# lmb-freiburg/optical-flow-2d-data-generation

Measured on AMD Instinct MI355X. Metric: training samples/sec (img0+img1+flow, 512x384), higher is better.
Workload: dtype u8 blends / fp64 affines -> f32 planes

## Files before the change

### include/ofdg.h

```cpp
#ifndef OFDG_H_
#define OFDG_H_

#include <stddef.h>
#include <stdint.h>

#ifdef __cplusplus
extern "C" {
#endif

#define OFDG_OK          0
#define OFDG_EBADMODE   (-1)
#define OFDG_ETEXTURES  (-2)
#define OFDG_EOBJTYPE   (-3)
#define OFDG_EHIP       (-4)
#define OFDG_ECAPACITY  (-5)
#define OFDG_EINVAL     (-6)
#define OFDG_ESTARTUP   (-7)

#define OFDG_OBJ_DUMMY     0
#define OFDG_OBJ_ELLIPSE   1
#define OFDG_OBJ_POLYGON   2
#define OFDG_OBJ_COMPOSITE 3
#define OFDG_SEG_DUMMY     0
#define OFDG_SEG_LINE      1
// ... 130 lines not shown
  int32_t  reserved[3];
} ofdg_extras_fmt;
int ofdg_render_ex_fmt(ofdg_ctx* ctx, const ofdg_task* tasks, int n_tasks, const ofdg_blueprint* bps, int n_bps,
                       void* d_image0, void* d_image1, void* d_flow, const ofdg_extras_fmt* ex, const ofdg_out_format* fmt,
                       void* stream);
int ofdg_forward_ex_fmt(ofdg_ctx* ctx, void* d_image0, void* d_image1, void* d_flow, const ofdg_extras_fmt* ex,
                        const ofdg_out_format* fmt, void* stream);
int ofdg_forward_counter_ex_fmt(ofdg_ctx* ctx, long long first_index, int n_samples, void* d_image0, void* d_image1,
                                void* d_flow, const ofdg_extras_fmt* ex, const ofdg_out_format* fmt, void* stream);

#define OFDG_MAX_OBJECT_ROWS 65
typedef struct ofdg_object_row {
  int32_t obj_id;
  int32_t obj_type;
  int32_t area0, area1;
  int32_t box0[4];
  int32_t box1[4];
  double  motion[6];
} ofdg_object_row;
int ofdg_object_table(ofdg_ctx* ctx, const uint8_t* d_label0, const uint8_t* d_label1,
                      ofdg_object_row* d_rows, int rows_per_sample, int32_t* d_counts, void* stream);
int ofdg_host_object_table(const uint8_t* label0, const uint8_t* label1, int n, int width, int height,
                           const int32_t* counts, ofdg_object_row* rows, int rows_per_sample);

#define OFDG_FLOW_HIST_BINS 64
#define OFDG_STATS_ACCUMULATE   1
#define OFDG_STATS_VISIBLE_ONLY 2
#define OFDG_STATS_ONE_ROW      4
typedef struct ofdg_flow_stats_row {
  uint32_t hist[OFDG_FLOW_HIST_BINS];
  uint32_t n_counted, n_bad, n_occluded, reserved;
  int64_t  sum_u_q8, sum_v_q8, sum_mag_q8;
  uint64_t max_key;
} ofdg_flow_stats_row;
int ofdg_flow_stats(ofdg_ctx* ctx, const void* d_flow, int flow_fmt, const void* d_occ, int occ_fmt,
                    int n_samples, float bin_px, int flags, ofdg_flow_stats_row* d_rows, void* stream);
int ofdg_host_flow_stats(const void* flow, int flow_fmt, const void* occ, int occ_fmt, int n, int width, int height,
                         float bin_px, int flags, ofdg_flow_stats_row* rows);

#define OFDG_PYR_MAX_LEVELS 6
#define OFDG_PYR_SCALE 1
struct ofdg_flow_pyramid {
  void* flow[OFDG_PYR_MAX_LEVELS];
  void* weight[OFDG_PYR_MAX_LEVELS];
  int32_t levels;
  int32_t out_fmt;
};
int ofdg_flow_pyramid(ofdg_ctx* ctx, const void* d_flow, int flow_fmt, const void* d_occ, int occ_fmt,
                      int n_samples, int flags, const struct ofdg_flow_pyramid* pyr, void* stream);
int ofdg_host_flow_pyramid(const void* flow, int flow_fmt, const void* occ, int occ_fmt, int n, int width, int height,
                           int flags, const struct ofdg_flow_pyramid* pyr);

int ofdg_flow_stats_sized(ofdg_ctx* ctx, const void* d_flow, int flow_fmt, const void* d_occ, int occ_fmt, int n_samples,
                          int width, int height, float bin_px, int flags, ofdg_flow_stats_row* d_rows, void* stream);
int ofdg_flow_pyramid_sized(ofdg_ctx* ctx, const void* d_flow, int flow_fmt, const void* d_occ, int occ_fmt, int n_samples,
                            int width, int height, int flags, const struct ofdg_flow_pyramid* pyr, void* stream);

#define OFDG_CROP_HFLIP         1
#define OFDG_CROP_VFLIP         2
#define OFDG_CROP_RANDOM_HFLIP  4
#define OFDG_CROP_RANDOM_VFLIP  8
#define OFDG_CROP_OCC_WINDOW   16
typedef struct ofdg_crop_rec { int32_t x0, y0, flags, reserved; } ofdg_crop_rec;
enum { OFDG_CROP_IMAGE0, OFDG_CROP_IMAGE1, OFDG_CROP_FLOW, OFDG_CROP_FLOW1,
       OFDG_CROP_OCC0, OFDG_CROP_OCC1, OFDG_CROP_LABEL0, OFDG_CROP_LABEL1, OFDG_CROP_PLANES };
struct ofdg_crop_job {
  const void* src[OFDG_CROP_PLANES];
  void*       dst[OFDG_CROP_PLANES];
  const ofdg_crop_rec* recs;
  ofdg_crop_rec*       recs_out;
  long long first_index;  uint32_t seed;
  int32_t crop_w, crop_h, flags, image_fmt, flow_fmt, occ_fmt, reserved;
};
int ofdg_crop(ofdg_ctx* ctx, const struct ofdg_crop_job* job, int n_samples, void* stream);
int ofdg_host_crop(const struct ofdg_crop_job* job, int n_samples, int width, int height);
int ofdg_crop_draw(uint32_t seed, long long index, int width, int height, int crop_w, int crop_h, int flags, ofdg_crop_rec* out);
int ofdg_crop_philox(const uint32_t counter[4], const uint32_t key[2], uint32_t out[4]);

long long ofdg_get_step(const ofdg_ctx* ctx);
int ofdg_set_step(ofdg_ctx* ctx, long long step);

void* ofdg_stream(ofdg_ctx* ctx);
int ofdg_num_chains(const ofdg_ctx* ctx);

int ofdg_synchronize(ofdg_ctx* ctx, void* stream);

int ofdg_poll_errors(ofdg_ctx* ctx);
long long ofdg_last_ticket(const ofdg_ctx* ctx);
int ofdg_poll_errors_of(ofdg_ctx* ctx, long long ticket);

int ofdg_warp_generate(ofdg_ctx* ctx, int n_fields, uint32_t seed);
int ofdg_warp_upload(ofdg_ctx* ctx, const float* crops, int n);
int ofdg_warp_info(const ofdg_ctx* ctx, int* n_crops, int* w, int* h);
int ofdg_warp_download(ofdg_ctx* ctx, int index, float* crop);
int ofdg_host_displacers(int width, int height, uint32_t seed, double* out, int cap);

int ofdg_debug_rasterize(ofdg_ctx* ctx, const double* xy, int n_vertices,
                         uint8_t* coverage_host);
int ofdg_debug_rasterize_path(ofdg_ctx* ctx, const double* xy, const int* types, int n, uint8_t* coverage_host);
int ofdg_debug_dda_rows(ofdg_ctx* ctx, const double* inv, int rows, int len, int* out_xy);
int ofdg_debug_coverage(ofdg_ctx* ctx, int sample, int shape, int frame,
                        uint8_t* coverage_host);
int ofdg_debug_num_shapes(ofdg_ctx* ctx, int sample);
int ofdg_debug_item_count(ofdg_ctx* ctx);
int ofdg_debug_bgprep_tiles(ofdg_ctx* ctx, int* tiles, int* workgroups);
int ofdg_debug_bgprep_paths(ofdg_ctx* ctx, unsigned* counts9);
int ofdg_debug_tables(ofdg_ctx* ctx, uint8_t* add_tbl, uint8_t* sub_tbl, uint8_t* aa_tbl,
                      uint8_t* blend_tbl, int s_fixed);
int ofdg_debug_detmath(ofdg_ctx* ctx, const double* angles, int n, double* sin_out, double* cos_out,
                       const float* x, int m, float* expf_out);
int ofdg_set_profiling(ofdg_ctx* ctx, int mode);
int ofdg_kernel_ms(ofdg_ctx* ctx, const char* kernel, float* ms);

typedef struct ofdg_host_sampler ofdg_host_sampler;
int ofdg_host_sampler_create(int mode, int width, int height, int num_objects,
                             ofdg_host_sampler** out);
int ofdg_host_sampler_next(ofdg_host_sampler* s, int n_tasks, ofdg_task* tasks,
                           ofdg_blueprint* bps, int bps_capacity, int* n_bps);
void ofdg_host_sampler_destroy(ofdg_host_sampler* s);
int ofdg_host_realize(const ofdg_params* prm, int pool_n, int pool_w, int pool_h,
                      const ofdg_task* tasks, int n_tasks, const ofdg_blueprint* bps,
                      int n_bps, double* shape_mats, int shape_cap, int* n_shapes,
                      double* object_mats, int object_cap, int* n_objects);
int ofdg_host_bg_prep(int pool_w, int pool_h, int width, int height, float angle, float zoom,
                      int shift_x, int shift_y, float* f, int* i);

int ofdg_host_decode_image(const char* path, uint8_t* planar_bgr, size_t capacity, int* width, int* height);

int ofdg_parse_prototxt(const char* text, ofdg_params* out, char* texture_dbases,
                        int texture_dbases_cap, int* n_top);
const char* ofdg_host_last_error(void);

typedef struct ofdg_layer ofdg_layer;
int ofdg_layer_create(const char* layer_prototxt, ofdg_layer** out);
int ofdg_layer_forward(ofdg_layer* layer, float** image0, float** image1, float** flow,
                       int* shape4);
void ofdg_layer_destroy(ofdg_layer* layer);
int ofdg_layer_in_flight(const ofdg_layer* layer);

#define OFDG_UNIQUE_ID_BYTES 128
#define OFDG_POOL_SYNTHETIC 0
#define OFDG_POOL_UNIFORM   1
#define OFDG_POOL_MIXED     2
typedef struct ofdg_setup {
  int32_t seed, mode, width, height, num_objects, use_antialiasing, batch_size, sampler, background_prep;
  int32_t n_tex;
  int32_t pool_kind;
  int32_t pool_w, pool_h;
  uint32_t pool_seed;
  int32_t n_table;
  int32_t status;
  int32_t max_shapes_per_sample;
  int32_t reserved;
} ofdg_setup;
typedef struct ofdg_tex_entry {
  uint64_t offset;
  uint32_t w, h, pitch, reserved;
} ofdg_tex_entry;
typedef struct ofdg_comm ofdg_comm;
int ofdg_comm_unique_id(void* id);
int ofdg_comm_init(const void* id, int rank, int world_size, int device, ofdg_comm** out);
int ofdg_comm_adopt(void* nccl_comm, int rank, int world_size, int device, ofdg_comm** out);
void ofdg_comm_destroy(ofdg_comm* comm);
int ofdg_comm_rank(const ofdg_comm* comm);
int ofdg_comm_world_size(const ofdg_comm* comm);
const char* ofdg_comm_last_error(const ofdg_comm* comm);
// ... 18 lines not shown
```

### optical-flow-2d-data-generation_amd/__init__.py

```python
import ctypes as C
import os
import subprocess

HERE = os.path.dirname(os.path.abspath(__file__))
LIB_PATH = os.environ.get("OFDG_LIB") or os.path.join(HERE, "lib", "libofdg.so")
MAX_SEG = 20

OK, EBADMODE, ETEXTURES, EOBJTYPE, EHIP, ECAPACITY, EINVAL, ESTARTUP = 0, -1, -2, -3, -4, -5, -6, -7
OBJ_ELLIPSE, OBJ_POLYGON, OBJ_COMPOSITE = 1, 2, 3
STREAM_OWN = (1 << 64) - 1
SEG_DUMMY, SEG_LINE, SEG_CURVE3 = 0, 1, 3


class Blueprint(C.Structure):
    _fields_ = [
        ("obj_id", C.c_int32), ("obj_type", C.c_int32),
        ("init_rot", C.c_float), ("init_scale", C.c_float),
        ("init_trans_x", C.c_float), ("init_trans_y", C.c_float),
        ("rot", C.c_float), ("scale", C.c_float),
        ("trans_x", C.c_float), ("trans_y", C.c_float),
        ("tex_id", C.c_int32), ("tex_rot", C.c_float), ("tex_scale", C.c_float),
        ("tex_shift_x", C.c_int32), ("tex_shift_y", C.c_int32),
        ("ellipse_scale_x", C.c_float), ("ellipse_scale_y", C.c_float),
        ("n_segments", C.c_int32),
        ("segment_type", C.c_int32 * MAX_SEG),
        ("segment_x", C.c_float * MAX_SEG),
        ("segment_y", C.c_float * MAX_SEG),
        ("first_component", C.c_int32), ("n_components", C.c_int32),
        ("is_additive_component", C.c_int32),
        ("do_warpfield_deformation", C.c_int32),
    ]


class Task(C.Structure):
    _fields_ = [("background", C.c_int32), ("first_object", C.c_int32),
                ("n_objects", C.c_int32), ("reserved", C.c_int32)]


class Params(C.Structure):
    _fields_ = [
        ("width", C.c_int32), ("height", C.c_int32), ("mode", C.c_int32),
        ("use_antialiasing", C.c_int32), ("batch_size", C.c_int32), ("prefetch", C.c_int32),
        ("first_level_threads", C.c_int32), ("second_level_threads", C.c_int32),
        ("num_objects", C.c_int32), ("sampler", C.c_int32), ("seed", C.c_int32),
        ("rank", C.c_int32), ("world_size", C.c_int32), ("device", C.c_int32),
        ("max_shapes_per_sample", C.c_int32), ("background_prep", C.c_int32),
        ("chains", C.c_int32), ("lookahead", C.c_int32), ("serial", C.c_int32), ("reserved", C.c_int32 * 5),
    ]


class Setup(C.Structure):
    _fields_ = [(k, C.c_int32) for k in ("seed", "mode", "width", "height", "num_objects", "use_antialiasing", "batch_size",
                                         "sampler", "background_prep", "n_tex", "pool_kind", "pool_w", "pool_h")] + \
               [("pool_seed", C.c_uint32), ("n_table", C.c_int32), ("status", C.c_int32), ("max_shapes_per_sample", C.c_int32),
                ("reserved", C.c_int32)]


class TexEntry(C.Structure):
    _fields_ = [("offset", C.c_uint64), ("w", C.c_uint32), ("h", C.c_uint32), ("pitch", C.c_uint32), ("reserved", C.c_uint32)]


UNIQUE_ID_BYTES = 128
POOL_SYNTHETIC, POOL_UNIFORM, POOL_MIXED = 0, 1, 2


class OfdgError(RuntimeError):
    def __init__(self, code, msg):
        super().__init__("ofdg error %d: %s" % (code, msg))
        self.code = code


_lib = None

EXPORTS = [
    "ofdg_default_params", "ofdg_create", "ofdg_destroy", "ofdg_last_error", "ofdg_ctx_info",
    "ofdg_host_bg_prep", "ofdg_ctx_params", "ofdg_pool_alloc_mixed", "ofdg_pool_upload_mixed", "ofdg_pool_synthetic", "ofdg_pool_alloc", "ofdg_pool_upload", "ofdg_pool_download", "ofdg_pool_info", "ofdg_pool_device",
    "ofdg_sample", "ofdg_render", "ofdg_render_resident", "ofdg_upload_slot", "ofdg_render_slot", "ofdg_forward", "ofdg_shard_first_index", "ofdg_synchronize", "ofdg_stream", "ofdg_get_step", "ofdg_set_step",
    "ofdg_debug_rasterize", "ofdg_debug_rasterize_path", "ofdg_debug_dda_rows", "ofdg_debug_coverage", "ofdg_debug_num_shapes", "ofdg_debug_item_count", "ofdg_debug_bgprep_tiles", "ofdg_debug_bgprep_paths", "ofdg_debug_tables", "ofdg_debug_detmath",
    "ofdg_set_profiling", "ofdg_kernel_ms",
    "ofdg_forward_counter", "ofdg_sample_counter", "ofdg_warp_generate", "ofdg_warp_upload", "ofdg_warp_info", "ofdg_warp_download", "ofdg_host_displacers",
    "ofdg_host_sampler_create", "ofdg_host_sampler_next", "ofdg_host_sampler_destroy", "ofdg_host_realize",
    "ofdg_parse_prototxt", "ofdg_host_last_error", "ofdg_host_decode_image", "ofdg_layer_create", "ofdg_layer_forward", "ofdg_layer_destroy",
    "ofdg_layer_in_flight", "ofdg_poll_errors", "ofdg_poll_errors_of", "ofdg_last_ticket", "ofdg_num_chains",
    "ofdg_comm_unique_id", "ofdg_comm_init", "ofdg_comm_adopt", "ofdg_comm_destroy", "ofdg_comm_rank", "ofdg_comm_world_size",
    "ofdg_comm_last_error", "ofdg_comm_bcast_setup", "ofdg_comm_bcast_abort", "ofdg_comm_nccl_count", "ofdg_comm_bcast_pool", "ofdg_comm_agree", "ofdg_setup_of", "ofdg_setup_params",
    "ofdg_setup_alloc_pool", "ofdg_pool_device_mixed", "ofdg_pool_device_image", "ofdg_layer_create_dist",
    "ofdg_render_ex", "ofdg_forward_ex", "ofdg_forward_counter_ex",
    "ofdg_render_fmt", "ofdg_forward_fmt", "ofdg_forward_counter_fmt",
    "ofdg_render_ex_fmt", "ofdg_forward_ex_fmt", "ofdg_forward_counter_ex_fmt",
    "ofdg_object_table", "ofdg_host_object_table",
    "ofdg_flow_stats", "ofdg_host_flow_stats",
    "ofdg_flow_pyramid", "ofdg_host_flow_pyramid",
    "ofdg_flow_stats_sized", "ofdg_flow_pyramid_sized", "ofdg_crop", "ofdg_host_crop", "ofdg_crop_draw", "ofdg_crop_philox",
]

EXTRAS = {"flow1": (2, "float32"), "occ0": (1, "float32"), "occ1": (1, "float32"), "label0": (None, "uint8"), "label1": (None, "uint8")}


class Extras(C.Structure):
    _fields_ = [("flow1", C.c_void_p), ("occ0", C.c_void_p), ("occ1", C.c_void_p), ("label0", C.c_void_p), ("label1", C.c_void_p)]


FMT_F32, FMT_U8, FMT_F16 = 0, 1, 2
_FMT_NAMES = {"f32": FMT_F32, "u8": FMT_U8, "f16": FMT_F16}


class OutFormat(C.Structure):
    _fields_ = [("image", C.c_int32), ("flow", C.c_int32), ("reserved", C.c_int32 * 2)]


def output_format(image0, image1, flow, n, height, width):
    def name(t):
        return str(t.dtype).replace("torch.", "")

    if image0.dtype != image1.dtype:
        raise ValueError("image0 and image1 must have one dtype, got %s and %s" % (name(image0), name(image1)))
    codes = []
    for what, t, valid in (("image0", image0, {"float32": FMT_F32, "uint8": FMT_U8}), ("flow", flow, {"float32": FMT_F32, "float16": FMT_F16})):
        if name(t) not in valid:
            raise ValueError("%s must be %s, got %s" % (what, " or ".join(sorted(valid)), name(t)))
        codes.append(valid[name(t)])
    for what, t, ch in (("image0", image0, 3), ("image1", image1, 3), ("flow", flow, 2)):
        if t.numel() < n * ch * height * width:
            raise ValueError("%s holds %d elements, [%d,%d,%d,%d] needs %d" % (what, t.numel(), n, ch, height, width, n * ch * height * width))
    return tuple(codes)


class ExtrasFmt(C.Structure):
    _fields_ = [("flow1", C.c_void_p), ("occ0", C.c_void_p), ("occ1", C.c_void_p), ("label0", C.c_void_p), ("label1", C.c_void_p),
                ("occ", C.c_int32), ("reserved", C.c_int32 * 3)]


def extras_format(extras, flow_code, n, height, width):
    def name(t):
        return str(t.dtype).replace("torch.", "")

    flow_dt = {FMT_F32: "float32", FMT_F16: "float16"}[flow_code]
    occ_dt = None
    for key, t in extras.items():
        if key not in EXTRAS:
            raise ValueError("unknown extra output %r (known: %s)" % (key, ", ".join(EXTRAS)))
        if t is None:
            continue
        ch = EXTRAS[key][0]
        shape = (n, height, width) if ch is None else (n, ch, height, width)
        if key == "flow1":
            valid = (flow_dt,)
        elif key in ("occ0", "occ1"):
            valid = ("float32", "uint8") if occ_dt is None else (occ_dt,)
        else:
            valid = ("uint8",)
        if tuple(t.shape) != shape or name(t) not in valid:
            why = " (the dtype of flow)" if key == "flow1" else " (occ0 and occ1 alike)" if key in ("occ0", "occ1") else ""
            raise ValueError("extra %r must be %s %s%s, got %s %s" % (key, " or ".join(valid), shape, why, name(t), tuple(t.shape)))
        if key in ("occ0", "occ1"):
            occ_dt = name(t)
    return FMT_U8 if occ_dt == "uint8" else FMT_F32


def _fmt_codes(fmt):
    if fmt is None:
        return FMT_F32, FMT_F32
    image, flow = fmt
    return tuple(_FMT_NAMES[f] if isinstance(f, str) else int(f) for f in (image, flow))


# ... 239 lines not shown
        L.ofdg_default_params.restype = None
        L.ofdg_create.argtypes = [C.POINTER(Params), C.POINTER(vp)]
        L.ofdg_destroy.argtypes = [vp]
        L.ofdg_destroy.restype = None
        L.ofdg_last_error.argtypes = [vp]
        L.ofdg_last_error.restype = C.c_char_p
        L.ofdg_ctx_info.argtypes = [vp]
        L.ofdg_ctx_info.restype = C.c_char_p
        L.ofdg_pool_synthetic.argtypes = [vp, i32, i32, i32, C.c_uint32]
        L.ofdg_pool_alloc.argtypes = [vp, i32, i32, i32]
        L.ofdg_pool_upload.argtypes = [vp, i32, vp, i32, i32]
        L.ofdg_pool_download.argtypes = [vp, i32, vp]
        L.ofdg_pool_device.argtypes = [vp, C.POINTER(vp), C.POINTER(C.c_ulonglong), i32]
        L.ofdg_pool_info.argtypes = [vp, C.POINTER(i32), C.POINTER(i32), C.POINTER(i32)]
        L.ofdg_sample.argtypes = [vp, i32, vp, vp, i32, C.POINTER(i32)]
        L.ofdg_render.argtypes = [vp, vp, i32, vp, i32, vp, vp, vp, vp]
        L.ofdg_render_resident.argtypes = [vp, vp, vp, vp, vp]
        L.ofdg_upload_slot.argtypes = [vp, i32, vp, i32, vp, i32, vp]
        L.ofdg_render_slot.argtypes = [vp, i32, vp, vp, vp, vp]
        L.ofdg_forward.argtypes = [vp, vp, vp, vp, vp]
        L.ofdg_synchronize.argtypes = [vp, vp]
        L.ofdg_stream.argtypes = [vp]
        L.ofdg_get_step.argtypes = [vp]
        L.ofdg_get_step.restype = C.c_longlong
        L.ofdg_set_step.argtypes = [vp, C.c_longlong]
        L.ofdg_stream.restype = vp
        L.ofdg_debug_rasterize.argtypes = [vp, vp, i32, vp]
        L.ofdg_debug_rasterize_path.argtypes = [vp, vp, vp, i32, vp]
        L.ofdg_debug_dda_rows.argtypes = [vp, vp, i32, i32, vp]
        L.ofdg_debug_coverage.argtypes = [vp, i32, i32, i32, vp]
        L.ofdg_debug_num_shapes.argtypes = [vp, i32]
        L.ofdg_debug_tables.argtypes = [vp, vp, vp, vp, vp, i32]
        L.ofdg_debug_bgprep_tiles.argtypes = [vp, C.POINTER(i32), C.POINTER(i32)]
        L.ofdg_debug_bgprep_paths.argtypes = [vp, C.POINTER(C.c_uint32)]
        L.ofdg_debug_detmath.argtypes = [vp, vp, i32, vp, vp, vp, i32, vp]
        L.ofdg_set_profiling.argtypes = [vp, i32]
        L.ofdg_kernel_ms.argtypes = [vp, C.c_char_p, C.POINTER(C.c_float)]
        L.ofdg_forward_counter.argtypes = [vp, C.c_longlong, i32, vp, vp, vp, vp]
        L.ofdg_render_ex.argtypes = [vp, vp, i32, vp, i32, vp, vp, vp, C.POINTER(Extras), vp]
        L.ofdg_forward_ex.argtypes = [vp, vp, vp, vp, C.POINTER(Extras), vp]
        L.ofdg_forward_counter_ex.argtypes = [vp, C.c_longlong, i32, vp, vp, vp, C.POINTER(Extras), vp]
        L.ofdg_render_fmt.argtypes = [vp, vp, i32, vp, i32, vp, vp, vp, C.POINTER(OutFormat), vp]
        L.ofdg_forward_fmt.argtypes = [vp, vp, vp, vp, C.POINTER(OutFormat), vp]
        L.ofdg_forward_counter_fmt.argtypes = [vp, C.c_longlong, i32, vp, vp, vp, C.POINTER(OutFormat), vp]
        L.ofdg_render_ex_fmt.argtypes = [vp, vp, i32, vp, i32, vp, vp, vp, C.POINTER(ExtrasFmt), C.POINTER(OutFormat), vp]
        L.ofdg_forward_ex_fmt.argtypes = [vp, vp, vp, vp, C.POINTER(ExtrasFmt), C.POINTER(OutFormat), vp]
        L.ofdg_forward_counter_ex_fmt.argtypes = [vp, C.c_longlong, i32, vp, vp, vp, C.POINTER(ExtrasFmt), C.POINTER(OutFormat), vp]
        L.ofdg_object_table.argtypes = [vp, vp, vp, vp, i32, vp, vp]
        L.ofdg_host_object_table.argtypes = [vp, vp, i32, i32, i32, vp, vp, i32]
        L.ofdg_flow_stats.argtypes = [vp, vp, i32, vp, i32, i32, C.c_float, i32, vp, vp]
        L.ofdg_host_flow_stats.argtypes = [vp, i32, vp, i32, i32, i32, i32, C.c_float, i32, vp]
        L.ofdg_flow_pyramid.argtypes = [vp, vp, i32, vp, i32, i32, i32, C.POINTER(FlowPyramid), vp]
        L.ofdg_host_flow_pyramid.argtypes = [vp, i32, vp, i32, i32, i32, i32, i32, C.POINTER(FlowPyramid)]
        L.ofdg_flow_stats_sized.argtypes = [vp, vp, i32, vp, i32, i32, i32, i32, C.c_float, i32, vp, vp]
        L.ofdg_flow_pyramid_sized.argtypes = [vp, vp, i32, vp, i32, i32, i32, i32, i32, C.POINTER(FlowPyramid), vp]
        L.ofdg_crop.argtypes = [vp, C.POINTER(CropJob), i32, vp]
        L.ofdg_host_crop.argtypes = [C.POINTER(CropJob), i32, i32, i32]
        L.ofdg_crop_draw.argtypes = [C.c_uint32, C.c_longlong, i32, i32, i32, i32, i32, C.POINTER(CropRec)]
        L.ofdg_crop_philox.argtypes = [C.POINTER(C.c_uint32 * 4), C.POINTER(C.c_uint32 * 2), C.POINTER(C.c_uint32 * 4)]
        L.ofdg_sample_counter.argtypes = [vp, C.c_longlong, i32, vp, vp]
        L.ofdg_warp_generate.argtypes = [vp, i32, C.c_uint32]
        L.ofdg_warp_upload.argtypes = [vp, vp, i32]
        L.ofdg_warp_info.argtypes = [vp, C.POINTER(i32), C.POINTER(i32), C.POINTER(i32)]
        L.ofdg_warp_download.argtypes = [vp, i32, vp]
        L.ofdg_host_displacers.argtypes = [i32, i32, C.c_uint32, vp, i32]
        L.ofdg_host_sampler_create.argtypes = [i32, i32, i32, i32, C.POINTER(vp)]
        L.ofdg_host_sampler_next.argtypes = [vp, i32, vp, vp, i32, C.POINTER(i32)]
        L.ofdg_host_sampler_destroy.argtypes = [vp]
        L.ofdg_host_sampler_destroy.restype = None
        L.ofdg_host_realize.argtypes = [C.POINTER(Params), i32, i32, i32, vp, i32, vp, i32, vp, i32, C.POINTER(i32),
                                        vp, i32, C.POINTER(i32)]
        L.ofdg_parse_prototxt.argtypes = [C.c_char_p, C.POINTER(Params), C.c_char_p, i32, C.POINTER(i32)]
        L.ofdg_host_last_error.restype = C.c_char_p
        L.ofdg_layer_create.argtypes = [C.c_char_p, C.POINTER(vp)]
        L.ofdg_layer_forward.argtypes = [vp, C.POINTER(vp), C.POINTER(vp), C.POINTER(vp), C.POINTER(i32 * 4)]
        L.ofdg_layer_destroy.argtypes = [vp]
        L.ofdg_layer_destroy.restype = None
        L.ofdg_layer_in_flight.argtypes = [vp]
        L.ofdg_poll_errors.argtypes = [vp]
        L.ofdg_poll_errors_of.argtypes = [vp, C.c_longlong]
        L.ofdg_last_ticket.argtypes = [vp]
        L.ofdg_last_ticket.restype = C.c_longlong
        L.ofdg_num_chains.argtypes = [vp]
        L.ofdg_comm_unique_id.argtypes = [vp]
        L.ofdg_comm_init.argtypes = [vp, i32, i32, i32, C.POINTER(vp)]
        L.ofdg_comm_adopt.argtypes = [vp, i32, i32, i32, C.POINTER(vp)]
        L.ofdg_comm_destroy.argtypes = [vp]
        L.ofdg_comm_destroy.restype = None
        L.ofdg_comm_rank.argtypes = [vp]
        L.ofdg_comm_world_size.argtypes = [vp]
        L.ofdg_comm_last_error.argtypes = [vp]
        L.ofdg_comm_last_error.restype = C.c_char_p
        L.ofdg_comm_bcast_setup.argtypes = [vp, i32, C.POINTER(Setup), vp, i32]
        L.ofdg_comm_bcast_pool.argtypes = [vp, i32, vp]
        L.ofdg_comm_agree.argtypes = [vp, i32]
        L.ofdg_comm_bcast_abort.argtypes = [vp, i32, i32, i32]
        L.ofdg_comm_nccl_count.argtypes = [vp]
        L.ofdg_setup_of.argtypes = [vp, C.POINTER(Setup), vp, i32]
        L.ofdg_setup_params.argtypes = [C.POINTER(Setup), vp, C.POINTER(Params)]
        L.ofdg_setup_alloc_pool.argtypes = [vp, C.POINTER(Setup), vp]
        L.ofdg_pool_device_image.argtypes = [vp, i32, C.POINTER(vp), C.POINTER(C.c_ulonglong)]
        L.ofdg_pool_device_mixed.argtypes = [vp, C.POINTER(vp), C.POINTER(C.c_ulonglong), C.POINTER(vp), C.POINTER(C.c_ulonglong)]
        L.ofdg_layer_create_dist.argtypes = [C.c_char_p, vp, C.POINTER(vp)]
        _lib = L
    return _lib


def shard_first_index(step, batch, world_size, rank):
    L = lib()
    L.ofdg_shard_first_index.argtypes = [C.c_longlong, C.c_int, C.c_int, C.c_int]
    L.ofdg_shard_first_index.restype = C.c_longlong
    return int(L.ofdg_shard_first_index(step, batch, world_size, rank))


def default_params(**kw):
    p = Params()
    lib().ofdg_default_params(C.byref(p))
    for k, v in kw.items():
        setattr(p, k, v)
    return p


class Generator:

    def __init__(self, params=None, **kw):
        self.params = params if params is not None else default_params(**kw)
        h = C.c_void_p()
        rc = lib().ofdg_create(C.byref(self.params), C.byref(h))
        if rc != OK:
            raise OfdgError(rc, lib().ofdg_last_error(None).decode())
        self.h = h
        self._last_n = None
        self._slot_n = {}

    def _check(self, rc):
        if rc != OK:
            raise OfdgError(rc, lib().ofdg_last_error(self.h).decode())

    def info(self):
        return lib().ofdg_ctx_info(self.h).decode()

    def close(self):
        if getattr(self, "h", None):
            lib().ofdg_destroy(self.h)
            self.h = None

    def __del__(self):
        try:
            self.close()
        except Exception:
            pass

    def pool_synthetic(self, n, w, h, seed=0):
        self._check(lib().ofdg_pool_synthetic(self.h, n, w, h, seed))

    def pool_alloc(self, n, w, h):
        self._check(lib().ofdg_pool_alloc(self.h, n, w, h))

    def pool_from_setup(self, setup, table=None):
        self._check(lib().ofdg_setup_alloc_pool(self.h, C.byref(setup), table))

    def pool_upload(self, index, bgr_planar):
        import numpy as np
        a = np.ascontiguousarray(bgr_planar, np.uint8)
        _, h, w = a.shape
        self._check(lib().ofdg_pool_upload(self.h, index, a.ctypes.data_as(C.c_void_p), w, h))
# ... 115 lines not shown
    def render_resident(self, img0, img1, flow, stream=0):
        self._check(lib().ofdg_render_resident(self.h, _dptr(img0), _dptr(img1), _dptr(flow), C.c_void_p(stream)))

    def upload_slot(self, slot, tasks, n_tasks, bps, n_bps, stream=0):
        self._check(lib().ofdg_upload_slot(self.h, slot, C.cast(tasks, C.c_void_p), n_tasks, C.cast(bps, C.c_void_p), n_bps,
                                           C.c_void_p(stream)))
        self._slot_n[slot] = n_tasks

    def render_slot(self, slot, img0, img1, flow, stream=0):
        self._check(lib().ofdg_render_slot(self.h, slot, _dptr(img0), _dptr(img1), _dptr(flow), C.c_void_p(stream)))
        self._last_n = self._slot_n.get(slot)

    def forward(self, img0, img1, flow, stream=0, extras=None, fmt=None):
        self._call("forward", (), img0, img1, flow, self.params.batch_size, stream, extras, fmt)

    def forward_counter(self, first_index, n, img0, img1, flow, stream=0, extras=None, fmt=None):
        self._call("forward_counter", (first_index, n), img0, img1, flow, n, stream, extras, fmt)

    def object_table(self, label0, label1, rows, counts, stream=0):
        n, per = object_table_format(label0, label1, rows, counts, self.params.height, self.params.width, self._last_n)
        self._check(lib().ofdg_object_table(self.h, _dptr(label0) if label0 is not None else None,
                                            _dptr(label1) if label1 is not None else None, _dptr(rows), per, _dptr(counts),
                                            C.c_void_p(stream)))

    def flow_stats(self, flow, rows, occ=None, bin_px=2.0, accumulate=False, visible_only=False, one_row=False, stream=0, size=None):
        height, width = (int(size[0]), int(size[1])) if size is not None else (self.params.height, self.params.width)
        n, fcode, ocode = flow_stats_format(flow, occ, rows, height, width, one_row)
        entry, plane = (lib().ofdg_flow_stats_sized, (width, height)) if size is not None else (lib().ofdg_flow_stats, ())
        self._check(entry(self.h, _dptr(flow), fcode, _dptr(occ) if occ is not None else None, ocode, n, *plane, float(bin_px),
                          _stats_flags(accumulate, visible_only, one_row), _dptr(rows), C.c_void_p(stream)))

    def flow_pyramid(self, flow, levels, occ=None, scale=True, out_dtype=None, weights=False, out=None, stream=0, size=None):
        n, height, width = int(flow.shape[0]), self.params.height, self.params.width
        if size is not None:
            height, width = int(size[0]), int(size[1])
        if out is None:
            out = alloc_flow_pyramid(n, height, width, levels, flow.dtype if out_dtype is None else out_dtype, weights, flow.device)
        lv, wt = out if isinstance(out, tuple) else (out, None)
        n, fcode, ocode, out_code = flow_pyramid_format(flow, occ, levels, lv, wt, height, width)
        rec = _pyramid_record(int(levels), out_code, [_dptr(t) for t in lv], None if wt is None else [_dptr(t) for t in wt])
        entry, plane = (lib().ofdg_flow_pyramid_sized, (width, height)) if size is not None else (lib().ofdg_flow_pyramid, ())
        self._check(entry(self.h, _dptr(flow), fcode, _dptr(occ) if occ is not None else None, ocode, n, *plane,
                          PYR_SCALE if scale else 0, C.byref(rec), C.c_void_p(stream)))
        return out

    def crop(self, src, dst, recs=None, first_index=0, seed=None, hflip=False, vflip=False, occ_window=False, recs_out=None, stream=0):
        n, crop_h, crop_w, *codes = crop_format(src, dst, self.params.height, self.params.width)
        for t in (recs, recs_out):
            if t is not None and (str(t.dtype) != "torch.int32" or tuple(t.shape) != (n, 4)):
                raise ValueError("recs and recs_out must be int32 [%d,4], got %s %s" % (n, t.dtype, tuple(t.shape)))
        job = _crop_job(src, dst, _dptr, codes, crop_h, crop_w, None if recs is None else _dptr(recs), None if recs_out is None else _dptr(recs_out),
                        first_index, self.params.seed if seed is None else seed, _crop_flags(hflip, vflip, occ_window))
        self._check(lib().ofdg_crop(self.h, C.byref(job), n, C.c_void_p(stream)))
        return dst

    def sample_counter(self, first_index, n):
        tasks = (Task * n)()
        bps = (Blueprint * (n * 257))()
        self._check(lib().ofdg_sample_counter(self.h, first_index, n, C.cast(tasks, C.c_void_p), C.cast(bps, C.c_void_p)))
        return tasks, bps, n * 257

    def synchronize(self, stream=0):
        self._check(lib().ofdg_synchronize(self.h, C.c_void_p(stream)))

    def last_ticket(self):
        return int(lib().ofdg_last_ticket(self.h))

    def poll_errors(self):
        self._check(lib().ofdg_poll_errors(self.h))

    def poll_errors_of(self, ticket):
        self._check(lib().ofdg_poll_errors_of(self.h, ticket))

    @property
    def step(self):
        return int(lib().ofdg_get_step(self.h))

    @step.setter
    def step(self, k):
        self._check(lib().ofdg_set_step(self.h, int(k)))

    def num_chains(self):
        return lib().ofdg_num_chains(self.h)

    def next_stream(self):
        return int(lib().ofdg_stream(self.h) or 0)

    def warp_generate(self, n_fields=1, seed=0):
        self._check(lib().ofdg_warp_generate(self.h, n_fields, seed))

    def warp_upload(self, crops):
        import numpy as np
        a = np.ascontiguousarray(crops, np.float32)
        assert a.ndim == 4 and a.shape[1:] == (4, self.params.height + 1, self.params.width + 1), a.shape
        self._check(lib().ofdg_warp_upload(self.h, a.ctypes.data_as(C.c_void_p), a.shape[0]))

    def warp_count(self):
        n = C.c_int()
        self._check(lib().ofdg_warp_info(self.h, C.byref(n), None, None))
        return n.value

    def warp_download(self, index):
        import numpy as np
        a = np.zeros((4, self.params.height + 1, self.params.width + 1), np.float32)
        self._check(lib().ofdg_warp_download(self.h, index, a.ctypes.data_as(C.c_void_p)))
        return a

    def debug_rasterize(self, xy):
        import numpy as np
        xy = np.ascontiguousarray(xy, np.float64)
        cov = np.zeros((self.params.height, self.params.width), np.uint8)
        self._check(lib().ofdg_debug_rasterize(self.h, xy.ctypes.data_as(C.c_void_p), len(xy), cov.ctypes.data_as(C.c_void_p)))
        return cov

    def debug_rasterize_path(self, xy, types):
        import numpy as np
        xy = np.ascontiguousarray(xy, np.float64)
        types = np.ascontiguousarray(types, np.int32)
        cov = np.zeros((self.params.height, self.params.width), np.uint8)
        self._check(lib().ofdg_debug_rasterize_path(self.h, xy.ctypes.data_as(C.c_void_p), types.ctypes.data_as(C.c_void_p), len(xy),
                                                    cov.ctypes.data_as(C.c_void_p)))
        return cov

    def debug_dda_rows(self, inv, rows, length):
        import numpy as np
        inv = np.ascontiguousarray(inv, np.float64)
        out = np.zeros((rows, length, 2), np.int32)
        self._check(lib().ofdg_debug_dda_rows(self.h, inv.ctypes.data_as(C.c_void_p), rows, length, out.ctypes.data_as(C.c_void_p)))
        return out

    def debug_num_shapes(self, sample):
        n = lib().ofdg_debug_num_shapes(self.h, sample)
        if n < 0:
            raise OfdgError(n, "debug_num_shapes")
        return n

    def debug_coverage(self, sample, shape, frame):
        import numpy as np
        cov = np.zeros((self.params.height, self.params.width), np.uint8)
        self._check(lib().ofdg_debug_coverage(self.h, sample, shape, frame, cov.ctypes.data_as(C.c_void_p)))
        return cov

    def debug_bgprep_tiles(self):
        t, w = C.c_int(0), C.c_int(0)
        self._check(lib().ofdg_debug_bgprep_tiles(self.h, C.byref(t), C.byref(w)))
        return t.value, w.value

    def debug_bgprep_paths(self):
        c = (C.c_uint32 * 9)()
        self._check(lib().ofdg_debug_bgprep_paths(self.h, c))
        return [[int(c[3 * r + k]) for k in range(3)] for r in range(3)]

    def debug_tables(self, s_fixed=200):
        import numpy as np
        add = np.zeros((256, 256), np.uint8)
        sub = np.zeros((256, 256), np.uint8)
        aa = np.zeros(256, np.uint8)
        bl = np.zeros((256, 256), np.uint8)
        vp = C.c_void_p
        self._check(lib().ofdg_debug_tables(self.h, add.ctypes.data_as(vp), sub.ctypes.data_as(vp), aa.ctypes.data_as(vp),
                                            bl.ctypes.data_as(vp), s_fixed))
        return add, sub, aa, bl

    def debug_detmath(self, angles, x):
        import numpy as np
        a = np.ascontiguousarray(angles, np.float64)
# ... 550 lines not shown
```

### optical-flow-2d-data-generation_amd/csrc/kernels.hip

```cpp
#include <hip/hip_runtime.h>
#include <stdint.h>
#include <type_traits>

#include "../../include/ofdg_detmath.h"
#include "ofdg_device.h"
#include "realize.h"
#include "warpfields.h"

namespace ofdg {

__device__ __forceinline__ int iround_d(double v) {
  return (int)((v < 0.0) ? v - 0.5 : v + 0.5);
}
__device__ __forceinline__ void xform(const Mat& m, double& x, double& y) {
  double t = x;
  x = t * m.sx + y * m.shx + m.tx;
  y = t * m.shy + y * m.sy + m.ty;
}
__device__ __forceinline__ long long floordiv64(long long a, long long b) {
  long long q = (long long)floor((double)a / (double)b);
  long long r = a - q * b;
  if (r < 0) --q;
  else if (r >= b) ++q;
  return q;
// ... 146 lines not shown
      xform(M, x, y);
      const int2 v = make_int2(iround_d(x * 256.0), iround_d(y * 256.0));
      out[k] = v;
      minx = min(minx, v.x); maxx = max(maxx, v.x);
      miny = min(miny, v.y); maxy = max(maxy, v.y);
    }
  } else {
    n_verts = path_verts(S.n_seg, [&](int i) { return S.seg_type[i]; },
                         [&](int i, double& x, double& y) { x = (double)S.seg_x[i]; y = (double)S.seg_y[i]; xform(M, x, y); },
                         out, stack, stage, err, lane, minx, miny, maxx, maxy);
  }
  minx = wave_min(minx); miny = wave_min(miny); maxx = wave_max(maxx); maxy = wave_max(maxy);
  return n_verts;
}

struct GeomWs {
  double stack[kCurveSlots][kCurveMaxDepth][5];
  int2 stage[kCurveSlots][kCurveMaxPts];
};
__device__ __forceinline__ void geom_wave(GeomWs& ws, int sf, int lane, const DevShape* __restrict__ shapes, int n_shapes,
                                          const double* __restrict__ cs_tab, int W, int H, DevShapeFrame* __restrict__ frames,
                                          int2* __restrict__ verts, unsigned long long* __restrict__ blockmask, uint32_t* __restrict__ err,
                                          int* __restrict__ item_count, int4* __restrict__ items, const DevCropRef* __restrict__ crops) {
  if (sf >= n_shapes * 2) return;
  const DevShape& S = shapes[sf >> 1];
  if (S.type == 0) return;
  const Mat M = S.m[sf & 1];
  int2* out = verts + (size_t)sf * kMaxVerts;

  int minx, miny, maxx, maxy;
  int n_verts = outline_verts(S, M, cs_tab, out, ws.stack, ws.stage, err, lane, minx, miny, maxx, maxy);
  if (n_verts > 0 && ((long long)maxx - (long long)minx >= (16384LL << 8))) {
    if (lane == 0) atomicOr(err, kErrDxLimit);
    n_verts = 0;
  }
  int x0 = minx >> 8, y0 = miny >> 8, x1 = maxx >> 8, y1 = maxy >> 8;
  const bool visible = !(n_verts < 2 || x1 < 0 || y1 < 0 || x0 > W - 1 || y0 > H - 1);
  int bx0 = 1, by0 = 1, bx1 = 0, by1 = 0;
  if (visible) {
    x0 = max(x0, 0); y0 = max(y0, 0); x1 = min(x1, W - 1); y1 = min(y1, H - 1);
    bx0 = x0; by0 = y0; bx1 = x1; by1 = y1;
    if ((sf & 1) && S.deform > 0) {
      const int d = (int)ceilf(__uint_as_float(*crops[S.deform - 1].max_bits)) + 2;
      bx0 = max(x0 - d, 0); by0 = max(y0 - d, 0); bx1 = min(x1 + d, W - 1); by1 = min(y1 + d, H - 1);
    }
  } else {
    x0 = 1; x1 = 0; y0 = 1; y1 = 0;
  }
  if (lane == 0) {
    DevShapeFrame f;
    f.n_verts = n_verts;
    f.x0 = x0; f.y0 = y0; f.x1 = x1; f.y1 = y1;
    f.pad[0] = S.sample; f.pad[1] = S.obj_local; f.pad[2] = 0;
    frames[sf] = f;
  }
  if (visible) {
    const int band0 = by0 / kBandRows, band1 = by1 / kBandRows;
    if ((sf & 1) && S.deform > 0) {
      const int nbx = (W + kTileW - 1) / kTileW, nby = (H + kBandRows - 1) / kBandRows;
      const int c0 = bx0 / kTileW, nc = bx1 / kTileW - c0 + 1;
      unsigned long long* m = blockmask + ((size_t)S.sample * nbx * nby) * 2 + (sf & 1);
      const unsigned long long bit = 1ull << S.obj_local;
      for (int i = lane; i < (band1 - band0 + 1) * nc; i += 64)
        atomicOr(m + (size_t)((band0 + i / nc) * nbx + c0 + i % nc) * 2, bit);
    }
    const int xa = (bx0 / kTileW) * kTileW, xb = min((bx1 / kTileW) * kTileW + kTileW - 1, W - 1);
    const int nchunks = (xb - xa + kChunkW) / kChunkW;
    const int n_items = (band1 - band0 + 1) * nchunks;
    int base = 0;
    if (lane == 0) base = atomicAdd(item_count, n_items);
    base = __shfl(base, 0, 64);
    for (int i = lane; i < n_items; i += 64) {
      const int b = band0 + i / nchunks, cx = xa + (i % nchunks) * kChunkW;
      items[base + i] = make_int4(sf, b, cx, min(cx + kChunkW - 1, xb));
    }
  }
}

__global__ __launch_bounds__(64 * kGeomWaves) void geom_kernel(const DevShape* __restrict__ shapes, int n_shapes,
                                                   const double* __restrict__ cs_tab, int W, int H,
                                                   DevShapeFrame* __restrict__ frames, int2* __restrict__ verts,
                                                   unsigned long long* __restrict__ blockmask, uint32_t* __restrict__ err,
                                                   int* __restrict__ item_count, int4* __restrict__ items,
                                                   const DevCropRef* __restrict__ crops) {
  __shared__ GeomWs s_ws[kGeomWaves];
  step_kernel_priority();
  const int wave = threadIdx.x >> 6, lane = threadIdx.x & 63;
  const int sf = __builtin_amdgcn_readfirstlane(blockIdx.x * kGeomWaves + wave);
  geom_wave(s_ws[wave], sf, lane, shapes, n_shapes, cs_tab, W, H, frames, verts, blockmask, err, item_count, items, crops);
}

struct CellAcc {
  int* cover;
  int* area;
  int pitch, X0, X1;
  __device__ __forceinline__ void add(int r, int cell, int dcover, int darea) const {
    if (cell > X1 || dcover == 0) return;
    if (cell < X0) {
      atomicAdd(&cover[r * pitch], dcover);
    } else {
      const int i = r * pitch + (cell - X0 + 1);
      atomicAdd(&cover[i], dcover);
      atomicAdd(&area[i], darea);
    }
  }
};

__device__ __forceinline__ int fdiv_small(int num, int den, float rcp) {
  int q = (int)floorf((float)num * rcp);
  const int r = num - q * den;
  if (r < 0) --q;
  else if (r >= den) ++q;
  return q;
}
__device__ __forceinline__ int fdiv_big(int num, int den, float rcp) {
  const int q0 = (int)floorf((float)num * rcp);
  const int r0 = num - q0 * den;
  return q0 + fdiv_small(r0, den, rcp);
}

template <class Acc>
__device__ __forceinline__ void hline32(const Acc& acc, int r, int xa, int ya, int xb, int yb) {
  if (ya == yb) return;
  const int exa = xa >> 8, exb = xb >> 8;
  const int fxa = xa & 255, fxb = xb & 255;
  const int Dy = yb - ya;
  if (exa == exb) {
    acc.add(r, exa, Dy, (fxa + fxb) * Dy);
    return;
  }
  const int lo = min(exa, exb), hi = max(exa, exb);
  if (hi < acc.X0) { acc.add(r, acc.X0 - 1, Dy, 0); return; }
  if (lo > acc.X1) return;
  const bool right = xb > xa;
  const int adx = right ? xb - xa : xa - xb;
  const float rcp = __frcp_rn((float)adx);
  const int m = hi - lo;
  const int f0 = right ? 256 - fxa : fxa;
  const int j_lo = right ? max(0, acc.X0 - exa) : max(0, exa - acc.X1);
  const int j_hi = right ? min(m, acc.X1 - exa) : min(m, exa - acc.X0);
  int yprev = (j_lo == 0) ? ya : ya + fdiv_small((f0 + 256 * (j_lo - 1)) * Dy, adx, rcp);
  if (right && j_lo > 0) acc.add(r, acc.X0 - 1, yprev - ya, 0);
  for (int j = j_lo; j <= j_hi; ++j) {
    const int ynext = (j == m) ? yb : ya + fdiv_small((f0 + 256 * j) * Dy, adx, rcp);
    const int d = ynext - yprev;
    const int fin = (j == 0) ? fxa : (right ? 0 : 256);
    const int fout = (j == m) ? fxb : (right ? 256 : 0);
    acc.add(r, right ? exa + j : exa - j, d, (fin + fout) * d);
    yprev = ynext;
  }
  if (!right && j_hi < m) acc.add(r, acc.X0 - 1, yb - yprev, 0);
}

template <class Acc>
__device__ __forceinline__ void hline(const Acc& acc, int r, int xa, int ya, int xb, int yb) {
  if (ya == yb) return;
  const int exa = xa >> 8, exb = xb >> 8;
  const int fxa = xa & 255, fxb = xb & 255;
  const int Dy = yb - ya;
  if (exa == exb) {
    acc.add(r, exa, Dy, (fxa + fxb) * Dy);
    return;
  }
  if (xb > xa) {
    const int m = exb - exa;
    const long long dxh = xb - xa;
    const long long f0 = 256 - fxa;
    int j = 0;
    int yprev = ya;
    if (exa < acc.X0) {
      const int jb = min(acc.X0 - exa, m + 1);
      int yb0 = (jb > m) ? yb : ya + (int)floordiv64((f0 + 256LL * (jb - 1)) * Dy, dxh);
// ... 2802 lines not shown
```

### optical-flow-2d-data-generation_amd/csrc/ofdg_api.hip

```cpp
#include <hip/hip_runtime.h>
#include <hip/hip_ext.h>

#include <algorithm>
#include <cmath>
#include <cstddef>
#include <cstdio>
#include <cstdlib>
#include <cstring>
#include <memory>
#include <string>
#include <type_traits>
#include <vector>

#include "../../include/ofdg.h"
#include "kernels.hip"
#include "sampler_counter.hip"
#include "cimg_resize.h"
#include "ofdg_device.h"
#include "owners.h"
#include "realize.h"
#include "sampler_ref.h"
#include "warpfields.h"

using namespace ofdg;
// ... 2 lines not shown
static const int g_hw_queues_env = [] { const char* q = std::getenv("GPU_MAX_HW_QUEUES"); return q ? std::atoi(q) : 0; }();

struct ofdg_ctx {
  ofdg_params prm;
  std::string err;
  std::string info;
  DevBuf<uint32_t> d_prep_paths;
  DevBuf<uint32_t> pool;
  int pool_n = 0, pool_w = 0, pool_h = 0;
  DevBuf<uint32_t> pool_fg;
  DevBuf<uint32_t> pool_bg;
  TexSource fg_src{}, bg_src{};
  bool pool_final = false;
  bool pool_mixed = false;
  std::vector<std::pair<int, int>> mixed_sizes;
  std::vector<DevBuf<uint32_t>> mixed_images;
  std::vector<DevTexEntry> tex_table;
  DevBuf<DevTexEntry> d_tex_table;
  int pool_kind = OFDG_POOL_UNIFORM;
  uint32_t pool_seed = 0;
  std::unique_ptr<RefSampler> sampler;
  long long step = 0;
  struct Slot {
    RealizedBatch batch;
    DevBuf<DevShape> d_shapes;
    DevBuf<DevShapeFrame> d_frames;
    DevBuf<int2> d_verts;
    DevBuf<DevObject> d_objects;
    DevBuf<DevSample> d_samples;
    DevBuf<char> d_rec;
    DevBuf<int4> d_items;
    DevBuf<DevBgPrep> d_bgprep;
    DevBuf<uint32_t> d_bgtex;
    DevBuf<uint32_t> d_bgC;
    DevBuf<unsigned long long> d_blockmask;
    int res_objects = 0;
    bool bgprep_pending = false;
    int box_parity = 0;
    size_t box_stride = 0;
    int mask_used[2] = {0, 0};
    Event ev_uploaded;
    bool upload_pending = false;
    hipStream_t upload_stream = nullptr;
    DevBuf<DevCropRef> d_croptab;
    DevBuf<float> d_bgwarp;
    DevBuf<unsigned> d_bgwarp_max;
    hipEvent_t compose_event = nullptr;
    bool compose_pending = false;
    hipStream_t compose_stream = nullptr;
    DevBuf<int> d_item_count;
    int res_samples = 0, res_shapes = 0;
  };
  static constexpr int kUserSlots = 16;
  Slot slots[kUserSlots];
  struct Stage {
    PinnedBuf h;
    Event free_ev;
    bool pending = false;
  };
  Stage user_stage;
  struct Chain {
    Stream stream;
    DevBuf<uint8_t> cov;
    DevBuf<uint8_t> x_labels;
    DevBuf<float> x_flow1;
    DevBuf<uint32_t> x_targets;
    Slot slot;
    Stage stage;
    Event ev_prep;
    Event ev_done;
    bool done_pending = false;
    hipStream_t done_stream = nullptr;
    struct Prepared {
      bool valid = false;
      Slot* slot = nullptr;
      long long first_index = -1;
      int n = 0;
      unsigned long long* box_cur = nullptr;
      const DevCropRef* croptab = nullptr;
      Event* ev = nullptr;
      hipStream_t stream = nullptr;
      long long ticket = -1;
      bool ahead = false;
    } prep;
  };
  static constexpr int kMaxChains = 8;
  Chain chains[kMaxChains];
  int lookahead = 0;
  long long last_first = -1;
  int n_chains = 3;
  unsigned next_chain = 0;
  int last_chain = 0;
  Slot* last_slot = nullptr;
  Chain* last_ch = nullptr;
  hipStream_t last_stream = nullptr;
  hipStream_t last_user_st = nullptr;
  bool have_last_user_st = false;
  CsMode cs_mode;
  DevBuf<ofdg_blueprint> d_cs_bps;
  DevBuf<int> d_cs_nobj;
  long long next_index = 0;
  long long last_ticket = -1;
  DevBuf<float> d_warp;
  DevBuf<unsigned> d_warp_max;
  DevBuf<DevCropRef> d_cs_croptab;
  DevBuf<float> d_cs_bgwarp;
  DevBuf<unsigned> d_cs_bgwarp_max;
  CropServer crop_server;
  int rs_w = 0, rs_h = 0;
  DevBuf<int> d_rs_xi, d_rs_yi;
  DevBuf<double> d_rs_xa, d_rs_ya;
  bool overlap = true;
  DevBuf<double> d_cs_tab;
  static constexpr int kErrWords = 256;
  DevBuf<uint32_t> d_err;
  bool asked_by_ticket = false;
  bool word_clean[kErrWords];
  long long word_reserved = -1;
  long long ticket = 0;
  DevBuf<uint16_t> d_bg_at_x, d_bg_at_y;
  DevBuf<double> d_bg_alpha_x, d_bg_alpha_y;
  int bg_tab_w = 0, bg_tab_h = 0;
  int bg_cap_cw = 0, bg_cap_ch = 0, bg_cap_n = -1;
  bool bg_fusable = false;
  PinnedBuf h_err;
  Stream err_stream;
  int profiling = 0;
  std::vector<Event> ev;
  int ev_sets = 0, ev_stride = 1;
  long long ev_count = 0, ev_alloc = 0, launch_count = 0;
  std::vector<char> ev_composed;
  std::vector<char> ev_bgprep;
  std::vector<ofdg_task> fw_tasks;
  std::vector<ofdg_blueprint> fw_bps;
};

#define HIP_OK(ctx, call)                                                                     \
  do {                                                                                        \
    hipError_t e_ = (call);                                                                   \
    if (e_ != hipSuccess) {                                                                   \
      (ctx)->err = std::string(#call) + ": " + hipGetErrorString(e_);                         \
      return OFDG_EHIP;                                                                       \
    }                                                                                         \
  } while (0)
#define OFDG_TRY(expr)                                                                        \
  do {                                                                                        \
    const int rc_ = (expr);                                                                   \
    if (rc_ != OFDG_OK) return rc_;                                                           \
  } while (0)

template <typename P, typename A>
constexpr bool kArgFits = std::is_same<A, P>::value ||
                          (std::is_pointer<P>::value && (std::is_convertible<A, P>::value || std::is_same<A, void*>::value));
struct Launch { unsigned grid, block; hipStream_t stream; hipEvent_t start, stop; };
template <typename... P, typename... A>
static void launch_kernel(const Launch& l, void (*kernel)(P...), A... args) {
  static_assert(sizeof...(P) == sizeof...(A), "one argument per kernel parameter");
  static_assert((kArgFits<P, A> && ...), "an argument that is neither of its parameter's type nor a void* for a pointer");
  hipExtLaunchKernelGGL(kernel, dim3(l.grid), dim3(l.block), 0, l.stream, l.start, l.stop, 0, static_cast<P>(args)...);
}

static uint32_t* err_word(ofdg_ctx* c, long long ticket) { return c->d_err.p + (size_t)(ticket % ofdg_ctx::kErrWords); }
static hipError_t take_err_word(ofdg_ctx* c, long long ticket, hipStream_t s) {
  const size_t i = (size_t)(ticket % ofdg_ctx::kErrWords);
  hipError_t e = hipSuccess;
  if (c->word_reserved == ticket) c->word_reserved = -1;
  else if (c->asked_by_ticket && !c->word_clean[i]) e = hipMemsetAsync(c->d_err.p + i, 0, sizeof(uint32_t), s);
  c->word_clean[i] = false;
  return e;
}
static std::string err_text(uint32_t e) {
  std::string t = "device capacity exceeded:";
  if (e & kErrVertCapacity) t += " outline vertices > 1024;";
  if (e & kErrCurveCapacity) t += " curve3 subdivision points/depth;";
  if (e & kErrDxLimit) t += " edge spans >= 16384 px;";
  if (e & kErrBgPrepCapacity) t += " background_prep: crop of the rotated image exceeds the workspace (zoom < 0.75);";
  return t;
}

static int discard_all_prepared(ofdg_ctx* c);
static int texture_of_image(ofdg_ctx* c, const uint32_t* image, int w, int h, int tw, int th, uint32_t* out);

extern "C" {

const char* ofdg_last_error(const ofdg_ctx* ctx) { return ctx ? ctx->err.c_str() : g_create_error.c_str(); }

int ofdg_create(const ofdg_params* params, ofdg_ctx** out) {
  if (!params || !out) { g_create_error = "null argument"; return OFDG_EINVAL; }
  *out = nullptr;
  if (params->mode < 1 || params->mode > 13) { g_create_error = "BAD MODE"; return OFDG_EBADMODE; }
  if (params->width < 8 || params->height < 2 || (params->width % 8) != 0 || (params->height % 2) != 0) {
    g_create_error = "width must be a multiple of 8 and height even";
    return OFDG_EINVAL;
  }
  {
    const int cap = params->sampler == OFDG_SAMPLER_COUNTER ? kCsMaxObjects : kMaxFgObjects;
    if (params->num_objects < 0 || params->num_objects > cap) {
      g_create_error = "num_objects must be 0 (reference: 16..23) or 1.." + std::to_string(cap) + " for this sampler";
      return OFDG_EINVAL;
    }
  }
  int ndev = 0;
  hipError_t e = hipGetDeviceCount(&ndev);
  if (e != hipSuccess || ndev <= 0) {
    g_create_error = "no HIP device available (the HIP kernels are the only render path)";
    return OFDG_EHIP;
  }
  e = hipSetDevice(params->device);
  if (e != hipSuccess) { g_create_error = std::string("hipSetDevice: ") + hipGetErrorString(e); return OFDG_EHIP; }
  std::unique_ptr<ofdg_ctx> c(new ofdg_ctx());
  std::fill(c->word_clean, c->word_clean + ofdg_ctx::kErrWords, true);
  c->prm = *params;
  if (c->prm.world_size < 1) c->prm.world_size = 1;
  c->sampler.reset(new RefSampler(params->mode, params->width, params->height, params->num_objects));
  if (!c->sampler->ok()) { g_create_error = "BAD MODE"; return OFDG_EBADMODE; }
  c->cs_mode = make_cs_mode(params->mode, params->width, params->height, params->num_objects, (uint32_t)params->seed);
  double tab[200];
  const double pi = 3.14159265358979323846;
  for (int step = 0; step < 100; ++step) {
    const double angle = double(step) / double(100) * 2.0 * pi;
    tab[2 * step] = std::cos(angle);
    tab[2 * step + 1] = std::sin(angle);
  }
  if ((e = c->d_cs_tab.alloc(sizeof(tab) / sizeof(tab[0]))) != hipSuccess ||
      (e = hipMemcpy(c->d_cs_tab.p, tab, sizeof(tab), hipMemcpyHostToDevice)) != hipSuccess ||
      (e = c->d_err.alloc(ofdg_ctx::kErrWords + 1)) != hipSuccess ||
      (e = hipMemset(c->d_err.p, 0, (ofdg_ctx::kErrWords + 1) * sizeof(uint32_t))) != hipSuccess ||
      (e = c->user_stage.free_ev.create(hipEventDisableTiming)) != hipSuccess) {
    g_create_error = std::string("HIP initialisation: ") + hipGetErrorString(e);
    return OFDG_EHIP;
  }
  c->overlap = params->serial == 0;
  c->lookahead = std::max(params->lookahead, 0);
  c->n_chains = params->chains > 0 ? std::min(params->chains, (int)ofdg_ctx::kMaxChains) : (g_hw_queues_env >= 8 ? 4 : 3);
  c->info = "chains=" + std::to_string(c->n_chains) +
            (params->chains > 0 ? " (ofdg_params.chains)"
             : g_hw_queues_env >= 8 ? " (GPU_MAX_HW_QUEUES=" + std::to_string(g_hw_queues_env) + ": one hardware queue per chain)"
             : g_hw_queues_env > 0 ? " (GPU_MAX_HW_QUEUES=" + std::to_string(g_hw_queues_env) + " < 8: start the process with GPU_MAX_HW_QUEUES=8 for four chains, +5-8 %)"
                                   : " (GPU_MAX_HW_QUEUES was not set when the library was loaded: HIP's default of 4 hardware queues; start the process with GPU_MAX_HW_QUEUES=8 for four chains, +5-8 %)") +
            " lookahead=" + std::to_string(c->lookahead) + (c->overlap ? "" : " serial");
  for (int i = 0; i < c->n_chains; ++i) {
    ofdg_ctx::Chain& ch = c->chains[i];
    if ((e = ch.stream.create(hipStreamNonBlocking)) != hipSuccess ||
        (e = ch.stage.free_ev.create(hipEventDisableTiming)) != hipSuccess ||
        (e = ch.ev_prep.create(hipEventDisableTiming)) != hipSuccess ||
        (e = ch.ev_done.create(hipEventDisableTiming)) != hipSuccess) {
      g_create_error = std::string("hipStreamCreate: ") + hipGetErrorString(e);
      return OFDG_EHIP;
    }
  }
  {
    hipFuncAttributes fa;
    e = hipFuncGetAttributes(&fa, (const void*)compose_rigid_kernel);
    if (e != hipSuccess) {
      g_create_error = std::string("compose_rigid_kernel is not loadable (is the gfx950 code object present?): ") + hipGetErrorString(e);
      return OFDG_EHIP;
    }
  }
  *out = c.release();
  return OFDG_OK;
}

const ofdg_params* ofdg_ctx_params(const ofdg_ctx* c) { return c ? &c->prm : nullptr; }
const char* ofdg_ctx_info(const ofdg_ctx* c) { return c ? c->info.c_str() : ""; }

void ofdg_destroy(ofdg_ctx* c) {
  if (!c) return;
  (void)hipDeviceSynchronize();
  delete c;
}

static int pool_check_dims(ofdg_ctx* c, int n, int w, int h) {
  const int W = c->prm.width, H = c->prm.height;
  if (n < 1) { c->err = "texture pool needs at least one image"; return OFDG_ETEXTURES; }
  (void)W; (void)H;
  if (w < 2 || h < 2) { c->err = "pool images must be at least 2 x 2"; return OFDG_ETEXTURES; }
  return OFDG_OK;
}

int ofdg_pool_alloc(ofdg_ctx* c, int n, int w, int h) {
  if (!c) return OFDG_EINVAL;
  OFDG_TRY(discard_all_prepared(c));
  OFDG_TRY(pool_check_dims(c, n, w, h));
  HIP_OK(c, hipDeviceSynchronize());
  HIP_OK(c, c->pool.alloc((size_t)n * w * h));
  HIP_OK(c, hipMemset(c->pool.p, 0, (size_t)n * w * h * sizeof(uint32_t)));
  c->pool_n = n; c->pool_w = w; c->pool_h = h;
  c->pool_final = false;
  c->pool_mixed = false;
  c->pool_kind = OFDG_POOL_UNIFORM;
  return OFDG_OK;
}

int ofdg_pool_alloc_mixed(ofdg_ctx* c, int n) {
  if (!c) return OFDG_EINVAL;
  OFDG_TRY(discard_all_prepared(c));
  if (n < 1) { c->err = "texture pool needs at least one image"; return OFDG_ETEXTURES; }
  const int W = c->prm.width, H = c->prm.height;
  HIP_OK(c, hipDeviceSynchronize());
  c->mixed_images.clear();
  c->mixed_images.resize((size_t)n);
  c->d_tex_table.release();
  c->tex_table.clear();
  c->pool.release(); c->pool_fg.release(); c->pool_bg.release();
  HIP_OK(c, c->pool_fg.alloc((size_t)n * W * H));
  HIP_OK(c, c->pool_bg.alloc((size_t)n * 4 * W * H));
  HIP_OK(c, hipMemset(c->pool_fg.p, 0, (size_t)n * W * H * sizeof(uint32_t)));
  HIP_OK(c, hipMemset(c->pool_bg.p, 0, (size_t)n * 4 * W * H * sizeof(uint32_t)));
  HIP_OK(c, hipDeviceSynchronize());
  c->pool_n = n; c->pool_w = 0; c->pool_h = 0;
  c->fg_src = TexSource{(uint64_t)W * H, 0, W, 0};
  c->bg_src = TexSource{(uint64_t)4 * W * H, 0, 2 * W, 0};
  c->pool_mixed = true;
  c->pool_final = true;
  c->pool_kind = OFDG_POOL_MIXED;
  c->mixed_sizes.assign((size_t)n, std::make_pair(0, 0));
  return OFDG_OK;
}

int ofdg_pool_upload_mixed(ofdg_ctx* c, int index, const uint8_t* bgr_planar, int w, int h) {
  if (!c || !bgr_planar) return OFDG_EINVAL;
  OFDG_TRY(discard_all_prepared(c));
  if (!c->pool_mixed || index < 0 || index >= c->pool_n || w < 2 || h < 2) {
// ... 269 lines not shown
}

static int finalise_pool(ofdg_ctx* c) {
  if (c->pool_final) return OFDG_OK;
  if (c->pool_mixed) { c->pool_final = true; return OFDG_OK; }
  HIP_OK(c, hipDeviceSynchronize());
  const int W = c->prm.width, H = c->prm.height, w = c->pool_w, h = c->pool_h;
  const uint64_t img = (uint64_t)w * h;
  c->pool_fg.release();
  c->pool_bg.release();
  if (w >= W && h >= H) {
    c->fg_src = TexSource{img, (uint64_t)(h / 2 - H / 2) * w + (uint64_t)(w / 2 - W / 2), w, 0};
  } else {
    OFDG_TRY(pool_resized_copy(c, W, H, c->pool_fg));
    c->fg_src = TexSource{(uint64_t)W * H, 0, W, 0};
  }
  if (w >= 2 * W && h >= 2 * H) {
    c->bg_src = TexSource{img, (uint64_t)(h / 2 - H) * w + (uint64_t)(w / 2 - W), w, 0};
  } else {
    OFDG_TRY(pool_resized_copy(c, 2 * W, 2 * H, c->pool_bg));
    c->bg_src = TexSource{(uint64_t)4 * W * H, 0, 2 * W, 0};
  }
  c->pool_final = true;
  return OFDG_OK;
}

static int ensure_tex_table(ofdg_ctx* c) {
  if (!c->pool_mixed || !c->prm.background_prep || c->d_tex_table.p) return OFDG_OK;
  c->tex_table.resize((size_t)c->pool_n);
  for (int i = 0; i < c->pool_n; ++i) {
    if (!c->mixed_images[(size_t)i].p) { c->err = "background_prep: image " + std::to_string(i) + " of the mixed pool has not been uploaded"; return OFDG_ETEXTURES; }
    c->tex_table[(size_t)i] = DevTexEntry{(uint64_t)(uintptr_t)c->mixed_images[(size_t)i].p, c->mixed_sizes[(size_t)i].first, c->mixed_sizes[(size_t)i].second};
  }
  HIP_OK(c, c->d_tex_table.alloc(c->tex_table.size()));
  HIP_OK(c, hipMemcpy(c->d_tex_table.p, c->tex_table.data(), c->tex_table.size() * sizeof(DevTexEntry), hipMemcpyHostToDevice));
  return OFDG_OK;
}
static void bgprep_caps(ofdg_ctx* c, int* cap_cw, int* cap_ch, bool* fusable) {
  if (c->bg_cap_n == c->pool_n && c->bg_cap_cw > 0) { *cap_cw = c->bg_cap_cw; *cap_ch = c->bg_cap_ch; *fusable = c->bg_fusable; return; }
  const int TW = 2 * c->prm.width, TH = 2 * c->prm.height;
  int cw = (int)((float)TW / 0.75f) + 2, ch = (int)((float)TH / 0.75f) + 2;
  bool all_large = true;
  auto small = [&](int w, int h) { if (w < TW || h < TH) { all_large = false; cw = std::max(cw, w + h / 8 + 4); ch = std::max(ch, h + w / 8 + 4); } };
  if (c->pool_mixed) for (const auto& wh : c->mixed_sizes) small(wh.first, wh.second);
  else small(c->pool_w, c->pool_h);
  c->bg_cap_cw = cw; c->bg_cap_ch = ch; c->bg_cap_n = c->pool_n; c->bg_fusable = all_large;
  *cap_cw = cw; *cap_ch = ch; *fusable = all_large;
}

static int reserve_workspaces(ofdg_ctx* c, size_t n_shapes) {
  const size_t need_cov = n_shapes * 2 * (size_t)c->prm.width * c->prm.height + 16;
  if (need_cov <= c->chains[0].cov.cap) return OFDG_OK;
  HIP_OK(c, hipDeviceSynchronize());
  for (int k = 0; k < c->n_chains; ++k) HIP_OK(c, c->chains[k].cov.reserve(need_cov));
  return OFDG_OK;
}

static int ensure_item_count(ofdg_ctx* c, ofdg_ctx::Slot& sl) {
  if (sl.d_item_count.p) return OFDG_OK;
  HIP_OK(c, sl.d_item_count.alloc(1));
  HIP_OK(c, hipMemset(sl.d_item_count.p, 0, sizeof(int)));
  HIP_OK(c, hipDeviceSynchronize());
  return OFDG_OK;
}
static int size_slot(ofdg_ctx* c, ofdg_ctx::Slot& sl, int n_samples, size_t n_shapes, size_t n_objects = 0) {
  const int W = c->prm.width, H = c->prm.height;
  if (n_objects) HIP_OK(c, sl.d_shapes.reserve(n_shapes));
  HIP_OK(c, sl.d_frames.reserve(n_shapes * 2));
  HIP_OK(c, sl.d_verts.reserve(n_shapes * 2 * kMaxVerts));
  if (n_objects) {
    HIP_OK(c, sl.d_objects.reserve(n_objects));
    HIP_OK(c, sl.d_samples.reserve(n_samples));
  }
  OFDG_TRY(reserve_workspaces(c, n_shapes));
  HIP_OK(c, sl.d_items.reserve(n_shapes * 2 * (size_t)((H + kBandRows - 1) / kBandRows) * ((W + kChunkW - 1) / kChunkW) + 1));
  OFDG_TRY(reserve_blockmask(c, sl, n_samples));
  if (n_objects && c->prm.background_prep) {
    HIP_OK(c, sl.d_bgprep.reserve(n_samples));
    HIP_OK(c, sl.d_bgtex.reserve((size_t)n_samples * 4 * W * H));
  }
  return ensure_item_count(c, sl);
}

static int prepare_backgrounds(ofdg_ctx* c, ofdg_ctx::Slot& sl, int n, bool records_resident, hipStream_t s, uint32_t* err, hipEvent_t stop = nullptr);
static int launch_counter_sampler(ofdg_ctx* c, ofdg_ctx::Slot& sl, long long first_index, hipStream_t s, uint32_t* err) {
  const int stride = sl.res_shapes / sl.res_samples;
  const int prep = c->prm.background_prep ? 1 : 0;
  CsRealizeDims D{c->prm.width, c->prm.height, c->pool_n, c->pool_w, c->pool_h, sl.res_samples, stride, prep,
                  c->prm.mode == 9 ? c->crop_server.n_crops : 0, c->fg_src.stride, c->fg_src.origin, c->bg_src.stride, c->bg_src.origin,
                  (unsigned long long)(uintptr_t)c->pool.p, c->d_tex_table.p, c->prm.mode == 9 ? c->d_cs_croptab.p : nullptr};
  hipLaunchKernelGGL(cs_sample_realize_kernel, dim3(sl.res_samples * kCsGroups), dim3(64), 0, s, c->cs_mode, D, first_index,
                     sl.d_shapes.p, sl.d_objects.p, sl.d_samples.p, err, sl.d_bgprep.p);
  HIP_OK(c, hipGetLastError());
  sl.bgprep_pending = prep != 0;
  return OFDG_OK;
}

static void* own_stream(ofdg_ctx* c, void* stream) { return stream == OFDG_STREAM_OWN ? ofdg_stream(c) : stream; }

static ofdg_ctx::Chain& take_chain(ofdg_ctx* c) {
  const int k = (int)(c->next_chain % (unsigned)c->n_chains);
  c->next_chain++;
  c->last_chain = k;
  return c->chains[k];
}
static hipStream_t chain_stream(const ofdg_ctx* c, const ofdg_ctx::Chain& ch, hipStream_t st) { return c->overlap ? ch.stream.s : st; }

static int discard_prepared(ofdg_ctx* c, ofdg_ctx::Chain& ch) {
  if (!ch.prep.valid) return OFDG_OK;
  ch.prep.valid = false;
  if (ch.prep.slot && ch.prep.slot->d_item_count.p) HIP_OK(c, hipMemsetAsync(ch.prep.slot->d_item_count.p, 0, sizeof(int), ch.prep.stream));
  if (ch.prep.ticket >= 0 && ch.prep.ticket + ofdg_ctx::kErrWords > c->ticket) {
    HIP_OK(c, hipMemsetAsync(err_word(c, ch.prep.ticket), 0, sizeof(uint32_t), ch.prep.stream));
    c->word_clean[(size_t)(ch.prep.ticket % ofdg_ctx::kErrWords)] = true;
  }
  return OFDG_OK;
}
static int discard_all_prepared(ofdg_ctx* c) {
  c->bg_cap_n = -1;
  for (int k = 0; k < c->n_chains; ++k) OFDG_TRY(discard_prepared(c, c->chains[k]));
  return OFDG_OK;
}

static RenderDims render_dims(const ofdg_ctx* c, const ofdg_ctx::Slot& sl) {
  const int W = c->prm.width, H = c->prm.height;
  RenderDims dm;
  dm.W = W; dm.H = H; dm.pool_w = c->pool_w; dm.pool_h = c->pool_h;
  dm.use_aa = c->prm.use_antialiasing ? 1 : 0;
  dm.n_samples = sl.res_samples;
  dm.n_shapes = sl.res_shapes;
  dm.tiles_x = (W + kTileW - 1) / kTileW;
  dm.tiles_y = (H + kTileH - 1) / kTileH;
  dm.bg_pitch = c->prm.background_prep ? 2 * W : c->bg_src.pitch;
  dm.fg_pitch = c->fg_src.pitch;
  return dm;
}

static int wait_unless_fired(ofdg_ctx* c, hipStream_t s, hipEvent_t ev, bool* pending, bool settles = false) {
  if (hipEventQuery(ev) == hipSuccess) { *pending = false; return OFDG_OK; }
  HIP_OK(c, hipStreamWaitEvent(s, ev, 0));
  if (settles) *pending = false;
  return OFDG_OK;
}
static void track_completion(ofdg_ctx::Slot& sl, ofdg_ctx::Chain& ch, hipStream_t s, hipEvent_t done) {
  sl.compose_pending = true; sl.compose_stream = s; sl.compose_event = done;
  ch.done_pending = true; ch.done_stream = s;
}

static int launch_prepare(ofdg_ctx* c, ofdg_ctx::Chain& ch, ofdg_ctx::Slot& sl, hipStream_t st, long long cs_first_index = -1,
                          bool hand_over = true) {
  const int W = c->prm.width, H = c->prm.height;
  const int n_sf = sl.res_shapes * 2;
  const RenderDims dm = render_dims(c, sl);
  OFDG_TRY(discard_prepared(c, ch));
  const long long ticket = c->ticket++;
  uint32_t* const err = err_word(c, ticket);
  Event* ev = nullptr;
  if (c->profiling && c->ev_sets > 0 && (c->launch_count % c->ev_stride) == 0) {
    const size_t set = (size_t)(c->ev_alloc++ % c->ev_sets);
    ev = &c->ev[set * 6];
    c->ev_composed[set] = 0;
    c->ev_bgprep[set] = 0;
  }
  c->launch_count++;
  if (!c->overlap) {
    if (c->have_last_user_st && c->last_user_st != st) HIP_OK(c, hipDeviceSynchronize());
    c->last_user_st = st; c->have_last_user_st = true;
  }
  hipStream_t S = chain_stream(c, ch, st);
  uint8_t* cov = ch.cov.p;
  if (sl.upload_pending && sl.upload_stream != S) OFDG_TRY(wait_unless_fired(c, S, sl.ev_uploaded, &sl.upload_pending));
  if (ch.done_pending && ch.done_stream != S) OFDG_TRY(wait_unless_fired(c, S, ch.ev_done, &ch.done_pending, true));
  if (sl.compose_pending && sl.compose_stream != S) OFDG_TRY(wait_unless_fired(c, S, sl.compose_event, &sl.compose_pending));
  const DevCropRef* croptab = cs_first_index >= 0 ? c->d_cs_croptab.p : sl.d_croptab.p;
  HIP_OK(c, take_err_word(c, ticket, S));
  if (cs_first_index >= 0) {
    OFDG_TRY(launch_counter_sampler(c, sl, cs_first_index, S, err));
  }
  const int bp = sl.box_parity;
  sl.box_parity ^= 1;
  unsigned long long* box_cur = sl.d_blockmask.p + (size_t)bp * sl.box_stride;
  unsigned long long* box_next = sl.d_blockmask.p + (size_t)(bp ^ 1) * sl.box_stride;
  sl.mask_used[bp] = sl.res_samples * dm.tiles_x * ((H + kBandRows - 1) / kBandRows) * 2;
  const int n_mask_words = sl.mask_used[bp ^ 1];
  const bool prof_prep = ev && c->profiling == 2;
  hipExtLaunchKernelGGL(geom_kernel, dim3(std::max(1, (n_sf + kGeomWaves - 1) / kGeomWaves)), dim3(64 * kGeomWaves), 0, S,
                        prof_prep ? ev[0].e : nullptr, prof_prep ? ev[1].e : nullptr, 0, sl.d_shapes.p, sl.res_shapes, c->d_cs_tab.p, W, H,
                        sl.d_frames.p, sl.d_verts.p, box_cur, err, sl.d_item_count.p, sl.d_items.p, croptab);
  HIP_OK(c, hipGetLastError());
  const bool prep_last = sl.bgprep_pending;
  hipEvent_t last_stop = ev ? (c->profiling == 2 ? nullptr : ev[4].e) : (hand_over ? ch.ev_prep.e : nullptr);
  hipExtLaunchKernelGGL(raster_kernel, dim3(kRasterGrid * 4 / kRasterWaves), dim3(64 * kRasterWaves), 0, S, nullptr,
                        (ev && (c->profiling == 2 || prep_last)) ? ev[3].e : (prep_last ? nullptr : last_stop), 0,
                        sl.d_frames.p, sl.d_items.p, sl.d_item_count.p, sl.d_verts.p, W, H, cov, box_next, n_mask_words, box_cur);
  HIP_OK(c, hipGetLastError());
  if (prep_last) {
    OFDG_TRY(prepare_backgrounds(c, sl, sl.res_samples, true, S, err, (ev && c->profiling == 2) ? ev[2].e : last_stop));
    sl.bgprep_pending = false;
    if (ev) c->ev_bgprep[(size_t)(ev - c->ev.data()) / 6] = 1;
  }
  if (ev && hand_over) HIP_OK(c, hipEventRecord(ch.ev_prep, S));
  ch.prep.valid = true; ch.prep.slot = &sl; ch.prep.first_index = cs_first_index; ch.prep.n = sl.res_samples;
  ch.prep.box_cur = box_cur; ch.prep.croptab = croptab; ch.prep.ev = ev; ch.prep.stream = S; ch.prep.ticket = ticket;
  ch.prep.ahead = false;
  return OFDG_OK;
}

struct CallOut {
  const char* fn;
  void *img0, *img1, *flow;
  ofdg_extras_fmt ex;
  int out_fmt;
};
static int invalid_argument(ofdg_ctx* c, const char* fn) {
  if (c) c->err = std::string(fn) + ": invalid argument";
  return OFDG_EINVAL;
}
static bool extras_requested(const ofdg_extras_fmt* ex) { return ex && (ex->flow1 || ex->occ0 || ex->occ1 || ex->label0 || ex->label1); }
static ofdg_extras_fmt widen_extras(const ofdg_extras* ex) {
  ofdg_extras_fmt x{};
  if (ex) { x.flow1 = ex->flow1; x.occ0 = ex->occ0; x.occ1 = ex->occ1; x.label0 = ex->label0; x.label1 = ex->label1; }
  x.occ = OFDG_FMT_F32;
  return x;
}
static int check_extras(ofdg_ctx* c, const ofdg_extras_fmt* ex, const char* fn) {
  if (extras_requested(ex) && c->prm.mode == 9) {
    c->err = std::string(fn) + ": backward flow, labels and occlusion are defined for the rigid modes only (mode 9: the reference's "
             "inverse branch adds the forward warp field, DG:403-406, 715-716)";
    return OFDG_EINVAL;
  }
  return OFDG_OK;
}
static int check_extras_fmt(ofdg_ctx* c, const ofdg_extras_fmt* ex, const char* fn) {
  if (!ex) return OFDG_OK;
  auto fail = [&](const std::string& field, int value, const char* valid) {
    c->err = std::string(fn) + ": ofdg_extras_fmt." + field + " = " + std::to_string(value) + " (valid: " + valid + ")";
    return OFDG_EINVAL;
  };
  if (ex->occ != OFDG_FMT_F32 && ex->occ != OFDG_FMT_U8) return fail("occ", ex->occ, "OFDG_FMT_F32, OFDG_FMT_U8");
  for (int k = 0; k < 3; ++k)
    if (ex->reserved[k] != 0) return fail("reserved[" + std::to_string(k) + "]", ex->reserved[k], "0");
  return check_extras(c, ex, fn);
}
static int check_out_format(ofdg_ctx* c, const ofdg_out_format* fmt, const char* fn, int* out_fmt) {
  *out_fmt = 0;
  if (!fmt) return OFDG_OK;
  auto fail = [&](const char* field, int value, const char* valid) {
    c->err = std::string(fn) + ": ofdg_out_format." + field + " = " + std::to_string(value) + " (valid: " + valid + ")";
    return OFDG_EINVAL;
  };
  if (fmt->image != OFDG_FMT_F32 && fmt->image != OFDG_FMT_U8) return fail("image", fmt->image, "OFDG_FMT_F32, OFDG_FMT_U8");
  if (fmt->flow != OFDG_FMT_F32 && fmt->flow != OFDG_FMT_F16) return fail("flow", fmt->flow, "OFDG_FMT_F32, OFDG_FMT_F16");
  for (int k = 0; k < 2; ++k)
    if (fmt->reserved[k] != 0) return fail(k ? "reserved[1]" : "reserved[0]", fmt->reserved[k], "0");
  *out_fmt = (fmt->image == OFDG_FMT_U8 ? kOutImageU8 : 0) | (fmt->flow == OFDG_FMT_F16 ? kOutFlowF16 : 0);
  return OFDG_OK;
}
static int check_call(ofdg_ctx* c, const char* fn, bool args_ok, void* img0, void* img1, void* flow, const ofdg_extras* ex,
                      const ofdg_extras_fmt* exf, const ofdg_out_format* fmt, CallOut* o, const char* args_fn = nullptr) {
  if (!args_ok) return invalid_argument(c, args_fn ? args_fn : fn);
  *o = CallOut{fn, img0, img1, flow, exf ? *exf : widen_extras(ex), 0};
  OFDG_TRY(check_out_format(c, fmt, fn, &o->out_fmt));
  return exf ? check_extras_fmt(c, exf, fn) : check_extras(c, &o->ex, fn);
}

struct ComposeExtras {
  bool any = false;
  bool occ = false;
  bool fmt = false;
  ExtOut xo{nullptr, nullptr, nullptr};
  uint32_t *tgt0 = nullptr, *tgt1 = nullptr;
};
static int plan_extras(ofdg_ctx* c, ofdg_ctx::Chain& ch, int n_samples, const CallOut& o, ComposeExtras* x) {
  const ofdg_extras_fmt& ex = o.ex;
  if (!extras_requested(&ex)) return OFDG_OK;
  x->any = true;
  x->occ = ex.occ0 || ex.occ1;
  x->fmt = o.out_fmt || ex.occ == OFDG_FMT_U8;
  const size_t plane = (size_t)c->prm.width * c->prm.height, n = (size_t)n_samples;
  const bool ws_labels = x->occ && (!ex.label0 || !ex.label1), ws_flow1 = !x->fmt && ex.occ1 && !ex.flow1, ws_tgt = x->fmt && x->occ;
  if ((ws_labels && 2 * n * plane > ch.x_labels.cap) || (ws_flow1 && 2 * n * plane > ch.x_flow1.cap) ||
      (ws_tgt && 2 * n * plane > ch.x_targets.cap)) {
    HIP_OK(c, hipDeviceSynchronize());
    if (ws_labels) HIP_OK(c, ch.x_labels.reserve(2 * n * plane));
    if (ws_flow1) HIP_OK(c, ch.x_flow1.reserve(2 * n * plane));
    if (ws_tgt) HIP_OK(c, ch.x_targets.reserve(2 * n * plane));
  }
  if (ws_tgt) {
    x->tgt0 = ex.occ0 ? ch.x_targets.p : nullptr;
    x->tgt1 = ex.occ1 ? ch.x_targets.p + n * plane : nullptr;
  }
  x->xo.flow1 = ex.flow1 ? static_cast<float*>(ex.flow1) : (ws_flow1 ? ch.x_flow1.p : nullptr);
  x->xo.label0 = ex.label0 ? ex.label0 : (x->occ ? ch.x_labels.p : nullptr);
  x->xo.label1 = ex.label1 ? ex.label1 : (x->occ ? ch.x_labels.p + n * plane : nullptr);
  return OFDG_OK;
}

static int compose_stream(ofdg_ctx* c, ofdg_ctx::Chain& ch, hipStream_t st, hipStream_t* cs) {
  *cs = ch.prep.stream;
  if (*cs == st) return OFDG_OK;
  HIP_OK(c, hipStreamWaitEvent(st, ch.ev_prep, 0));
  *cs = st;
  return OFDG_OK;
}

static int launch_compose_kernels(ofdg_ctx* c, const ofdg_ctx::Chain& ch, const ofdg_ctx::Slot& sl, const CallOut& o, const ComposeExtras& x,
                                  const uint32_t* fgpool, const uint32_t* bgpool, hipStream_t cs, hipEvent_t done) {
  const int W = c->prm.width, H = c->prm.height;
  const RenderDims dm = render_dims(c, sl);
  const int grid = dm.tiles_x * dm.tiles_y * dm.n_samples * 4;
  Event* const ev = ch.prep.ev;
  enum class Kind { kRigid, kRigidExt, kRigidFmt, kRigidExtFmt, kDeform, kDeformFmt };
  const Kind kind = c->prm.mode == 9 ? (o.out_fmt ? Kind::kDeformFmt : Kind::kDeform)
                                     : x.fmt ? Kind::kRigidExtFmt : x.any ? Kind::kRigidExt : o.out_fmt ? Kind::kRigidFmt : Kind::kRigid;
  const bool pow2 = (W & (W - 1)) == 0;
  const Launch lc{(unsigned)grid, 64, cs, (ev && c->profiling == 2) ? ev[4].e : nullptr, ev ? ev[5].e : (x.occ ? nullptr : done)};
  auto compose = [&](auto* k_pow2, auto* k, auto... args) { launch_kernel(lc, pow2 ? k_pow2 : k, args...); };
  auto rigid = [&](auto* k_pow2, auto* k, auto... tail) {
    compose(k_pow2, k, sl.d_samples.p, ch.prep.box_cur, sl.d_objects.p, ch.cov.p, grid, dm.tiles_x, dm.tiles_y, W, H, dm.use_aa, dm.bg_pitch,
            dm.fg_pitch, fgpool, bgpool, o.img0, o.img1, o.flow, sl.d_frames.p, sl.d_item_count.p, tail...);
  };
  auto deform = [&](auto* k_pow2, auto* k, auto... tail) {
    compose(k_pow2, k, dm, sl.d_samples.p, sl.d_objects.p, ch.prep.box_cur, ch.cov.p, fgpool, bgpool, o.img0, o.img1, o.flow, sl.d_frames.p,
            ch.prep.croptab, sl.d_item_count.p, tail...);
  };
  switch (kind) {
    case Kind::kRigid: rigid(compose_rigid_pow2_kernel, compose_rigid_kernel); break;
    case Kind::kRigidExt: rigid(compose_rigid_ext_pow2_kernel, compose_rigid_ext_kernel, x.xo); break;
    case Kind::kRigidFmt: rigid(compose_rigid_fmt_pow2_kernel, compose_rigid_fmt_kernel, o.out_fmt); break;
    case Kind::kRigidExtFmt: rigid(compose_rigid_ext_fmt_pow2_kernel, compose_rigid_ext_fmt_kernel, x.xo, o.out_fmt, x.tgt0, x.tgt1); break;
    case Kind::kDeform: deform(compose_deform_pow2_kernel, compose_deform_kernel); break;
    case Kind::kDeformFmt: deform(compose_deform_fmt_pow2_kernel, compose_deform_fmt_kernel, o.out_fmt); break;
  }
  HIP_OK(c, hipGetLastError());
  if (x.occ) {
    const long long quads = (long long)dm.n_samples * H * (W / 4);
    const Launch lo{(unsigned)((quads + 255) / 256), 256, cs, nullptr, ev ? nullptr : done};
    if (x.fmt)
      launch_kernel(lo, occlusion_fmt_kernel, x.tgt0, x.tgt1, x.xo.label0, x.xo.label1, o.ex.occ0, o.ex.occ1, W, H, dm.n_samples,
                    o.ex.occ == OFDG_FMT_U8 ? kOutOccU8 : 0);
    else
      launch_kernel(lo, occlusion_kernel, o.flow, x.xo.flow1, x.xo.label0, x.xo.label1, o.ex.occ0, o.ex.occ1, W, H, dm.n_samples);
    HIP_OK(c, hipGetLastError());
  }
  return OFDG_OK;
}

static int note_compose(ofdg_ctx* c, ofdg_ctx::Chain& ch, ofdg_ctx::Slot& sl, hipStream_t cs, bool foreign, hipEvent_t done) {
  if (Event* const ev = ch.prep.ev) {
    if (done) HIP_OK(c, hipEventRecord(done, cs));
    const bool span_is_the_launch = c->profiling == 2 || (!foreign && !ch.prep.ahead);
    if (span_is_the_launch) {
      c->ev_count++;
      c->ev_composed[(size_t)(ev - c->ev.data()) / 6] = 1;
    }
  }
  if (done) track_completion(sl, ch, cs, done);
  else sl.compose_pending = false;
  return OFDG_OK;
}

static int launch_compose(ofdg_ctx* c, ofdg_ctx::Chain& ch, const CallOut& o, hipStream_t st) {
  if (!ch.prep.valid) { c->err = "internal: compose without a prepared batch"; return OFDG_EINVAL; }
  ofdg_ctx::Slot& sl = *ch.prep.slot;
  ComposeExtras x;
  OFDG_TRY(plan_extras(c, ch, sl.res_samples, o, &x));
  const uint32_t* bgpool = c->prm.background_prep ? sl.d_bgtex.p : (c->pool_bg.p ? c->pool_bg.p : c->pool.p);
  const uint32_t* fgpool = c->pool_fg.p ? c->pool_fg.p : c->pool.p;
  if (c->prm.background_prep && !bgpool) { c->err = "background_prep: the slot has no prepared backgrounds"; return OFDG_EINVAL; }
  c->last_slot = &sl; c->last_ch = &ch;
  c->last_stream = ch.prep.stream; c->last_ticket = ch.prep.ticket;
  ch.prep.valid = false;
  const bool foreign = ch.prep.stream != st;
  hipStream_t cs;
  OFDG_TRY(compose_stream(c, ch, st, &cs));
  const bool shared_slot = &sl != &ch.slot;
  const hipEvent_t done = (foreign || shared_slot) ? ch.ev_done.e : nullptr;
  OFDG_TRY(launch_compose_kernels(c, ch, sl, o, x, fgpool, bgpool, cs, done));
  return note_compose(c, ch, sl, cs, foreign, done);
}

static int launch_resident(ofdg_ctx* c, ofdg_ctx::Chain& ch, ofdg_ctx::Slot& sl, const CallOut& o, hipStream_t st, long long cs_first_index = -1) {
  OFDG_TRY(launch_prepare(c, ch, sl, st, cs_first_index, chain_stream(c, ch, st) != st));
  return launch_compose(c, ch, o, st);
}

constexpr int kPrepGrid = 4096;
static int ensure_bgprep_tables(ofdg_ctx* c) {
  const int TW = 2 * c->prm.width, TH = 2 * c->prm.height;
  if (c->bg_tab_w == TW && c->bg_tab_h == TH) return OFDG_OK;
  auto build = [&](int s, DevBuf<uint16_t>& d_at, DevBuf<double>& d_alpha) -> int {
    std::vector<uint16_t> at((size_t)s * s, 0);
    std::vector<double> alpha((size_t)s * s, 0.0);
    for (int n = 1; n < s; ++n) cimg_enlarge_table(n, s, &at[(size_t)n * s], &alpha[(size_t)n * s]);
    HIP_OK(c, d_at.reserve(at.size()));
    HIP_OK(c, d_alpha.reserve(alpha.size()));
    HIP_OK(c, hipMemcpy(d_at.p, at.data(), at.size() * sizeof(uint16_t), hipMemcpyHostToDevice));
    HIP_OK(c, hipMemcpy(d_alpha.p, alpha.data(), alpha.size() * sizeof(double), hipMemcpyHostToDevice));
    return OFDG_OK;
  };
  if (TW > 65535 || TH > 65535) { c->err = "background_prep: frame too large for the resize tables"; return OFDG_EINVAL; }
  HIP_OK(c, hipDeviceSynchronize());
  int rc = build(TW, c->d_bg_at_x, c->d_bg_alpha_x);
  if (rc == OFDG_OK) rc = build(TH, c->d_bg_at_y, c->d_bg_alpha_y);
  if (rc != OFDG_OK) return rc;
  c->bg_tab_w = TW; c->bg_tab_h = TH;
  return OFDG_OK;
}

static int prepare_backgrounds(ofdg_ctx* c, ofdg_ctx::Slot& sl, int n, bool records_resident, hipStream_t s, uint32_t* err, hipEvent_t stop) {
  const int W = c->prm.width, H = c->prm.height;
  if (!records_resident || !sl.d_bgprep.p || sl.d_bgprep.cap < (size_t)n) { c->err = "internal: background preparation without its records"; return OFDG_EINVAL; }
  HIP_OK(c, sl.d_bgtex.reserve((size_t)n * 4 * W * H));
  int cap_cw, cap_ch;
  bool fusable;
  bgprep_caps(c, &cap_cw, &cap_ch, &fusable);
  const bool staged = c->prm.background_prep == 1;
  constexpr int kBgPrepBlocks = 192;
  if (staged) {
    OFDG_TRY(ensure_bgprep_tables(c));
  }
  if (!staged) {
    hipExtLaunchKernelGGL(bgprep_kernel, dim3((W * H + 255) / 256, n), dim3(256), 0, s, nullptr, stop, 0, sl.d_bgprep.p, W, H, sl.d_bgtex.p);
    HIP_OK(c, hipGetLastError());
    return OFDG_OK;
  }
  const DevResizeTabs T{c->d_bg_at_x.p, c->d_bg_alpha_x.p, c->d_bg_at_y.p, c->d_bg_alpha_y.p};
  if (fusable && n <= kPrepMaxSamples) {
    hipExtLaunchKernelGGL(bgprep_stream_kernel, dim3(kPrepGrid), dim3(64), (size_t)(n + 1) * sizeof(int), s, nullptr, stop, 0, sl.d_bgprep.p, T, W, H, n, cap_cw, cap_ch, sl.d_bgtex.p, err,
                          c->d_prep_paths.p);
    HIP_OK(c, hipGetLastError());
    return OFDG_OK;
  }
  HIP_OK(c, sl.d_bgC.reserve((size_t)n * cap_cw * cap_ch));
  hipLaunchKernelGGL(bgprep_rotcrop_kernel, dim3(kBgPrepBlocks, n), dim3(256), 0, s, sl.d_bgprep.p, T, W, H, cap_cw, cap_ch, sl.d_bgC.p,
                     err);
  hipExtLaunchKernelGGL(bgprep_resize_kernel, dim3(kBgPrepBlocks, n), dim3(256), 0, s, nullptr, stop, 0, sl.d_bgprep.p, T, W, H, cap_cw, cap_ch, sl.d_bgC.p,
                        sl.d_bgtex.p);
  HIP_OK(c, hipGetLastError());
  return OFDG_OK;
}

static int upload_slot(ofdg_ctx* c, ofdg_ctx::Slot& sl, const ofdg_task* tasks, int n_tasks, const ofdg_blueprint* bps,
                       int n_bps, hipStream_t st, ofdg_ctx::Stage& stage, bool shared) {
  if (!c->pool.p && !c->pool_mixed) { c->err = "Could not open texture collection (no texture pool)"; return OFDG_ETEXTURES; }
  OFDG_TRY(finalise_pool(c));
  OFDG_TRY(ensure_tex_table(c));
  RealizeConfig cfg{c->prm.width, c->prm.height, c->prm.mode, c->pool_n, c->pool_w, c->pool_h, c->prm.background_prep};
  cfg.pool_addr = (uint64_t)(uintptr_t)c->pool.p;
  cfg.tex_table = c->pool_mixed && c->prm.background_prep ? c->tex_table.data() : nullptr;
  cfg.fg_stride = c->fg_src.stride; cfg.fg_origin = c->fg_src.origin; cfg.bg_stride = c->bg_src.stride; cfg.bg_origin = c->bg_src.origin;
  if (stage.pending) {
    if (hipEventQuery(stage.free_ev) != hipSuccess) HIP_OK(c, hipEventSynchronize(stage.free_ev));
    stage.pending = false;
  }
  if (sl.compose_pending && sl.compose_stream != st) {
    HIP_OK(c, hipStreamWaitEvent(st, sl.compose_event, 0));
    sl.compose_pending = false;
  }
  sl.res_samples = 0;
  OFDG_TRY(realize_batch(cfg, tasks, n_tasks, bps, n_bps, &sl.batch, &c->err, &c->crop_server));
  const RealizedBatch& B = sl.batch;
  const size_t n_shapes = B.shapes.size(), n_obj = B.objects.size();
  const size_t b_shapes = (n_shapes * sizeof(DevShape) + 255) & ~(size_t)255, b_obj = (n_obj * sizeof(DevObject) + 255) & ~(size_t)255,
               b_smp = ((size_t)n_tasks * sizeof(DevSample) + 255) & ~(size_t)255,
               b_prep = c->prm.background_prep ? B.bgprep.size() * sizeof(DevBgPrep) : 0;
  const size_t need = b_shapes + b_obj + b_smp + b_prep + 64;
  if (need > sl.d_rec.cap) {
    HIP_OK(c, hipDeviceSynchronize());
    HIP_OK(c, sl.d_rec.reserve(need));
  }
  HIP_OK(c, sl.d_shapes.alias((DevShape*)sl.d_rec.p, n_shapes));
  HIP_OK(c, sl.d_objects.alias((DevObject*)(sl.d_rec.p + b_shapes), n_obj));
  HIP_OK(c, sl.d_samples.alias((DevSample*)(sl.d_rec.p + b_shapes + b_obj), (size_t)n_tasks));
  if (b_prep) HIP_OK(c, sl.d_bgprep.alias((DevBgPrep*)(sl.d_rec.p + b_shapes + b_obj + b_smp), B.bgprep.size()));
  OFDG_TRY(size_slot(c, sl, n_tasks, n_shapes));
  if (need > stage.h.bytes) HIP_OK(c, stage.h.alloc(need * 2, hipHostMallocDefault));
  char* hs = (char*)stage.h.p;
  if (n_shapes) std::memcpy(hs, B.shapes.data(), n_shapes * sizeof(DevShape));
  std::memcpy(hs + b_shapes, B.objects.data(), n_obj * sizeof(DevObject));
  std::memcpy(hs + b_shapes + b_obj, B.samples.data(), (size_t)n_tasks * sizeof(DevSample));
  if (b_prep) std::memcpy(hs + b_shapes + b_obj + b_smp, B.bgprep.data(), b_prep);
  HIP_OK(c, hipMemcpyAsync(sl.d_rec.p, hs, b_shapes + b_obj + b_smp + b_prep, hipMemcpyHostToDevice, st));
  if (!B.crops.empty()) {
    const int W = c->prm.width, H = c->prm.height;
    const size_t crop_floats = (size_t)4 * (W + 1) * (H + 1), bg_floats = (size_t)4 * 2 * W * 2 * H;
    size_t n_bg = 0;
    for (const CropUse& u : B.crops) n_bg += u.background ? 1 : 0;
    HIP_OK(c, sl.d_croptab.reserve(B.crops.size()));
    if (n_bg) {
      HIP_OK(c, sl.d_bgwarp.reserve(n_bg * bg_floats));
      HIP_OK(c, sl.d_bgwarp_max.reserve(n_bg));
      HIP_OK(c, hipMemsetAsync(sl.d_bgwarp_max.p, 0, n_bg * sizeof(unsigned), st));
      OFDG_TRY(ensure_resize_tables(c));
    }
    std::vector<DevCropRef> tab(B.crops.size());
    size_t bg_at = 0;
    for (size_t k = 0; k < B.crops.size(); ++k) {
      const float* src = c->d_warp.p + (size_t)B.crops[k].crop * crop_floats;
      if (B.crops[k].background) {
        OFDG_TRY(upscale_crop(c, src, sl.d_bgwarp.p + bg_at * bg_floats, sl.d_bgwarp_max.p + bg_at, st, &tab[k]));
        ++bg_at;
      } else {
        tab[k] = make_crop_ref(src, c->d_warp_max.p + B.crops[k].crop, W + 1, H + 1);
      }
    }
    HIP_OK(c, hipMemcpyAsync(sl.d_croptab.p, tab.data(), tab.size() * sizeof(DevCropRef), hipMemcpyHostToDevice, st));
    HIP_OK(c, hipStreamSynchronize(st));
  }
  if (c->prm.background_prep) {
    if (shared) {
      if (c->word_reserved != c->ticket) { HIP_OK(c, take_err_word(c, c->ticket, st)); c->word_reserved = c->ticket; }
      OFDG_TRY(prepare_backgrounds(c, sl, n_tasks, true, st, err_word(c, c->ticket)));
      sl.bgprep_pending = false;
    } else {
      sl.bgprep_pending = true;
    }
  }
  HIP_OK(c, hipEventRecord(stage.free_ev, st));
  stage.pending = true;
  if (shared) {
    if (!sl.ev_uploaded.e) HIP_OK(c, sl.ev_uploaded.create(hipEventDisableTiming));
    HIP_OK(c, hipEventRecord(sl.ev_uploaded, st));
    sl.upload_pending = true;
    sl.upload_stream = st;
  } else {
    sl.upload_pending = false;
  }
  sl.res_samples = n_tasks;
  sl.res_shapes = (int)n_shapes;
  sl.res_objects = (int)n_obj;
  return OFDG_OK;
}

static int render_impl(ofdg_ctx* c, const ofdg_task* tasks, int n_tasks, const ofdg_blueprint* bps, int n_bps, const CallOut& o, void* stream) {
  stream = own_stream(c, stream);
  ofdg_ctx::Chain& ch = take_chain(c);
  OFDG_TRY(upload_slot(c, ch.slot, tasks, n_tasks, bps, n_bps, chain_stream(c, ch, (hipStream_t)stream), ch.stage, false));
  return launch_resident(c, ch, ch.slot, o, (hipStream_t)stream);
}
static bool render_args_ok(const ofdg_ctx* c, const ofdg_task* tasks, int n_tasks, const ofdg_blueprint* bps, const void* d_img0,
                           const void* d_img1, const void* d_flow) {
  return c && tasks && bps && n_tasks >= 1 && d_img0 && d_img1 && d_flow;
}
int ofdg_render(ofdg_ctx* c, const ofdg_task* tasks, int n_tasks, const ofdg_blueprint* bps, int n_bps,
                float* d_img0, float* d_img1, float* d_flow, void* stream) {
  CallOut o;
  OFDG_TRY(check_call(c, "ofdg_render", render_args_ok(c, tasks, n_tasks, bps, d_img0, d_img1, d_flow),
                      d_img0, d_img1, d_flow, nullptr, nullptr, nullptr, &o));
  return render_impl(c, tasks, n_tasks, bps, n_bps, o, stream);
}
int ofdg_render_ex(ofdg_ctx* c, const ofdg_task* tasks, int n_tasks, const ofdg_blueprint* bps, int n_bps,
                   float* d_img0, float* d_img1, float* d_flow, const ofdg_extras* ex, void* stream) {
  CallOut o;
  OFDG_TRY(check_call(c, "ofdg_render_ex", render_args_ok(c, tasks, n_tasks, bps, d_img0, d_img1, d_flow),
                      d_img0, d_img1, d_flow, ex, nullptr, nullptr, &o, "ofdg_render"));
  return render_impl(c, tasks, n_tasks, bps, n_bps, o, stream);
}
int ofdg_render_fmt(ofdg_ctx* c, const ofdg_task* tasks, int n_tasks, const ofdg_blueprint* bps, int n_bps,
                    void* d_img0, void* d_img1, void* d_flow, const ofdg_out_format* fmt, void* stream) {
  CallOut o;
  OFDG_TRY(check_call(c, "ofdg_render_fmt", render_args_ok(c, tasks, n_tasks, bps, d_img0, d_img1, d_flow),
                      d_img0, d_img1, d_flow, nullptr, nullptr, fmt, &o));
  return render_impl(c, tasks, n_tasks, bps, n_bps, o, stream);
}
int ofdg_render_ex_fmt(ofdg_ctx* c, const ofdg_task* tasks, int n_tasks, const ofdg_blueprint* bps, int n_bps,
                       void* d_img0, void* d_img1, void* d_flow, const ofdg_extras_fmt* ex, const ofdg_out_format* fmt, void* stream) {
  CallOut o;
  OFDG_TRY(check_call(c, "ofdg_render_ex_fmt", render_args_ok(c, tasks, n_tasks, bps, d_img0, d_img1, d_flow),
                      d_img0, d_img1, d_flow, nullptr, ex, fmt, &o));
  return render_impl(c, tasks, n_tasks, bps, n_bps, o, stream);
}

int ofdg_upload_slot(ofdg_ctx* c, int slot, const ofdg_task* tasks, int n_tasks, const ofdg_blueprint* bps, int n_bps,
                     void* stream) {
  if (!c || !tasks || !bps || n_tasks < 1 || slot < 0 || slot >= ofdg_ctx::kUserSlots) return invalid_argument(c, "ofdg_upload_slot");
  return upload_slot(c, c->slots[slot], tasks, n_tasks, bps, n_bps, (hipStream_t)stream, c->user_stage, true);
}

int ofdg_render_slot(ofdg_ctx* c, int slot, float* d_img0, float* d_img1, float* d_flow, void* stream) {
  if (!c || !d_img0 || !d_img1 || !d_flow || slot < 0 || slot >= ofdg_ctx::kUserSlots) return invalid_argument(c, "ofdg_render_slot");
  if (c->slots[slot].res_samples <= 0) { c->err = "ofdg_render_slot: no batch is resident in this slot"; return OFDG_EINVAL; }
  stream = own_stream(c, stream);
  return launch_resident(c, take_chain(c), c->slots[slot], CallOut{"ofdg_render_slot", d_img0, d_img1, d_flow, {}, 0}, (hipStream_t)stream);
}

int ofdg_render_resident(ofdg_ctx* c, float* d_img0, float* d_img1, float* d_flow, void* stream) {
  if (!c || !d_img0 || !d_img1 || !d_flow) return invalid_argument(c, "ofdg_render_resident");
  if (!c->last_slot || c->last_slot->res_samples <= 0) { c->err = "ofdg_render_resident: nothing has been rendered yet"; return OFDG_EINVAL; }
  stream = own_stream(c, stream);
  for (int k = 0; k < c->n_chains; ++k)
    if (&c->chains[k].slot == c->last_slot && !c->last_slot->compose_pending) HIP_OK(c, hipStreamSynchronize(c->chains[k].stream));
  return launch_resident(c, take_chain(c), *c->last_slot, CallOut{"ofdg_render_resident", d_img0, d_img1, d_flow, {}, 0}, (hipStream_t)stream);
}

static_assert(sizeof(ofdg_object_row) == sizeof(DevObjectRow) && sizeof(ofdg_object_row) == 96 && offsetof(ofdg_object_row, area0) == 8 &&
              offsetof(ofdg_object_row, area0) == offsetof(DevObjectRow, area) && offsetof(ofdg_object_row, box0) == 16 &&
              offsetof(ofdg_object_row, box0) == offsetof(DevObjectRow, box) && offsetof(ofdg_object_row, box1) == 32 &&
              offsetof(ofdg_object_row, motion) == 48 && offsetof(ofdg_object_row, motion) == offsetof(DevObjectRow, motion),
              "ofdg_object_row: 96 bytes without padding, the layout the kernels write");
static_assert(OFDG_MAX_OBJECT_ROWS == kObjectRows, "background + kMaxFgObjects");
int ofdg_object_table(ofdg_ctx* c, const uint8_t* d_label0, const uint8_t* d_label1, ofdg_object_row* d_rows, int rows_per_sample,
                      int32_t* d_counts, void* stream) {
  if (!c) return OFDG_EINVAL;
  auto fail = [&](const std::string& why) { c->err = "ofdg_object_table: " + why; return OFDG_EINVAL; };
  if (c->prm.mode == 9) return fail("the table restates the label planes, which are defined for the rigid modes only (mode 9)");
  if (!d_rows) return fail("d_rows is NULL");
  if (!d_counts) return fail("d_counts is NULL");
  if (rows_per_sample < 1) return fail("rows_per_sample = " + std::to_string(rows_per_sample) + " (valid: >= 1)");
  if (((uintptr_t)d_rows & 7) || ((uintptr_t)d_counts & 3) || ((uintptr_t)d_label0 & 3) || ((uintptr_t)d_label1 & 3))
    return fail("d_rows must be 8-byte aligned, d_counts and the label planes 4-byte aligned");
  if (!c->last_slot || !c->last_ch || c->last_slot->res_samples <= 0)
    return fail("no render / forward call has been made yet on this context");
  ofdg_ctx::Slot& sl = *c->last_slot;
  ofdg_ctx::Chain& ch = *c->last_ch;
  const hipStream_t S = c->last_stream;
  const hipStream_t st = stream == OFDG_STREAM_OWN ? S : (hipStream_t)stream;
  const int W = c->prm.width, H = c->prm.height, n = sl.res_samples;
  const bool tracked = st != S || &sl != &ch.slot;
  const hipEvent_t done = tracked ? ch.ev_done.e : nullptr;
  const bool reduce = d_label0 || d_label1;
  DevObjectRow* const rows = reinterpret_cast<DevObjectRow*>(d_rows);
  const long long cells = (long long)n * rows_per_sample;
  hipExtLaunchKernelGGL(object_table_header_kernel, dim3((unsigned)((cells + 255) / 256)), dim3(256), 0, st, nullptr, reduce ? nullptr : done, 0,
                        sl.d_samples.p, sl.d_objects.p, sl.d_shapes.p, n, rows_per_sample, W, H, rows, d_counts);
  HIP_OK(c, hipGetLastError());
  if (reduce) {
    hipExtLaunchKernelGGL(object_table_reduce_kernel, dim3((unsigned)((H + kTabBand - 1) / kTabBand), 2, (unsigned)n), dim3(64 * kTabWaves), 0,
                          st, nullptr, done, 0, sl.d_samples.p, d_label0, d_label1, W, H, rows_per_sample, rows);
    HIP_OK(c, hipGetLastError());
  }
  if (tracked) track_completion(sl, ch, st, done);
  return OFDG_OK;
}

static_assert(sizeof(ofdg_flow_stats_row) == sizeof(DevFlowStatsRow) && OFDG_FLOW_HIST_BINS == kFlowHistBins &&
              offsetof(ofdg_flow_stats_row, n_counted) == offsetof(DevFlowStatsRow, count) &&
              offsetof(ofdg_flow_stats_row, sum_u_q8) == offsetof(DevFlowStatsRow, sum_q8) &&
              offsetof(ofdg_flow_stats_row, max_key) == offsetof(DevFlowStatsRow, max_key) && offsetof(ofdg_flow_stats_row, max_key) == 296,
              "ofdg_flow_stats_row: 304 bytes without padding, the layout the kernel adds to");
static_assert(OFDG_FMT_F32 == 0 && OFDG_FMT_U8 == 1 && OFDG_FMT_F16 == 2 && OFDG_STATS_ACCUMULATE == 1 && OFDG_STATS_VISIBLE_ONLY == 2 &&
              OFDG_STATS_ONE_ROW == 4, "flow_stats_arg_error spells these codes out");
static int flow_stats_on(ofdg_ctx* c, const char* who, int W, int H, const void* d_flow, int flow_fmt, const void* d_occ, int occ_fmt,
                         int n_samples, float bin_px, int flags, ofdg_flow_stats_row* d_rows, void* stream) {
  auto fail = [&](const std::string& why) { c->err = std::string(who) + ": " + why; return OFDG_EINVAL; };
  if (const char* why = flow_stats_arg_error(d_flow, flow_fmt, d_occ, occ_fmt, n_samples, W, H, bin_px, flags, d_rows)) return fail(why);
  const bool half = flow_fmt == OFDG_FMT_F16;
  if ((uintptr_t)d_flow & (half ? 7 : 15)) return fail(half ? "d_flow must be 8-byte aligned (binary16)" : "d_flow must be 16-byte aligned (float32)");
  if (d_occ && ((uintptr_t)d_occ & (occ_fmt == OFDG_FMT_U8 ? 3 : 15)))
    return fail(occ_fmt == OFDG_FMT_U8 ? "d_occ must be 4-byte aligned (uint8)" : "d_occ must be 16-byte aligned (float32)");
  if (stream == OFDG_STREAM_OWN && !c->last_ch) return fail("stream: OFDG_STREAM_OWN before any render / forward call on this context");
  const hipStream_t st = stream == OFDG_STREAM_OWN ? c->last_stream : (hipStream_t)stream;
  const bool one_row = flags & OFDG_STATS_ONE_ROW;
  if (!(flags & OFDG_STATS_ACCUMULATE))
    HIP_OK(c, hipMemsetAsync(d_rows, 0, sizeof(ofdg_flow_stats_row) * (one_row ? 1 : (size_t)n_samples), st));
  const uint32_t plane_quads = (uint32_t)((size_t)W * H / 4);
  const dim3 grid((plane_quads + kStatsQuads - 1) / kStatsQuads, (unsigned)std::min(n_samples, 65535));
  const int kind = (half ? 3 : 0) + (d_occ ? (occ_fmt == OFDG_FMT_U8 ? 2 : 1) : 0);
  DevFlowStatsRow* const rows = reinterpret_cast<DevFlowStatsRow*>(d_rows);
  const float inv_bin = 1.0f / bin_px;
  const int vis = (flags & OFDG_STATS_VISIBLE_ONLY) ? 1 : 0, one = one_row ? 1 : 0;
#define OFDG_STATS_LAUNCH(HALF, OCC)                                                                                               \
  hipLaunchKernelGGL((flow_stats_kernel<HALF, OCC>), grid, dim3(kStatsThreads), 0, st, d_flow, d_occ, n_samples, plane_quads, bin_px, \
                     inv_bin, vis, one, rows)
  switch (kind) {
    case 0: OFDG_STATS_LAUNCH(false, 0); break;
    case 1: OFDG_STATS_LAUNCH(false, 1); break;
    case 2: OFDG_STATS_LAUNCH(false, 2); break;
    case 3: OFDG_STATS_LAUNCH(true, 0); break;
    case 4: OFDG_STATS_LAUNCH(true, 1); break;
    default: OFDG_STATS_LAUNCH(true, 2); break;
  }
#undef OFDG_STATS_LAUNCH
  HIP_OK(c, hipGetLastError());
  return OFDG_OK;
}
int ofdg_flow_stats(ofdg_ctx* c, const void* d_flow, int flow_fmt, const void* d_occ, int occ_fmt, int n_samples, float bin_px,
                    int flags, ofdg_flow_stats_row* d_rows, void* stream) {
  if (!c) return OFDG_EINVAL;
  return flow_stats_on(c, "ofdg_flow_stats", c->prm.width, c->prm.height, d_flow, flow_fmt, d_occ, occ_fmt, n_samples, bin_px, flags, d_rows, stream);
}
int ofdg_flow_stats_sized(ofdg_ctx* c, const void* d_flow, int flow_fmt, const void* d_occ, int occ_fmt, int n_samples, int width, int height,
                          float bin_px, int flags, ofdg_flow_stats_row* d_rows, void* stream) {
  if (!c) return OFDG_EINVAL;
  if (const char* why = plane_size_error(width, height)) { c->err = std::string("ofdg_flow_stats_sized: ") + why; return OFDG_EINVAL; }
  return flow_stats_on(c, "ofdg_flow_stats_sized", width, height, d_flow, flow_fmt, d_occ, occ_fmt, n_samples, bin_px, flags, d_rows, stream);
}

static_assert(sizeof(struct ofdg_flow_pyramid) == sizeof(DevFlowPyramid) && OFDG_PYR_MAX_LEVELS == kPyrMaxLevels &&
              offsetof(struct ofdg_flow_pyramid, weight) == offsetof(DevFlowPyramid, weight) &&
              offsetof(struct ofdg_flow_pyramid, levels) == offsetof(DevFlowPyramid, levels) &&
              offsetof(struct ofdg_flow_pyramid, out_fmt) == offsetof(DevFlowPyramid, out_fmt) && OFDG_PYR_SCALE == 1,
              "struct ofdg_flow_pyramid: the layout the kernel takes; flow_pyramid_arg_error spells the flag out");
static int flow_pyramid_on(ofdg_ctx* c, const char* who, int W, int H, const void* d_flow, int flow_fmt, const void* d_occ, int occ_fmt,
                           int n_samples, int flags, const struct ofdg_flow_pyramid* pyr, void* stream) {
  auto fail = [&](const std::string& why) { c->err = std::string(who) + ": " + why; return OFDG_EINVAL; };
  const DevFlowPyramid* const out = reinterpret_cast<const DevFlowPyramid*>(pyr);
  if (const char* why = flow_pyramid_arg_error(d_flow, flow_fmt, d_occ, occ_fmt, n_samples, W, H, flags, out)) return fail(why);
  const bool half = flow_fmt == OFDG_FMT_F16, half_out = pyr->out_fmt == OFDG_FMT_F16;
  if ((uintptr_t)d_flow & (half ? 7 : 15)) return fail(half ? "d_flow must be 8-byte aligned (binary16)" : "d_flow must be 16-byte aligned (float32)");
  if (d_occ && ((uintptr_t)d_occ & (occ_fmt == OFDG_FMT_U8 ? 3 : 15)))
    return fail(occ_fmt == OFDG_FMT_U8 ? "d_occ must be 4-byte aligned (uint8)" : "d_occ must be 16-byte aligned (float32)");
  if (stream == OFDG_STREAM_OWN && !c->last_ch) return fail("stream: OFDG_STREAM_OWN before any render / forward call on this context");
  const hipStream_t st = stream == OFDG_STREAM_OWN ? c->last_stream : (hipStream_t)stream;
  DevFlowPyramid arg = *out;
  for (int k = arg.levels; k < kPyrMaxLevels; ++k) arg.flow[k] = arg.weight[k] = nullptr;
  const dim3 grid((unsigned)((W + kPyrTile - 1) / kPyrTile), (unsigned)((H + kPyrTile - 1) / kPyrTile), (unsigned)std::min(n_samples, 65535));
  const int kind = (half ? 6 : 0) + (half_out ? 3 : 0) + (d_occ ? (occ_fmt == OFDG_FMT_U8 ? 2 : 1) : 0);
  const int scaled = (flags & OFDG_PYR_SCALE) ? 1 : 0, n_weights = arg.weight[0] ? 1 : 0;
#define OFDG_PYR_LAUNCH(HALF, HALF_OUT, OCC)                                                                                          \
  hipLaunchKernelGGL((flow_pyramid_kernel<HALF, HALF_OUT, OCC>), grid, dim3(kPyrThreads), 0, st, d_flow, d_occ, n_samples, W, H, scaled, \
                     n_weights, arg)
// ... 4 lines not shown
    case 3: OFDG_PYR_LAUNCH(false, true, 0); break;
    case 4: OFDG_PYR_LAUNCH(false, true, 1); break;
    case 5: OFDG_PYR_LAUNCH(false, true, 2); break;
    case 6: OFDG_PYR_LAUNCH(true, false, 0); break;
    case 7: OFDG_PYR_LAUNCH(true, false, 1); break;
    case 8: OFDG_PYR_LAUNCH(true, false, 2); break;
    case 9: OFDG_PYR_LAUNCH(true, true, 0); break;
    case 10: OFDG_PYR_LAUNCH(true, true, 1); break;
    default: OFDG_PYR_LAUNCH(true, true, 2); break;
  }
#undef OFDG_PYR_LAUNCH
  HIP_OK(c, hipGetLastError());
  return OFDG_OK;
}
int ofdg_flow_pyramid(ofdg_ctx* c, const void* d_flow, int flow_fmt, const void* d_occ, int occ_fmt, int n_samples, int flags,
                      const struct ofdg_flow_pyramid* pyr, void* stream) {
  if (!c) return OFDG_EINVAL;
  return flow_pyramid_on(c, "ofdg_flow_pyramid", c->prm.width, c->prm.height, d_flow, flow_fmt, d_occ, occ_fmt, n_samples, flags, pyr, stream);
}
int ofdg_flow_pyramid_sized(ofdg_ctx* c, const void* d_flow, int flow_fmt, const void* d_occ, int occ_fmt, int n_samples, int width, int height,
                            int flags, const struct ofdg_flow_pyramid* pyr, void* stream) {
  if (!c) return OFDG_EINVAL;
  if (const char* why = plane_size_error(width, height)) { c->err = std::string("ofdg_flow_pyramid_sized: ") + why; return OFDG_EINVAL; }
  return flow_pyramid_on(c, "ofdg_flow_pyramid_sized", width, height, d_flow, flow_fmt, d_occ, occ_fmt, n_samples, flags, pyr, stream);
}

static_assert(sizeof(ofdg_crop_rec) == sizeof(DevCropRec) && sizeof(struct ofdg_crop_job) == sizeof(DevCropJob) && OFDG_CROP_PLANES == kCropPlanes &&
              offsetof(struct ofdg_crop_job, dst) == offsetof(DevCropJob, dst) && offsetof(struct ofdg_crop_job, recs) == offsetof(DevCropJob, recs) &&
              offsetof(struct ofdg_crop_job, recs_out) == offsetof(DevCropJob, recs_out) &&
              offsetof(struct ofdg_crop_job, first_index) == offsetof(DevCropJob, first_index) &&
              offsetof(struct ofdg_crop_job, seed) == offsetof(DevCropJob, seed) && offsetof(struct ofdg_crop_job, crop_w) == offsetof(DevCropJob, crop_w) &&
              offsetof(struct ofdg_crop_job, occ_fmt) == offsetof(DevCropJob, occ_fmt) && offsetof(struct ofdg_crop_job, reserved) == 180,
              "struct ofdg_crop_job: the layout the kernel takes");
static_assert(OFDG_CROP_HFLIP == 1 && OFDG_CROP_VFLIP == 2 && OFDG_CROP_RANDOM_HFLIP == 4 && OFDG_CROP_RANDOM_VFLIP == 8 && OFDG_CROP_OCC_WINDOW == 16 &&
              OFDG_CROP_FLOW == 2 && OFDG_CROP_OCC0 == 4 && OFDG_CROP_LABEL0 == 6, "crop_arg_error and crop_kernel spell these codes out");
int ofdg_crop(ofdg_ctx* c, const struct ofdg_crop_job* job, int n_samples, void* stream) {
  if (!c) return OFDG_EINVAL;
  auto fail = [&](const std::string& why) { c->err = "ofdg_crop: " + why; return OFDG_EINVAL; };
  const int W = c->prm.width, H = c->prm.height;
  const DevCropJob* const j = reinterpret_cast<const DevCropJob*>(job);
  if (const char* why = crop_arg_error(j, n_samples, W, H)) return fail(why);
  static const char* const kPlane[kCropPlanes] = {"image0", "image1", "flow", "flow1", "occ0", "occ1", "label0", "label1"};
  for (int k = 0; k < kCropPlanes; ++k) {
    if (!j->src[k]) continue;
    const int es = crop_elem_bytes(*j, k), need = es == 4 ? 16 : es == 2 ? 8 : 4;
    if ((uintptr_t)j->src[k] & (uintptr_t)(need - 1))
      return fail(std::string("src[") + kPlane[k] + "] must be " + std::to_string(need) + "-byte aligned");
    if ((uintptr_t)j->dst[k] & 15) return fail(std::string("dst[") + kPlane[k] + "] must be 16-byte aligned");
  }
  if ((uintptr_t)j->recs & 15) return fail("recs must be 16-byte aligned");
  if ((uintptr_t)j->recs_out & 15) return fail("recs_out must be 16-byte aligned");
  if (stream == OFDG_STREAM_OWN && !c->last_ch) return fail("stream: OFDG_STREAM_OWN before any render / forward call on this context");
  const hipStream_t st = stream == OFDG_STREAM_OWN ? c->last_stream : (hipStream_t)stream;
  DevCropGrid grid;
  uint32_t blocks = 0;
  for (int k = 0, slot = 0; k < kCropPlanes; ++k) {
    const uint32_t pieces = (uint32_t)((size_t)j->crop_w * j->crop_h * crop_elem_bytes(*j, k) / 16);
    const uint32_t per_channel = j->src[k] ? (pieces + kCropThreads * kCropPerLane - 1) / (kCropThreads * kCropPerLane) : 0u;
    for (int ch = 0; ch < crop_channels(k); ++ch, ++slot) {
      grid.first_block[slot] = blocks;
      blocks += per_channel;
    }
  }
  grid.first_block[kCropSlots] = blocks;
  const dim3 g(blocks, (unsigned)std::min(n_samples, 65535));
  const int kind = (j->image_fmt == OFDG_FMT_U8 ? 4 : 0) + (j->flow_fmt == OFDG_FMT_F16 ? 2 : 0) + (j->occ_fmt == OFDG_FMT_U8 ? 1 : 0);
#define OFDG_CROP_LAUNCH(IMAGE_U8, FLOW_HALF, OCC_U8) \
  hipLaunchKernelGGL((crop_kernel<IMAGE_U8, FLOW_HALF, OCC_U8>), g, dim3(kCropThreads), 0, st, *j, grid, n_samples, W, H)
  switch (kind) {
    case 0: OFDG_CROP_LAUNCH(false, false, false); break;
    case 1: OFDG_CROP_LAUNCH(false, false, true); break;
    case 2: OFDG_CROP_LAUNCH(false, true, false); break;
    case 3: OFDG_CROP_LAUNCH(false, true, true); break;
    case 4: OFDG_CROP_LAUNCH(true, false, false); break;
    case 5: OFDG_CROP_LAUNCH(true, false, true); break;
    case 6: OFDG_CROP_LAUNCH(true, true, false); break;
    default: OFDG_CROP_LAUNCH(true, true, true); break;
  }
#undef OFDG_CROP_LAUNCH
  HIP_OK(c, hipGetLastError());
  return OFDG_OK;
}

static int prepare_counter_slot(ofdg_ctx* c, ofdg_ctx::Slot& sl, int n) {
  if (c->prm.mode == 9) OFDG_TRY(ensure_counter_croptab(c));
  OFDG_TRY(finalise_pool(c));
  OFDG_TRY(ensure_tex_table(c));
  if (!c->pool.p && !c->pool_mixed) { c->err = "Could not open texture collection (no texture pool)"; return OFDG_ETEXTURES; }
  if (n < 1 || n > 512) { c->err = "counter sampler: batch must be 1..512 samples"; return OFDG_EINVAL; }
  const int max_objects = c->prm.num_objects > 0 ? std::min(c->prm.num_objects, kCsMaxObjects) : 24;
  const size_t shapes_cap = (size_t)n * (size_t)(c->prm.mode >= 6 ? max_objects * 7 : max_objects);
  const size_t n_obj = (size_t)n * (1 + kCsMaxObjects);
  OFDG_TRY(size_slot(c, sl, n, shapes_cap, n_obj));
  sl.res_samples = n;
  sl.res_shapes = (int)shapes_cap;
  sl.res_objects = (int)n_obj;
  sl.batch.samples.clear();
  return OFDG_OK;
}

static int forward_counter_impl(ofdg_ctx* c, long long first_index, int n_samples, const CallOut& o, void* stream) {
  stream = own_stream(c, stream);
  const int k = (int)(c->next_chain % (unsigned)c->n_chains);
  ofdg_ctx::Chain& ch = take_chain(c);
  hipStream_t st = (hipStream_t)stream;
  auto prepare_on = [&](ofdg_ctx::Chain& cj, long long first, hipStream_t s_, bool hand_over) -> int {
    if (cj.prep.valid && cj.prep.slot == &cj.slot && cj.prep.first_index == first && cj.prep.n == n_samples) return OFDG_OK;
    OFDG_TRY(prepare_counter_slot(c, cj.slot, n_samples));
    return launch_prepare(c, cj, cj.slot, s_, first, hand_over);
  };
  OFDG_TRY(prepare_on(ch, first_index, st, chain_stream(c, ch, st) != st));
  OFDG_TRY(launch_compose(c, ch, o, st));
  const long long prev_first = c->last_first;
  c->last_first = first_index;
  if (c->overlap && c->lookahead > 0) {
    const long long stride = (prev_first >= 0 && first_index > prev_first) ? first_index - prev_first
                                                                             : (long long)n_samples * std::max(1, c->prm.world_size);
    for (int d = 1; d <= std::min(c->lookahead, c->n_chains - 1); ++d) {
      ofdg_ctx::Chain& cj = c->chains[(k + d) % c->n_chains];
      if (prepare_on(cj, first_index + (long long)d * stride, cj.stream, true) != OFDG_OK) { (void)discard_prepared(c, cj); break; }
      cj.prep.ahead = true;
    }
  }
  return OFDG_OK;
}

static bool forward_counter_args_ok(const ofdg_ctx* c, long long first_index, const void* d_img0, const void* d_img1, const void* d_flow) {
  return c && d_img0 && d_img1 && d_flow && first_index >= 0;
}
int ofdg_forward_counter(ofdg_ctx* c, long long first_index, int n_samples, float* d_img0, float* d_img1, float* d_flow,
                         void* stream) {
  CallOut o;
  OFDG_TRY(check_call(c, "ofdg_forward_counter", forward_counter_args_ok(c, first_index, d_img0, d_img1, d_flow),
                      d_img0, d_img1, d_flow, nullptr, nullptr, nullptr, &o));
  return forward_counter_impl(c, first_index, n_samples, o, stream);
}
int ofdg_forward_counter_ex(ofdg_ctx* c, long long first_index, int n_samples, float* d_img0, float* d_img1, float* d_flow,
                            const ofdg_extras* ex, void* stream) {
  CallOut o;
  OFDG_TRY(check_call(c, "ofdg_forward_counter_ex", forward_counter_args_ok(c, first_index, d_img0, d_img1, d_flow),
                      d_img0, d_img1, d_flow, ex, nullptr, nullptr, &o));
  return forward_counter_impl(c, first_index, n_samples, o, stream);
}
int ofdg_forward_counter_fmt(ofdg_ctx* c, long long first_index, int n_samples, void* d_img0, void* d_img1, void* d_flow,
                             const ofdg_out_format* fmt, void* stream) {
  CallOut o;
  OFDG_TRY(check_call(c, "ofdg_forward_counter_fmt", forward_counter_args_ok(c, first_index, d_img0, d_img1, d_flow),
                      d_img0, d_img1, d_flow, nullptr, nullptr, fmt, &o));
  return forward_counter_impl(c, first_index, n_samples, o, stream);
}
int ofdg_forward_counter_ex_fmt(ofdg_ctx* c, long long first_index, int n_samples, void* d_img0, void* d_img1, void* d_flow,
                                const ofdg_extras_fmt* ex, const ofdg_out_format* fmt, void* stream) {
  CallOut o;
  OFDG_TRY(check_call(c, "ofdg_forward_counter_ex_fmt", forward_counter_args_ok(c, first_index, d_img0, d_img1, d_flow),
                      d_img0, d_img1, d_flow, nullptr, ex, fmt, &o));
  return forward_counter_impl(c, first_index, n_samples, o, stream);
}

int ofdg_num_chains(const ofdg_ctx* c) { return c ? c->n_chains : OFDG_EINVAL; }
void* ofdg_stream(ofdg_ctx* c) {
  if (!c) return nullptr;
  return (void*)c->chains[c->next_chain % (unsigned)c->n_chains].stream.s;
}

int ofdg_sample_counter(ofdg_ctx* c, long long first_index, int n_samples, ofdg_task* tasks, ofdg_blueprint* bps) {
  if (!c || !tasks || !bps || n_samples < 1 || first_index < 0) return OFDG_EINVAL;
  HIP_OK(c, hipDeviceSynchronize());
  HIP_OK(c, c->d_cs_bps.reserve((size_t)n_samples * kCsBlueprintsPerSample));
  HIP_OK(c, c->d_cs_nobj.reserve(n_samples));
  hipLaunchKernelGGL(cs_sample_kernel, dim3(n_samples * kCsGroups), dim3(64), 0, 0, c->cs_mode, first_index, n_samples,
                     c->prm.mode == 9 ? c->crop_server.n_crops : 0, c->d_cs_bps.p,
                     c->d_cs_nobj.p);
  HIP_OK(c, hipGetLastError());
  std::vector<int> nobj(n_samples);
  HIP_OK(c, hipMemcpy(bps, c->d_cs_bps.p, (size_t)n_samples * kCsBlueprintsPerSample * sizeof(ofdg_blueprint), hipMemcpyDeviceToHost));
  HIP_OK(c, hipMemcpy(nobj.data(), c->d_cs_nobj.p, n_samples * sizeof(int), hipMemcpyDeviceToHost));
  for (int s = 0; s < n_samples; ++s) {
    tasks[s].background = s * kCsBlueprintsPerSample;
    tasks[s].first_object = s * kCsBlueprintsPerSample + 1;
    tasks[s].n_objects = nobj[s];
    tasks[s].reserved = 0;
  }
  return OFDG_OK;
}

long long ofdg_shard_first_index(long long step, int batch, int world_size, int rank) {
  if (step < 0 || batch < 1 || world_size < 1 || rank < 0 || rank >= world_size) return -1;
  return step * (long long)batch * world_size + (long long)rank * batch;
}

static int forward_impl(ofdg_ctx* c, const CallOut& o, void* stream) {
  const int B = c->prm.batch_size, world = c->prm.world_size, rank = c->prm.rank;
  if (B < 1 || rank < 0 || rank >= world) { c->err = "ofdg_forward: bad batch_size / rank"; return OFDG_EINVAL; }
  const bool outputs = o.img0 && o.img1 && o.flow;
  int rc = OFDG_EINVAL;
  if (c->prm.sampler == OFDG_SAMPLER_COUNTER) {
    const long long first = ofdg_shard_first_index(c->step, B, world, rank);
    if (!outputs || first < 0) return invalid_argument(c, o.fn);
    rc = forward_counter_impl(c, first, B, o, stream);
    if (rc == OFDG_OK) c->step++;
    return rc;
  }
  c->fw_bps.clear();
  c->fw_tasks.assign((size_t)B * world, ofdg_task());
  for (int i = 0; i < B * world; ++i) OFDG_TRY(c->sampler->next_task(&c->fw_bps, &c->fw_tasks[i], &c->err));
  if (!outputs) c->err = "ofdg_render: invalid argument";
  else rc = render_impl(c, c->fw_tasks.data() + (size_t)rank * B, B, c->fw_bps.data(), (int)c->fw_bps.size(), o, stream);
  if (rc == OFDG_OK) c->step++;
  else ofdg_set_step(c, c->step);
  return rc;
}
int ofdg_forward(ofdg_ctx* c, float* d_img0, float* d_img1, float* d_flow, void* stream) {
  CallOut o;
  OFDG_TRY(check_call(c, "ofdg_forward", c != nullptr, d_img0, d_img1, d_flow, nullptr, nullptr, nullptr, &o));
  return forward_impl(c, o, stream);
}
int ofdg_forward_ex(ofdg_ctx* c, float* d_img0, float* d_img1, float* d_flow, const ofdg_extras* ex, void* stream) {
  CallOut o;
  OFDG_TRY(check_call(c, "ofdg_forward_ex", c != nullptr, d_img0, d_img1, d_flow, ex, nullptr, nullptr, &o));
  return forward_impl(c, o, stream);
}
int ofdg_forward_fmt(ofdg_ctx* c, void* d_img0, void* d_img1, void* d_flow, const ofdg_out_format* fmt, void* stream) {
  CallOut o;
  OFDG_TRY(check_call(c, "ofdg_forward_fmt", c != nullptr, d_img0, d_img1, d_flow, nullptr, nullptr, fmt, &o));
  return forward_impl(c, o, stream);
}
int ofdg_forward_ex_fmt(ofdg_ctx* c, void* d_img0, void* d_img1, void* d_flow, const ofdg_extras_fmt* ex, const ofdg_out_format* fmt,
                        void* stream) {
  CallOut o;
  OFDG_TRY(check_call(c, "ofdg_forward_ex_fmt", c != nullptr, d_img0, d_img1, d_flow, nullptr, ex, fmt, &o));
  return forward_impl(c, o, stream);
}

long long ofdg_get_step(const ofdg_ctx* c) { return c ? c->step : -1; }
int ofdg_set_step(ofdg_ctx* c, long long step) {
  if (!c || step < 0) return OFDG_EINVAL;
  if (c->prm.sampler != OFDG_SAMPLER_COUNTER) {
    const long long n = step * (long long)std::max(c->prm.batch_size, 1) * c->prm.world_size;
    c->sampler.reset(new RefSampler(c->prm.mode, c->prm.width, c->prm.height, c->prm.num_objects));
    std::vector<ofdg_blueprint> bps;
    ofdg_task t;
    const int B = std::max(c->prm.batch_size, 1), world = c->prm.world_size, rank = c->prm.rank;
    const bool crops = c->prm.mode == 9 && c->crop_server.n_crops > 0;
    if (crops) { c->crop_server.head = 0; c->crop_server.counter = 0; }
    for (long long i = 0; i < n; ++i) {
      bps.clear();
      OFDG_TRY(c->sampler->next_task(&bps, &t, &c->err));
      if (crops && (i / B) % world == rank) {
        if (bps[t.background].do_warpfield_deformation) (void)c->crop_server.get();
        for (int k = 0; k < t.n_objects; ++k)
          if (bps[t.first_object + k].do_warpfield_deformation) (void)c->crop_server.get();
      }
    }
  }
  c->step = step;
  return OFDG_OK;
}

int ofdg_synchronize(ofdg_ctx* c, void* stream) {
  if (!c) return OFDG_EINVAL;
  if (stream == OFDG_STREAM_OWN) stream = nullptr;
  HIP_OK(c, hipStreamSynchronize((hipStream_t)stream));
  for (int k = 0; k < c->n_chains; ++k) {
    HIP_OK(c, hipStreamSynchronize(c->chains[k].stream));
    if (c->chains[k].done_pending) HIP_OK(c, hipEventSynchronize(c->chains[k].ev_done));
  }
  uint32_t words[ofdg_ctx::kErrWords];
  HIP_OK(c, hipMemcpy(words, c->d_err.p, sizeof(words), hipMemcpyDeviceToHost));
  uint32_t e = 0;
  long long first_bad = -1;
  for (int i = 0; i < ofdg_ctx::kErrWords; ++i)
    if (words[i]) {
      e |= words[i];
      const long long q = c->ticket - 1 - ((c->ticket - 1 - i) % ofdg_ctx::kErrWords + ofdg_ctx::kErrWords) % ofdg_ctx::kErrWords;
      if (first_bad < 0 || q < first_bad) first_bad = q;
    }
  if (e) HIP_OK(c, hipMemset(c->d_err.p, 0, sizeof(words)));
  if (c->word_reserved < 0) std::fill(c->word_clean, c->word_clean + ofdg_ctx::kErrWords, true);
  if (e) {
    c->err = err_text(e) + " (first in batch " + std::to_string(first_bad) + " of this context, or one " + std::to_string(ofdg_ctx::kErrWords) + " calls earlier)";
    return OFDG_ECAPACITY;
  }
  return OFDG_OK;
}

static int poll_words(ofdg_ctx* c, int first, int n, uint32_t* flags) {
  if (!c->h_err.p) HIP_OK(c, c->h_err.alloc(sizeof(uint32_t), hipHostMallocMapped));
  if (!c->err_stream.s) HIP_OK(c, c->err_stream.create(hipStreamNonBlocking));
  uint32_t* h_dev = nullptr;
  HIP_OK(c, hipHostGetDevicePointer((void**)&h_dev, c->h_err.p, 0));
  hipLaunchKernelGGL(err_exchange_kernel, dim3(1), dim3(64), 0, c->err_stream, c->d_err.p + first, n, h_dev);
  HIP_OK(c, hipGetLastError());
  HIP_OK(c, hipStreamSynchronize(c->err_stream));
  *flags = *(const uint32_t*)c->h_err.p;
  return OFDG_OK;
}
int ofdg_poll_errors(ofdg_ctx* c) {
  if (!c) return OFDG_EINVAL;
  uint32_t e = 0;
  OFDG_TRY(poll_words(c, 0, ofdg_ctx::kErrWords, &e));
  if (e) { c->err = err_text(e); return OFDG_ECAPACITY; }
  return OFDG_OK;
}

long long ofdg_last_ticket(const ofdg_ctx* c) { return c ? c->last_ticket : -1; }
int ofdg_poll_errors_of(ofdg_ctx* c, long long ticket) {
  if (!c) return OFDG_EINVAL;
  if (ticket < 0 || ticket >= c->ticket || ticket + ofdg_ctx::kErrWords <= c->ticket) { c->err = "ofdg_poll_errors_of: no such batch (tickets of the last " + std::to_string(ofdg_ctx::kErrWords) + " calls are kept)"; return OFDG_EINVAL; }
  uint32_t e = 0;
  c->asked_by_ticket = true;
  OFDG_TRY(poll_words(c, (int)(ticket % ofdg_ctx::kErrWords), 1, &e));
  c->word_clean[(size_t)(ticket % ofdg_ctx::kErrWords)] = true;
  if (e) { c->err = "batch " + std::to_string(ticket) + ": " + err_text(e); return OFDG_ECAPACITY; }
  return OFDG_OK;
}

static int warp_alloc(ofdg_ctx* c, int n_crops) {
  const size_t crop_floats = (size_t)4 * (c->prm.width + 1) * (c->prm.height + 1);
  HIP_OK(c, hipDeviceSynchronize());
  drop_counter_croptab(c);
  HIP_OK(c, c->d_warp.alloc((size_t)n_crops * crop_floats));
  HIP_OK(c, c->d_warp_max.alloc((size_t)n_crops));
  HIP_OK(c, hipMemset(c->d_warp_max.p, 0, (size_t)n_crops * sizeof(unsigned)));
  c->crop_server = CropServer();
  c->crop_server.n_crops = n_crops;
  return OFDG_OK;
}

int ofdg_warp_generate(ofdg_ctx* c, int n_fields, uint32_t seed) {
  if (!c || n_fields < 1) return OFDG_EINVAL;
  OFDG_TRY(discard_all_prepared(c));
  const int W = c->prm.width, H = c->prm.height;
  const int S = std::max(W, H) * 3;
  std::vector<std::pair<int, int>> org;
  for (int y = H / 4; y < S - 5 * H / 4; y += H / 3)
    for (int x = W / 4; x < S - 5 * W / 4; x += W / 3) org.push_back({x, y});
  if (org.empty()) { c->err = "frame too small for warp crops"; return OFDG_EINVAL; }
  OFDG_TRY(warp_alloc(c, n_fields * (int)org.size()));
// ... 136 lines not shown
}

int ofdg_debug_rasterize_path(ofdg_ctx* c, const double* xy, const int* types, int n, uint8_t* coverage_host) {
  if (!c || !xy || !types || !coverage_host || n < 1 || n > 64) return OFDG_EINVAL;
  OFDG_TRY(discard_all_prepared(c));
  HIP_OK(c, hipDeviceSynchronize());
  DevBuf<double> d_xy;
  DevBuf<int> d_ty, d_n;
  DevBuf<int2> d_v;
  HIP_OK(c, d_xy.alloc(2 * (size_t)n));
  HIP_OK(c, d_ty.alloc(n));
  HIP_OK(c, d_v.alloc(kMaxVerts));
  HIP_OK(c, d_n.alloc(1));
  HIP_OK(c, hipMemcpy(d_xy.p, xy, sizeof(double) * 2 * n, hipMemcpyHostToDevice));
  HIP_OK(c, hipMemcpy(d_ty.p, types, sizeof(int) * n, hipMemcpyHostToDevice));
  HIP_OK(c, hipMemset(d_v.p, 0, sizeof(int2) * kMaxVerts));
  uint32_t* const dbg_err = c->d_err.p + ofdg_ctx::kErrWords;
  hipLaunchKernelGGL(debug_path_kernel, dim3(1), dim3(64), 0, 0, d_xy.p, d_ty.p, n, d_v.p, d_n.p, dbg_err);
  HIP_OK(c, hipGetLastError());
  uint32_t dbg_flags = 0;
  HIP_OK(c, hipMemcpy(&dbg_flags, dbg_err, sizeof(uint32_t), hipMemcpyDeviceToHost));
  if (dbg_flags) HIP_OK(c, hipMemset(dbg_err, 0, sizeof(uint32_t)));
  std::vector<int2> v(kMaxVerts);
  int nv = 0;
  HIP_OK(c, hipMemcpy(v.data(), d_v.p, sizeof(int2) * kMaxVerts, hipMemcpyDeviceToHost));
  HIP_OK(c, hipMemcpy(&nv, d_n.p, sizeof(int), hipMemcpyDeviceToHost));
  if (dbg_flags) { c->err = "debug_rasterize_path: " + err_text(dbg_flags); return OFDG_ECAPACITY; }
  if (nv < 1 || nv > kMaxVerts) { c->err = "debug_rasterize_path: the flattened outline has " + std::to_string(nv) + " vertices"; return OFDG_ECAPACITY; }
  return debug_rasterize_verts(c, v, nv, coverage_host);
}

int ofdg_debug_dda_rows(ofdg_ctx* c, const double* inv, int rows, int len, int* out_xy) {
  if (!c || !inv || !out_xy || rows < 1 || len < 1 || (size_t)rows * len > (1u << 24)) return OFDG_EINVAL;
  DevBuf<int2> d;
  HIP_OK(c, d.alloc((size_t)rows * len));
  const Mat m{inv[0], inv[1], inv[2], inv[3], inv[4], inv[5]};
  hipLaunchKernelGGL(debug_dda_kernel, dim3((rows * len + 255) / 256), dim3(256), 0, 0, m, rows, len, d.p);
  HIP_OK(c, hipGetLastError());
  HIP_OK(c, hipMemcpy(out_xy, d.p, sizeof(int2) * (size_t)rows * len, hipMemcpyDeviceToHost));
  return OFDG_OK;
}

int ofdg_debug_num_shapes(ofdg_ctx* c, int sample) {
  if (!c || !c->last_slot) return OFDG_EINVAL;
  const ofdg_ctx::Slot& sl = *c->last_slot;
  if (sl.res_samples <= 0 || sample < 0 || sample >= (int)sl.batch.samples.size()) return OFDG_EINVAL;
  return sl.batch.samples[sample].n_shapes;
}

int ofdg_debug_coverage(ofdg_ctx* c, int sample, int shape, int frame, uint8_t* coverage_host) {
  if (!c || !coverage_host || frame < 0 || frame > 1 || !c->last_slot || c->last_slot->res_samples <= 0) return OFDG_EINVAL;
  const ofdg_ctx::Slot& sl = *c->last_slot;
  if (sample < 0 || sample >= (int)sl.batch.samples.size()) return OFDG_EINVAL;
  const DevSample& s = sl.batch.samples[sample];
  if (shape < 0 || shape >= s.n_shapes) return OFDG_EINVAL;
  const int W = c->prm.width, H = c->prm.height;
  const size_t sf = (size_t)(s.first_shape + shape) * 2 + frame;
  HIP_OK(c, hipDeviceSynchronize());
  DevShapeFrame f;
  HIP_OK(c, hipMemcpy(&f, sl.d_frames.p + sf, sizeof(f), hipMemcpyDeviceToHost));
  std::vector<uint8_t> tmp((size_t)W * H);
  HIP_OK(c, hipMemcpy(tmp.data(), c->chains[c->last_chain].cov.p + sf * W * H, tmp.size(), hipMemcpyDeviceToHost));
  std::memset(coverage_host, 0, tmp.size());
  for (int y = f.y0; y <= f.y1; ++y)
    for (int x = f.x0; x <= f.x1; ++x) coverage_host[(size_t)y * W + x] = tmp[(size_t)y * W + x];
  return OFDG_OK;
}

int ofdg_debug_item_count(ofdg_ctx* c) {
  if (!c || !c->last_slot || !c->last_slot->d_item_count.p) return OFDG_EINVAL;
  int n = 0;
  if (hipDeviceSynchronize() != hipSuccess) return OFDG_EHIP;
  if (hipMemcpy(&n, c->last_slot->d_item_count.p, sizeof(int), hipMemcpyDeviceToHost) != hipSuccess) return OFDG_EHIP;
  return n;
}

int ofdg_debug_bgprep_tiles(ofdg_ctx* c, int* tiles, int* workgroups) {
  if (!c || !tiles || !workgroups || !c->last_slot) return OFDG_EINVAL;
  const ofdg_ctx::Slot& sl = *c->last_slot;
  *tiles = 0; *workgroups = kPrepGrid;
  int cap_cw, cap_ch;
  bool fusable;
  bgprep_caps(c, &cap_cw, &cap_ch, &fusable);
  const int n = sl.res_samples;
  if (c->prm.background_prep != 1 || !fusable || n > kPrepMaxSamples || n < 1 || !sl.d_bgprep.p) return OFDG_OK;
  HIP_OK(c, hipDeviceSynchronize());
  std::vector<DevBgPrep> rec((size_t)n);
  HIP_OK(c, hipMemcpy(rec.data(), sl.d_bgprep.p, rec.size() * sizeof(DevBgPrep), hipMemcpyDeviceToHost));
  for (const DevBgPrep& q : rec)
    if (prep_sample_fits(q, cap_cw, cap_ch)) *tiles += prep_tile_cols(q) * prep_tile_rows(q);
  return OFDG_OK;
}

int ofdg_debug_bgprep_paths(ofdg_ctx* c, unsigned* counts9) {
  if (!c || !counts9) return OFDG_EINVAL;
  HIP_OK(c, hipDeviceSynchronize());
  if (!c->d_prep_paths.p) {
    HIP_OK(c, c->d_prep_paths.alloc(9));
    HIP_OK(c, hipMemset(c->d_prep_paths.p, 0, 9 * sizeof(uint32_t)));
  }
  HIP_OK(c, hipMemcpy(counts9, c->d_prep_paths.p, 9 * sizeof(uint32_t), hipMemcpyDeviceToHost));
  HIP_OK(c, hipMemset(c->d_prep_paths.p, 0, 9 * sizeof(uint32_t)));
  return OFDG_OK;
}

int ofdg_set_profiling(ofdg_ctx* c, int mode) {
  if (!c || mode < 0 || mode > 2) return OFDG_EINVAL;
  HIP_OK(c, hipDeviceSynchronize());
  OFDG_TRY(discard_all_prepared(c));
  HIP_OK(c, hipDeviceSynchronize());
  c->profiling = mode;
  c->ev_count = 0; c->ev_alloc = 0;
  c->launch_count = 0;
  c->ev_stride = (mode == 1) ? 4 : 1;
  if (mode && c->ev.empty()) {
    c->ev_sets = 256;
    c->ev.resize((size_t)c->ev_sets * 6);
    for (auto& e : c->ev) HIP_OK(c, e.create(hipEventDefault));
  }
  c->ev_composed.assign((size_t)c->ev_sets, 0);
  c->ev_bgprep.assign((size_t)c->ev_sets, 0);
  return OFDG_OK;
}

int ofdg_kernel_ms(ofdg_ctx* c, const char* kernel, float* ms) {
  if (!c || !kernel || !ms) return OFDG_EINVAL;
  int i = -1;
  if (!std::strcmp(kernel, "geom")) i = 0;
  else if (!std::strcmp(kernel, "raster")) i = 1;
  else if (!std::strcmp(kernel, "compose")) i = 2;
  else if (!std::strcmp(kernel, "background_prep")) i = 3;
  if (i < 0) { c->err = "unknown kernel name"; return OFDG_EINVAL; }
  if (!c->profiling || c->ev_count == 0 || (i < 2 && c->profiling != 2)) {
    c->err = "no profiled launch of that kernel yet (ofdg_set_profiling)";
    return OFDG_EINVAL;
  }
  int n = 0;
  double acc = 0;
  for (int k = 0; k < c->ev_sets; ++k) {
    if (!c->ev_composed[(size_t)k]) continue;
    if (i == 3 && !c->ev_bgprep[(size_t)k]) continue;
    ++n;
    const Event* ev = &c->ev[(size_t)k * 6];
    HIP_OK(c, hipEventSynchronize(ev[5]));
    float t = 0;
    if (i == 3) {
      HIP_OK(c, hipEventElapsedTime(&t, ev[3], ev[c->profiling == 2 ? 2 : 4]));
      acc += t;
      continue;
    }
    HIP_OK(c, hipEventElapsedTime(&t, ev[i == 0 ? 0 : (i == 2 ? 4 : 1)], ev[2 * i + 1]));
    acc += t;
  }
  if (n == 0) { c->err = "no profiled launch of that kernel yet (ofdg_set_profiling)"; return OFDG_EINVAL; }
  *ms = (float)(acc / n);
  return OFDG_OK;
}

int ofdg_debug_tables(ofdg_ctx* c, uint8_t* add_tbl, uint8_t* sub_tbl, uint8_t* aa_tbl, uint8_t* blend_tbl, int s_fixed) {
  if (!c) return OFDG_EINVAL;
  DevBuf<uint8_t> buf;
  HIP_OK(c, buf.alloc(3 * 65536 + 256));
  uint8_t* const d = buf.p;
  hipLaunchKernelGGL(tables_kernel, dim3(256), dim3(256), 0, 0, d, d + 65536, d + 3 * 65536, d + 2 * 65536, s_fixed);
  HIP_OK(c, hipGetLastError());
  HIP_OK(c, hipMemcpy(add_tbl, d, 65536, hipMemcpyDeviceToHost));
  HIP_OK(c, hipMemcpy(sub_tbl, d + 65536, 65536, hipMemcpyDeviceToHost));
  HIP_OK(c, hipMemcpy(blend_tbl, d + 2 * 65536, 65536, hipMemcpyDeviceToHost));
  HIP_OK(c, hipMemcpy(aa_tbl, d + 3 * 65536, 256, hipMemcpyDeviceToHost));
  return OFDG_OK;
}

int ofdg_debug_detmath(ofdg_ctx* c, const double* angles, int n, double* sin_out, double* cos_out, const float* x, int m, float* expf_out) {
  if (!c || n < 0 || m < 0 || (n > 0 && (!angles || !sin_out || !cos_out)) || (m > 0 && (!x || !expf_out))) return OFDG_EINVAL;
  DevBuf<double> dbuf;
  DevBuf<float> fbuf;
  const int k = std::max(std::max(n, m), 1);
  HIP_OK(c, dbuf.alloc((size_t)3 * k));
  HIP_OK(c, fbuf.alloc((size_t)2 * k));
  double* const d = dbuf.p;
  float* const f = fbuf.p;
  if (n) HIP_OK(c, hipMemcpy(d, angles, (size_t)n * sizeof(double), hipMemcpyHostToDevice));
  if (m) HIP_OK(c, hipMemcpy(f, x, (size_t)m * sizeof(float), hipMemcpyHostToDevice));
  hipLaunchKernelGGL(detmath_kernel, dim3((k + 255) / 256), dim3(256), 0, 0, d, n, d + k, d + 2 * k, f, m, f + k);
  HIP_OK(c, hipGetLastError());
  if (n) {
    HIP_OK(c, hipMemcpy(sin_out, d + k, (size_t)n * sizeof(double), hipMemcpyDeviceToHost));
    HIP_OK(c, hipMemcpy(cos_out, d + 2 * k, (size_t)n * sizeof(double), hipMemcpyDeviceToHost));
  }
  if (m) HIP_OK(c, hipMemcpy(expf_out, f + k, (size_t)m * sizeof(float), hipMemcpyDeviceToHost));
  return OFDG_OK;
}

}
```

### optical-flow-2d-data-generation_amd/csrc/ofdg_device.h

```cpp
#pragma once
#include <math.h>
#include <stdint.h>

namespace ofdg {

constexpr int kMaxSegments = 20;
constexpr int kMaxComponents = 8;
constexpr int kMaxVerts = 1024;
constexpr int kCurveMaxPts = 96;
constexpr int kCurveMaxDepth = 16;
constexpr int kBandRows = 8;
constexpr int kMaxFgObjects = 64;
constexpr int kRasterGrid = 512;

constexpr uint32_t kErrVertCapacity = 1u;
constexpr uint32_t kErrCurveCapacity = 2u;
constexpr uint32_t kErrDxLimit = 4u;
constexpr uint32_t kErrBgPrepCapacity = 8u;

struct Mat {
  double sx, shy, shx, sy, tx, ty;
};

struct DevShape {
  Mat m[2];
  float seg_x[kMaxSegments];
  float seg_y[kMaxSegments];
  int32_t seg_type[kMaxSegments];
  float rx, ry;
  int32_t type;
  int32_t n_seg;
  int32_t sample;
  int32_t deform;
  int32_t object;
  int32_t obj_local;
};

struct DevShapeFrame {
  int32_t n_verts;
  int32_t x0, y0, x1, y1;
  int32_t pad[3];
};

struct DevObject {
  Mat motion;
  Mat tex_inv;
  uint64_t tex_base;
  int32_t first_shape;
  int32_t n_shapes;
  uint32_t additive;
  int32_t kind;
  int32_t id;
  int32_t deform;
  int32_t pad[2];
};
static_assert(sizeof(DevObject) == 136, "record layout is read dword-wise by compose");

struct DevSample {
  int32_t first_object;
  int32_t n_objects;
  int32_t first_shape;
  int32_t n_shapes;
  Mat bg_motion;
  Mat bg_tex_inv;
  uint64_t bg_tex_base;
  int32_t bg_deform;
  int32_t pad;
  uint16_t shape_of[kMaxFgObjects];
};
static_assert(sizeof(DevSample) == 256, "compose reads the sample record as 128 + 128 bytes");
constexpr uint16_t kShapeComposite = 0x8000u;

struct DevObjectHdr {
  uint64_t tex_base;
  int32_t first_shape, n_shapes;
  uint32_t additive;
  int32_t kind, id, deform;
};

struct DevObjectRow {
  int32_t obj_id, obj_type;
  int32_t area[2];
  int32_t box[2][4];
  double motion[6];
};
static_assert(sizeof(DevObjectRow) == 96, "ofdg_object_row is 96 bytes without padding");
constexpr int kObjectRows = kMaxFgObjects + 1;

constexpr int kFlowHistBins = 64;
struct DevFlowStatsRow {
  uint32_t hist[kFlowHistBins];
  uint32_t count[4];
  unsigned long long sum_q8[3];
  unsigned long long max_key;
};
static_assert(sizeof(DevFlowStatsRow) == 304, "ofdg_flow_stats_row is 304 bytes without padding");
// ... 204 lines not shown
```

### optical-flow-2d-data-generation_amd/csrc/sampler_counter.hip

```cpp
#pragma once
#include <hip/hip_runtime.h>
#include <stdint.h>

#include "../../include/ofdg.h"
#include "../../include/ofdg_detmath.h"
#include "ofdg_device.h"
#include "realize.h"
#include "sampler_ref.h"

namespace ofdg {

constexpr int kCsMaxObjects = 32;
constexpr int kCsParts = 8;
constexpr int kCsBlueprintsPerSample = 1 + kCsMaxObjects * (1 + 7);

__device__ __forceinline__ uint4 philox4x32(uint4 ctr, uint2 key) {
  const uint32_t M0 = 0xD2511F53u, M1 = 0xCD9E8D57u, W0 = 0x9E3779B9u, W1 = 0xBB67AE85u;
#pragma unroll
  for (int r = 0; r < 10; ++r) {
    const unsigned long long p0 = (unsigned long long)M0 * ctr.x, p1 = (unsigned long long)M1 * ctr.z;
    const uint32_t hi0 = (uint32_t)(p0 >> 32), lo0 = (uint32_t)p0;
    const uint32_t hi1 = (uint32_t)(p1 >> 32), lo1 = (uint32_t)p1;
    ctr = make_uint4(hi1 ^ ctr.y ^ key.x, lo1, hi0 ^ ctr.w ^ key.y, lo0);
    key.x += W0; key.y += W1;
// ... 357 lines not shown
      ob.tex_base = (unsigned long long)(bg.tex_id % D.pool_n) * D.bg_stride + bg_origin;
      if (D.background_prep) {
        const int ti = bg.tex_id % D.pool_n;
        int ipw = D.pool_w, iph = D.pool_h;
        unsigned long long iaddr = D.pool_addr + (unsigned long long)ti * img_texels * 4ull;
        if (D.tex_table) { const DevTexEntry e = D.tex_table[ti]; ipw = e.w; iph = e.h; iaddr = e.addr; }
        double sa, ca;
        ofdg_det_sincos((double)bg_prep_rad(bg.tex_rot), &sa, &ca);
        DevBgPrep bp = make_bg_prep(ipw, iph, W, H, (float)ca, (float)sa, bg.tex_scale, bg.tex_shift_x, bg.tex_shift_y, iaddr);
        const bool bg_deforms = bg.do_warpfield_deformation && D.n_crops > 0;
        if (!bg_deforms || D.crops) {
          double grow = 0.;
          if (bg_deforms) grow = ceil((double)__uint_as_float(*D.crops[D.n_crops + cs_crop_of(key, kCsSampleCtx, D.n_crops)].max_bits)) + 2.;
          bg_prep_region(ob.tex_inv, W, H, grow, &bp);
        }
        bgprep[s] = bp;
        ob.tex_base = (unsigned long long)s * 4ull * (unsigned long long)W * (unsigned long long)H;
      }
      ob.id = bg.obj_id;
      if (bg.do_warpfield_deformation && D.n_crops > 0) ob.deform = 1 + D.n_crops + cs_crop_of(key, kCsSampleCtx, D.n_crops);
      objects[obj_base] = ob;
      DevSample* sp = samples + s;
      sp->bg_motion = ob.motion; sp->bg_tex_inv = ob.tex_inv; sp->bg_tex_base = ob.tex_base; sp->bg_deform = ob.deform; sp->pad = 0;
    }
  }
  CsLane L;
  cs_generate(M, key, n_obj, group, S, L);
  if (tid == 0) {
    int acc = 0;
    for (int o = 0; o < kCsMaxObjects; ++o) { const int c = S.cnt[o]; S.cnt[o] = acc; acc += c; }
    S.n_items = acc;
    if (group == 0) {
      if (acc > D.shape_stride) atomicOr(err, kErrVertCapacity);
      DevSample* sp = samples + s;
      sp->first_object = obj_base; sp->n_objects = 1 + n_obj;
      sp->first_shape = s * D.shape_stride; sp->n_shapes = min(acc, D.shape_stride);
    }
  }
  __syncthreads();
  for (int i = S.n_items + group * 64 + tid; i < D.shape_stride; i += 64 * kCsGroups) { sh_base[i].type = 0; sh_base[i].n_seg = 0; sh_base[i].deform = 0; }
  if (L.type == 0) return;
  const Mat bgm = s_bgm;
  const Mat intr = mat_mul(mat_rotation_det((double)L.init_rot), mat_translation((double)L.init_tx, (double)L.init_ty));
  Mat mot = mat_mul(mat_mul(mat_rotation_det((double)L.rot), mat_scaling((double)L.scale)), mat_translation((double)L.tx, (double)L.ty));
  mot = mat_mul(mot, mat_mul(mat_mul(mat_translation(-W / 2., -H / 2.), bgm), mat_translation(W / 2., H / 2.)));
  const bool composite = (part == 0 && L.type == OFDG_OBJ_COMPOSITE);
  const int n_sh = composite ? L.n_comp : 1;
  const int first = S.cnt[object];
  const int off = first + (part > 0 ? part - 1 : 0);
  const bool fits = first + (part == 0 ? n_sh : part) <= D.shape_stride;
  if (part == 0) {
    DevObject ob = DevObject();
    ob.motion = mot;
    ob.tex_inv = mat_invert(mot);
    ob.tex_base = (unsigned long long)(L.tex_id % D.pool_n) * D.fg_stride + fg_origin;
    ob.first_shape = s * D.shape_stride + first;
    ob.n_shapes = fits ? n_sh : 0;
    ob.additive = S.additive[tid >> 3];
    ob.kind = (composite || !fits) ? 2 : 1;
    ob.id = object + 10;
    if (L.deform && D.n_crops > 0) ob.deform = 1 + cs_crop_of(key, object, D.n_crops);
    objects[obj_base + 1 + object] = ob;
    samples[s].shape_of[object] = (uint16_t)(first | (ob.kind == 2 ? kShapeComposite : 0));
  }
  if (!composite && fits) {
    DevShape* sh = sh_base + off;
    sh->m[0] = intr;
    sh->m[1] = mat_mul(intr, mot);
    for (int i = 0; i < L.spokes; ++i) { sh->seg_x[i] = S.seg_x[i][tid]; sh->seg_y[i] = S.seg_y[i][tid]; }
    if (L.spokes > 0) cs_segment_types(S.trig[tid], L.spokes, sh->seg_type);
    sh->rx = L.rx; sh->ry = L.ry;
    sh->type = L.type;
    sh->n_seg = L.spokes;
    sh->sample = s;
    sh->deform = (L.deform && D.n_crops > 0) ? 1 + cs_crop_of(key, object, D.n_crops) : 0;
    sh->object = obj_base + 1 + object;
    sh->obj_local = object;
  }
}

__global__ __launch_bounds__(64) void cs_sample_realize_kernel(CsMode M, CsRealizeDims D, long long first_index,
                                                               DevShape* __restrict__ shapes, DevObject* __restrict__ objects,
                                                               DevSample* __restrict__ samples, uint32_t* __restrict__ err,
                                                               DevBgPrep* __restrict__ bgprep) {
  __shared__ CsShared S;
  __shared__ Mat s_bgm;
  __builtin_amdgcn_s_setprio(3);
  cs_sample_realize_block(S, s_bgm, (int)blockIdx.x, M, D, first_index, shapes, objects, samples, err, bgprep);
}

}
```

Baseline: 355,900.

## Batch two future front-end preparations into one paired geometry/raster launch

Adds a 'front_batches' mode, on by default at 2. Each chain runs the sampler, geometry and raster kernels once for two batches: the current one and the one it will serve n_chains calls later. Only the current half's background prep runs immediately. The second half reuses the stored geometry, launches only its background prep, and composes over a sample/box offset view. This amortises launch overhead and small-grid underutilisation of the front-end kernels through a larger raster grid. In exchange it adds complex bookkeeping for error words, discard paths and profiling events, with a risk of stale halves when indices don't follow the expected stride.

```diff
diff --git a/include/ofdg.h b/include/ofdg.h
--- a/include/ofdg.h
+++ b/include/ofdg.h
@@ -236,6 +236,7 @@
 
 void* ofdg_stream(ofdg_ctx* ctx);
 int ofdg_num_chains(const ofdg_ctx* ctx);
+int ofdg_set_front_batches(ofdg_ctx* ctx, int n);
 
 int ofdg_synchronize(ofdg_ctx* ctx, void* stream);
 
diff --git a/optical-flow-2d-data-generation_amd/__init__.py b/optical-flow-2d-data-generation_amd/__init__.py
--- a/optical-flow-2d-data-generation_amd/__init__.py
+++ b/optical-flow-2d-data-generation_amd/__init__.py
@@ -81,7 +81,7 @@
     "ofdg_forward_counter", "ofdg_sample_counter", "ofdg_warp_generate", "ofdg_warp_upload", "ofdg_warp_info", "ofdg_warp_download", "ofdg_host_displacers",
     "ofdg_host_sampler_create", "ofdg_host_sampler_next", "ofdg_host_sampler_destroy", "ofdg_host_realize",
     "ofdg_parse_prototxt", "ofdg_host_last_error", "ofdg_host_decode_image", "ofdg_layer_create", "ofdg_layer_forward", "ofdg_layer_destroy",
-    "ofdg_layer_in_flight", "ofdg_poll_errors", "ofdg_poll_errors_of", "ofdg_last_ticket", "ofdg_num_chains",
+    "ofdg_layer_in_flight", "ofdg_poll_errors", "ofdg_poll_errors_of", "ofdg_last_ticket", "ofdg_num_chains", "ofdg_set_front_batches",
     "ofdg_comm_unique_id", "ofdg_comm_init", "ofdg_comm_adopt", "ofdg_comm_destroy", "ofdg_comm_rank", "ofdg_comm_world_size",
     "ofdg_comm_last_error", "ofdg_comm_bcast_setup", "ofdg_comm_bcast_abort", "ofdg_comm_nccl_count", "ofdg_comm_bcast_pool", "ofdg_comm_agree", "ofdg_setup_of", "ofdg_setup_params",
     "ofdg_setup_alloc_pool", "ofdg_pool_device_mixed", "ofdg_pool_device_image", "ofdg_layer_create_dist",
@@ -487,6 +487,7 @@
         L.ofdg_last_ticket.argtypes = [vp]
         L.ofdg_last_ticket.restype = C.c_longlong
         L.ofdg_num_chains.argtypes = [vp]
+        L.ofdg_set_front_batches.argtypes = [vp, i32]
         L.ofdg_comm_unique_id.argtypes = [vp]
         L.ofdg_comm_init.argtypes = [vp, i32, i32, i32, C.POINTER(vp)]
         L.ofdg_comm_adopt.argtypes = [vp, i32, i32, i32, C.POINTER(vp)]
@@ -768,6 +769,9 @@
 
     def num_chains(self):
         return lib().ofdg_num_chains(self.h)
+
+    def set_front_batches(self, n):
+        self._check(lib().ofdg_set_front_batches(self.h, int(n)))
 
     def next_stream(self):
         return int(lib().ofdg_stream(self.h) or 0)
diff --git a/optical-flow-2d-data-generation_amd/csrc/kernels.hip b/optical-flow-2d-data-generation_amd/csrc/kernels.hip
--- a/optical-flow-2d-data-generation_amd/csrc/kernels.hip
+++ b/optical-flow-2d-data-generation_amd/csrc/kernels.hip
@@ -252,12 +252,12 @@
                                                    DevShapeFrame* __restrict__ frames, int2* __restrict__ verts,
                                                    unsigned long long* __restrict__ blockmask, uint32_t* __restrict__ err,
                                                    int* __restrict__ item_count, int4* __restrict__ items,
-                                                   const DevCropRef* __restrict__ crops) {
+                                                   const DevCropRef* __restrict__ crops, int split_sf, uint32_t* __restrict__ err2) {
   __shared__ GeomWs s_ws[kGeomWaves];
   step_kernel_priority();
   const int wave = threadIdx.x >> 6, lane = threadIdx.x & 63;
   const int sf = __builtin_amdgcn_readfirstlane(blockIdx.x * kGeomWaves + wave);
-  geom_wave(s_ws[wave], sf, lane, shapes, n_shapes, cs_tab, W, H, frames, verts, blockmask, err, item_count, items, crops);
+  geom_wave(s_ws[wave], sf, lane, shapes, n_shapes, cs_tab, W, H, frames, verts, blockmask, sf >= split_sf ? err2 : err, item_count, items, crops);
 }
 
 struct CellAcc {
diff --git a/optical-flow-2d-data-generation_amd/csrc/ofdg_api.hip b/optical-flow-2d-data-generation_amd/csrc/ofdg_api.hip
--- a/optical-flow-2d-data-generation_amd/csrc/ofdg_api.hip
+++ b/optical-flow-2d-data-generation_amd/csrc/ofdg_api.hip
@@ -108,16 +108,21 @@
       hipStream_t stream = nullptr;
       long long ticket = -1;
       bool ahead = false;
+      int base = 0;
     } prep;
+    Prepared half;
   };
   static constexpr int kMaxChains = 8;
   Chain chains[kMaxChains];
   int lookahead = 0;
+  int front_batches = 2;
+  std::string info_head;
   long long last_first = -1;
   int n_chains = 3;
   unsigned next_chain = 0;
   int last_chain = 0;
   Slot* last_slot = nullptr;
+  int last_base = 0, last_n = 0;
   Chain* last_ch = nullptr;
   hipStream_t last_stream = nullptr;
   hipStream_t last_user_st = nullptr;
@@ -157,6 +162,7 @@
   long long ev_count = 0, ev_alloc = 0, launch_count = 0;
   std::vector<char> ev_composed;
   std::vector<char> ev_bgprep;
+  std::vector<char> ev_front;
   std::vector<ofdg_task> fw_tasks;
   std::vector<ofdg_blueprint> fw_bps;
 };
@@ -259,12 +265,13 @@
   c->overlap = params->serial == 0;
   c->lookahead = std::max(params->lookahead, 0);
   c->n_chains = params->chains > 0 ? std::min(params->chains, (int)ofdg_ctx::kMaxChains) : (g_hw_queues_env >= 8 ? 4 : 3);
-  c->info = "chains=" + std::to_string(c->n_chains) +
+  c->info_head = "chains=" + std::to_string(c->n_chains) +
             (params->chains > 0 ? " (ofdg_params.chains)"
              : g_hw_queues_env >= 8 ? " (GPU_MAX_HW_QUEUES=" + std::to_string(g_hw_queues_env) + ": one hardware queue per chain)"
              : g_hw_queues_env > 0 ? " (GPU_MAX_HW_QUEUES=" + std::to_string(g_hw_queues_env) + " < 8: start the process with GPU_MAX_HW_QUEUES=8 for four chains, +5-8 %)"
                                    : " (GPU_MAX_HW_QUEUES was not set when the library was loaded: HIP's default of 4 hardware queues; start the process with GPU_MAX_HW_QUEUES=8 for four chains, +5-8 %)") +
             " lookahead=" + std::to_string(c->lookahead) + (c->overlap ? "" : " serial");
+  c->info = c->info_head + " front=" + std::to_string(c->front_batches);
   for (int i = 0; i < c->n_chains; ++i) {
     ofdg_ctx::Chain& ch = c->chains[i];
     if ((e = ch.stream.create(hipStreamNonBlocking)) != hipSuccess ||
@@ -700,15 +707,17 @@
   return ensure_item_count(c, sl);
 }
 
-static int prepare_backgrounds(ofdg_ctx* c, ofdg_ctx::Slot& sl, int n, bool records_resident, hipStream_t s, uint32_t* err, hipEvent_t stop = nullptr);
-static int launch_counter_sampler(ofdg_ctx* c, ofdg_ctx::Slot& sl, long long first_index, hipStream_t s, uint32_t* err) {
+static int prepare_backgrounds(ofdg_ctx* c, ofdg_ctx::Slot& sl, int n, bool records_resident, hipStream_t s, uint32_t* err, hipEvent_t stop = nullptr,
+                               int base = 0, hipEvent_t start = nullptr);
+static int launch_counter_sampler(ofdg_ctx* c, ofdg_ctx::Slot& sl, long long first_index, hipStream_t s, uint32_t* err, int split,
+                                  long long first_index2, uint32_t* err2) {
   const int stride = sl.res_shapes / sl.res_samples;
   const int prep = c->prm.background_prep ? 1 : 0;
   CsRealizeDims D{c->prm.width, c->prm.height, c->pool_n, c->pool_w, c->pool_h, sl.res_samples, stride, prep,
                   c->prm.mode == 9 ? c->crop_server.n_crops : 0, c->fg_src.stride, c->fg_src.origin, c->bg_src.stride, c->bg_src.origin,
                   (unsigned long long)(uintptr_t)c->pool.p, c->d_tex_table.p, c->prm.mode == 9 ? c->d_cs_croptab.p : nullptr};
   hipLaunchKernelGGL(cs_sample_realize_kernel, dim3(sl.res_samples * kCsGroups), dim3(64), 0, s, c->cs_mode, D, first_index,
-                     sl.d_shapes.p, sl.d_objects.p, sl.d_samples.p, err, sl.d_bgprep.p);
+                     sl.d_shapes.p, sl.d_objects.p, sl.d_samples.p, err, sl.d_bgprep.p, split, first_index2, err2);
   HIP_OK(c, hipGetLastError());
   sl.bgprep_pending = prep != 0;
   return OFDG_OK;
@@ -724,15 +733,24 @@
 }
 static hipStream_t chain_stream(const ofdg_ctx* c, const ofdg_ctx::Chain& ch, hipStream_t st) { return c->overlap ? ch.stream.s : st; }
 
+static int clean_discarded_word(ofdg_ctx* c, const ofdg_ctx::Chain::Prepared& p) {
+  if (p.ticket >= 0 && p.ticket + ofdg_ctx::kErrWords > c->ticket) {
+    HIP_OK(c, hipMemsetAsync(err_word(c, p.ticket), 0, sizeof(uint32_t), p.stream));
+    c->word_clean[(size_t)(p.ticket % ofdg_ctx::kErrWords)] = true;
+  }
+  return OFDG_OK;
+}
+static int discard_half(ofdg_ctx* c, ofdg_ctx::Chain& ch) {
+  if (!ch.half.valid) return OFDG_OK;
+  ch.half.valid = false;
+  return clean_discarded_word(c, ch.half);
+}
 static int discard_prepared(ofdg_ctx* c, ofdg_ctx::Chain& ch) {
+  OFDG_TRY(discard_half(c, ch));
   if (!ch.prep.valid) return OFDG_OK;
   ch.prep.valid = false;
   if (ch.prep.slot && ch.prep.slot->d_item_count.p) HIP_OK(c, hipMemsetAsync(ch.prep.slot->d_item_count.p, 0, sizeof(int), ch.prep.stream));
-  if (ch.prep.ticket >= 0 && ch.prep.ticket + ofdg_ctx::kErrWords > c->ticket) {
-    HIP_OK(c, hipMemsetAsync(err_word(c, ch.prep.ticket), 0, sizeof(uint32_t), ch.prep.stream));
-    c->word_clean[(size_t)(ch.prep.ticket % ofdg_ctx::kErrWords)] = true;
-  }
-  return OFDG_OK;
+  return clean_discarded_word(c, ch.prep);
 }
 static int discard_all_prepared(ofdg_ctx* c) {
   c->bg_cap_n = -1;
@@ -766,19 +784,26 @@
 }
 
 static int launch_prepare(ofdg_ctx* c, ofdg_ctx::Chain& ch, ofdg_ctx::Slot& sl, hipStream_t st, long long cs_first_index = -1,
-                          bool hand_over = true) {
+                          bool hand_over = true, int view_base = 0, int view_n = 0, long long cs_first2 = -1, int n_first = 0) {
   const int W = c->prm.width, H = c->prm.height;
   const int n_sf = sl.res_shapes * 2;
   const RenderDims dm = render_dims(c, sl);
+  const bool paired = cs_first_index >= 0 && cs_first2 >= 0;
   OFDG_TRY(discard_prepared(c, ch));
+  if (&sl != &ch.slot)
+    for (int k = 0; k < c->n_chains; ++k)
+      if (c->chains[k].half.valid && c->chains[k].half.slot == &sl) OFDG_TRY(discard_half(c, c->chains[k]));
   const long long ticket = c->ticket++;
   uint32_t* const err = err_word(c, ticket);
+  const long long ticket2 = paired ? c->ticket++ : -1;
+  uint32_t* const err2 = paired ? err_word(c, ticket2) : err;
   Event* ev = nullptr;
   if (c->profiling && c->ev_sets > 0 && (c->launch_count % c->ev_stride) == 0) {
     const size_t set = (size_t)(c->ev_alloc++ % c->ev_sets);
     ev = &c->ev[set * 6];
     c->ev_composed[set] = 0;
     c->ev_bgprep[set] = 0;
+    c->ev_front[set] = 1;
   }
   c->launch_count++;
   if (!c->overlap) {
@@ -792,8 +817,9 @@
   if (sl.compose_pending && sl.compose_stream != S) OFDG_TRY(wait_unless_fired(c, S, sl.compose_event, &sl.compose_pending));
   const DevCropRef* croptab = cs_first_index >= 0 ? c->d_cs_croptab.p : sl.d_croptab.p;
   HIP_OK(c, take_err_word(c, ticket, S));
+  if (paired) HIP_OK(c, take_err_word(c, ticket2, S));
   if (cs_first_index >= 0) {
-    OFDG_TRY(launch_counter_sampler(c, sl, cs_first_index, S, err));
+    OFDG_TRY(launch_counter_sampler(c, sl, cs_first_index, S, err, paired ? n_first : sl.res_samples, cs_first2, err2));
   }
   const int bp = sl.box_parity;
   sl.box_parity ^= 1;
@@ -804,23 +830,59 @@
   const bool prof_prep = ev && c->profiling == 2;
   hipExtLaunchKernelGGL(geom_kernel, dim3(std::max(1, (n_sf + kGeomWaves - 1) / kGeomWaves)), dim3(64 * kGeomWaves), 0, S,
                         prof_prep ? ev[0].e : nullptr, prof_prep ? ev[1].e : nullptr, 0, sl.d_shapes.p, sl.res_shapes, c->d_cs_tab.p, W, H,
-                        sl.d_frames.p, sl.d_verts.p, box_cur, err, sl.d_item_count.p, sl.d_items.p, croptab);
+                        sl.d_frames.p, sl.d_verts.p, box_cur, err, sl.d_item_count.p, sl.d_items.p, croptab,
+                        paired ? n_first * (sl.res_shapes / sl.res_samples) * 2 : 0x7fffffff, err2);
   HIP_OK(c, hipGetLastError());
   const bool prep_last = sl.bgprep_pending;
   hipEvent_t last_stop = ev ? (c->profiling == 2 ? nullptr : ev[4].e) : (hand_over ? ch.ev_prep.e : nullptr);
-  hipExtLaunchKernelGGL(raster_kernel, dim3(kRasterGrid * 4 / kRasterWaves), dim3(64 * kRasterWaves), 0, S, nullptr,
+  hipExtLaunchKernelGGL(raster_kernel, dim3((paired ? kRasterGridPaired : kRasterGrid) * 4 / kRasterWaves), dim3(64 * kRasterWaves), 0, S, nullptr,
                         (ev && (c->profiling == 2 || prep_last)) ? ev[3].e : (prep_last ? nullptr : last_stop), 0,
                         sl.d_frames.p, sl.d_items.p, sl.d_item_count.p, sl.d_verts.p, W, H, cov, box_next, n_mask_words, box_cur);
   HIP_OK(c, hipGetLastError());
   if (prep_last) {
-    OFDG_TRY(prepare_backgrounds(c, sl, sl.res_samples, true, S, err, (ev && c->profiling == 2) ? ev[2].e : last_stop));
+    OFDG_TRY(prepare_backgrounds(c, sl, paired ? n_first : sl.res_samples, true, S, err, (ev && c->profiling == 2) ? ev[2].e : last_stop));
     sl.bgprep_pending = false;
     if (ev) c->ev_bgprep[(size_t)(ev - c->ev.data()) / 6] = 1;
   }
   if (ev && hand_over) HIP_OK(c, hipEventRecord(ch.ev_prep, S));
-  ch.prep.valid = true; ch.prep.slot = &sl; ch.prep.first_index = cs_first_index; ch.prep.n = sl.res_samples;
+  ch.prep.valid = true; ch.prep.slot = &sl; ch.prep.first_index = cs_first_index;
+  ch.prep.n = paired ? n_first : (view_n > 0 ? view_n : sl.res_samples);
+  ch.prep.base = view_n > 0 ? view_base : 0;
   ch.prep.box_cur = box_cur; ch.prep.croptab = croptab; ch.prep.ev = ev; ch.prep.stream = S; ch.prep.ticket = ticket;
   ch.prep.ahead = false;
+  if (paired) {
+    ch.half = ch.prep;
+    ch.half.first_index = cs_first2; ch.half.base = n_first; ch.half.ev = nullptr; ch.half.ticket = ticket2;
+  }
+  return OFDG_OK;
+}
+
+static int launch_second_half(ofdg_ctx* c, ofdg_ctx::Chain& ch, bool hand_over) {
+  ofdg_ctx::Chain::Prepared h = ch.half;
+  ofdg_ctx::Slot& sl = *h.slot;
+  const hipStream_t S = h.stream;
+  const bool prep = c->prm.background_prep != 0;
+  Event* ev = nullptr;
+  if (c->profiling && c->ev_sets > 0 && (c->launch_count % c->ev_stride) == 0 && (c->profiling == 2 || prep)) {
+    const size_t set = (size_t)(c->ev_alloc++ % c->ev_sets);
+    ev = &c->ev[set * 6];
+    c->ev_composed[set] = 0;
+    c->ev_bgprep[set] = 0;
+    c->ev_front[set] = 0;
+  }
+  c->launch_count++;
+  if (ch.done_pending && ch.done_stream != S) OFDG_TRY(wait_unless_fired(c, S, ch.ev_done, &ch.done_pending, true));
+  if (sl.compose_pending && sl.compose_stream != S) OFDG_TRY(wait_unless_fired(c, S, sl.compose_event, &sl.compose_pending));
+  ch.half.valid = false;
+  h.ev = ev;
+  ch.prep = h;
+  if (prep) {
+    const bool prof2 = ev && c->profiling == 2;
+    const hipEvent_t stop = ev ? (prof2 ? ev[2].e : ev[4].e) : (hand_over ? ch.ev_prep.e : nullptr);
+    OFDG_TRY(prepare_backgrounds(c, sl, h.n, true, S, err_word(c, h.ticket), stop, h.base, prof2 ? ev[3].e : nullptr));
+    if (prof2) c->ev_bgprep[(size_t)(ev - c->ev.data()) / 6] = 1;
+  }
+  if (hand_over && (ev || !prep)) HIP_OK(c, hipEventRecord(ch.ev_prep, S));
   return OFDG_OK;
 }
 
@@ -925,7 +987,10 @@
 static int launch_compose_kernels(ofdg_ctx* c, const ofdg_ctx::Chain& ch, const ofdg_ctx::Slot& sl, const CallOut& o, const ComposeExtras& x,
                                   const uint32_t* fgpool, const uint32_t* bgpool, hipStream_t cs, hipEvent_t done) {
   const int W = c->prm.width, H = c->prm.height;
-  const RenderDims dm = render_dims(c, sl);
+  RenderDims dm = render_dims(c, sl);
+  dm.n_samples = ch.prep.n;
+  const DevSample* const samples = sl.d_samples.p + ch.prep.base;
+  const unsigned long long* const box = ch.prep.box_cur + (size_t)ch.prep.base * dm.tiles_x * ((H + kBandRows - 1) / kBandRows) * 2;
   const int grid = dm.tiles_x * dm.tiles_y * dm.n_samples * 4;
   Event* const ev = ch.prep.ev;
   enum class Kind { kRigid, kRigidExt, kRigidFmt, kRigidExtFmt, kDeform, kDeformFmt };
@@ -935,11 +1000,11 @@
   const Launch lc{(unsigned)grid, 64, cs, (ev && c->profiling == 2) ? ev[4].e : nullptr, ev ? ev[5].e : (x.occ ? nullptr : done)};
   auto compose = [&](auto* k_pow2, auto* k, auto... args) { launch_kernel(lc, pow2 ? k_pow2 : k, args...); };
   auto rigid = [&](auto* k_pow2, auto* k, auto... tail) {
-    compose(k_pow2, k, sl.d_samples.p, ch.prep.box_cur, sl.d_objects.p, ch.cov.p, grid, dm.tiles_x, dm.tiles_y, W, H, dm.use_aa, dm.bg_pitch,
+    compose(k_pow2, k, samples, box, sl.d_objects.p, ch.cov.p, grid, dm.tiles_x, dm.tiles_y, W, H, dm.use_aa, dm.bg_pitch,
             dm.fg_pitch, fgpool, bgpool, o.img0, o.img1, o.flow, sl.d_frames.p, sl.d_item_count.p, tail...);
   };
   auto deform = [&](auto* k_pow2, auto* k, auto... tail) {
-    compose(k_pow2, k, dm, sl.d_samples.p, sl.d_objects.p, ch.prep.box_cur, ch.cov.p, fgpool, bgpool, o.img0, o.img1, o.flow, sl.d_frames.p,
+    compose(k_pow2, k, dm, samples, sl.d_objects.p, box, ch.cov.p, fgpool, bgpool, o.img0, o.img1, o.flow, sl.d_frames.p,
             ch.prep.croptab, sl.d_item_count.p, tail...);
   };
   switch (kind) {
@@ -982,11 +1047,12 @@
   if (!ch.prep.valid) { c->err = "internal: compose without a prepared batch"; return OFDG_EINVAL; }
   ofdg_ctx::Slot& sl = *ch.prep.slot;
   ComposeExtras x;
-  OFDG_TRY(plan_extras(c, ch, sl.res_samples, o, &x));
+  OFDG_TRY(plan_extras(c, ch, ch.prep.n, o, &x));
   const uint32_t* bgpool = c->prm.background_prep ? sl.d_bgtex.p : (c->pool_bg.p ? c->pool_bg.p : c->pool.p);
   const uint32_t* fgpool = c->pool_fg.p ? c->pool_fg.p : c->pool.p;
   if (c->prm.background_prep && !bgpool) { c->err = "background_prep: the slot has no prepared backgrounds"; return OFDG_EINVAL; }
   c->last_slot = &sl; c->last_ch = &ch;
+  c->last_base = ch.prep.base; c->last_n = ch.prep.n;
   c->last_stream = ch.prep.stream; c->last_ticket = ch.prep.ticket;
   ch.prep.valid = false;
   const bool foreign = ch.prep.stream != st;
@@ -998,8 +1064,9 @@
   return note_compose(c, ch, sl, cs, foreign, done);
 }
 
-static int launch_resident(ofdg_ctx* c, ofdg_ctx::Chain& ch, ofdg_ctx::Slot& sl, const CallOut& o, hipStream_t st, long long cs_first_index = -1) {
-  OFDG_TRY(launch_prepare(c, ch, sl, st, cs_first_index, chain_stream(c, ch, st) != st));
+static int launch_resident(ofdg_ctx* c, ofdg_ctx::Chain& ch, ofdg_ctx::Slot& sl, const CallOut& o, hipStream_t st, long long cs_first_index = -1,
+                           int view_base = 0, int view_n = 0) {
+  OFDG_TRY(launch_prepare(c, ch, sl, st, cs_first_index, chain_stream(c, ch, st) != st, view_base, view_n));
   return launch_compose(c, ch, o, st);
 }
 
@@ -1026,10 +1093,14 @@
   return OFDG_OK;
 }
 
-static int prepare_backgrounds(ofdg_ctx* c, ofdg_ctx::Slot& sl, int n, bool records_resident, hipStream_t s, uint32_t* err, hipEvent_t stop) {
+static int prepare_backgrounds(ofdg_ctx* c, ofdg_ctx::Slot& sl, int n, bool records_resident, hipStream_t s, uint32_t* err, hipEvent_t stop, int base,
+                               hipEvent_t start) {
   const int W = c->prm.width, H = c->prm.height;
-  if (!records_resident || !sl.d_bgprep.p || sl.d_bgprep.cap < (size_t)n) { c->err = "internal: background preparation without its records"; return OFDG_EINVAL; }
-  HIP_OK(c, sl.d_bgtex.reserve((size_t)n * 4 * W * H));
+  if (!records_resident || !sl.d_bgprep.p || sl.d_bgprep.cap < (size_t)(base + n)) { c->err = "internal: background preparation without its records"; return OFDG_EINVAL; }
+  if (base == 0) HIP_OK(c, sl.d_bgtex.reserve((size_t)n * 4 * W * H));
+  else if (sl.d_bgtex.cap < (size_t)(base + n) * 4 * W * H) { c->err = "internal: background preparation of a second batch the slot was not sized for"; return OFDG_EINVAL; }
+  const DevBgPrep* const rec = sl.d_bgprep.p + base;
+  uint32_t* const tex = sl.d_bgtex.p + (size_t)base * 4 * W * H;
   int cap_cw, cap_ch;
   bool fusable;
   bgprep_caps(c, &cap_cw, &cap_ch, &fusable);
@@ -1039,22 +1110,22 @@
     OFDG_TRY(ensure_bgprep_tables(c));
   }
   if (!staged) {
-    hipExtLaunchKernelGGL(bgprep_kernel, dim3((W * H + 255) / 256, n), dim3(256), 0, s, nullptr, stop, 0, sl.d_bgprep.p, W, H, sl.d_bgtex.p);
+    hipExtLaunchKernelGGL(bgprep_kernel, dim3((W * H + 255) / 256, n), dim3(256), 0, s, start, stop, 0, rec, W, H, tex);
     HIP_OK(c, hipGetLastError());
     return OFDG_OK;
   }
   const DevResizeTabs T{c->d_bg_at_x.p, c->d_bg_alpha_x.p, c->d_bg_at_y.p, c->d_bg_alpha_y.p};
   if (fusable && n <= kPrepMaxSamples) {
-    hipExtLaunchKernelGGL(bgprep_stream_kernel, dim3(kPrepGrid), dim3(64), (size_t)(n + 1) * sizeof(int), s, nullptr, stop, 0, sl.d_bgprep.p, T, W, H, n, cap_cw, cap_ch, sl.d_bgtex.p, err,
+    hipExtLaunchKernelGGL(bgprep_stream_kernel, dim3(kPrepGrid), dim3(64), (size_t)(n + 1) * sizeof(int), s, start, stop, 0, rec, T, W, H, n, cap_cw, cap_ch, tex, err,
                           c->d_prep_paths.p);
     HIP_OK(c, hipGetLastError());
     return OFDG_OK;
   }
   HIP_OK(c, sl.d_bgC.reserve((size_t)n * cap_cw * cap_ch));
-  hipLaunchKernelGGL(bgprep_rotcrop_kernel, dim3(kBgPrepBlocks, n), dim3(256), 0, s, sl.d_bgprep.p, T, W, H, cap_cw, cap_ch, sl.d_bgC.p,
-                     err);
-  hipExtLaunchKernelGGL(bgprep_resize_kernel, dim3(kBgPrepBlocks, n), dim3(256), 0, s, nullptr, stop, 0, sl.d_bgprep.p, T, W, H, cap_cw, cap_ch, sl.d_bgC.p,
-                        sl.d_bgtex.p);
+  hipExtLaunchKernelGGL(bgprep_rotcrop_kernel, dim3(kBgPrepBlocks, n), dim3(256), 0, s, start, nullptr, 0, rec, T, W, H, cap_cw, cap_ch, sl.d_bgC.p,
+                        err);
+  hipExtLaunchKernelGGL(bgprep_resize_kernel, dim3(kBgPrepBlocks, n), dim3(256), 0, s, nullptr, stop, 0, rec, T, W, H, cap_cw, cap_ch, sl.d_bgC.p,
+                        tex);
   HIP_OK(c, hipGetLastError());
   return OFDG_OK;
 }
@@ -1209,7 +1280,9 @@
   stream = own_stream(c, stream);
   for (int k = 0; k < c->n_chains; ++k)
     if (&c->chains[k].slot == c->last_slot && !c->last_slot->compose_pending) HIP_OK(c, hipStreamSynchronize(c->chains[k].stream));
-  return launch_resident(c, take_chain(c), *c->last_slot, CallOut{"ofdg_render_resident", d_img0, d_img1, d_flow, {}, 0}, (hipStream_t)stream);
+  const int view_base = c->last_base, view_n = c->last_n;
+  return launch_resident(c, take_chain(c), *c->last_slot, CallOut{"ofdg_render_resident", d_img0, d_img1, d_flow, {}, 0}, (hipStream_t)stream, -1,
+                         view_base, view_n);
 }
 
 static_assert(sizeof(ofdg_object_row) == sizeof(DevObjectRow) && sizeof(ofdg_object_row) == 96 && offsetof(ofdg_object_row, area0) == 8 &&
@@ -1234,18 +1307,19 @@
   ofdg_ctx::Chain& ch = *c->last_ch;
   const hipStream_t S = c->last_stream;
   const hipStream_t st = stream == OFDG_STREAM_OWN ? S : (hipStream_t)stream;
-  const int W = c->prm.width, H = c->prm.height, n = sl.res_samples;
+  const int W = c->prm.width, H = c->prm.height, n = c->last_n;
+  const DevSample* const samples = sl.d_samples.p + c->last_base;
   const bool tracked = st != S || &sl != &ch.slot;
   const hipEvent_t done = tracked ? ch.ev_done.e : nullptr;
   const bool reduce = d_label0 || d_label1;
   DevObjectRow* const rows = reinterpret_cast<DevObjectRow*>(d_rows);
   const long long cells = (long long)n * rows_per_sample;
   hipExtLaunchKernelGGL(object_table_header_kernel, dim3((unsigned)((cells + 255) / 256)), dim3(256), 0, st, nullptr, reduce ? nullptr : done, 0,
-                        sl.d_samples.p, sl.d_objects.p, sl.d_shapes.p, n, rows_per_sample, W, H, rows, d_counts);
+                        samples, sl.d_objects.p, sl.d_shapes.p, n, rows_per_sample, W, H, rows, d_counts);
   HIP_OK(c, hipGetLastError());
   if (reduce) {
     hipExtLaunchKernelGGL(object_table_reduce_kernel, dim3((unsigned)((H + kTabBand - 1) / kTabBand), 2, (unsigned)n), dim3(64 * kTabWaves), 0,
-                          st, nullptr, done, 0, sl.d_samples.p, d_label0, d_label1, W, H, rows_per_sample, rows);
+                          st, nullptr, done, 0, samples, d_label0, d_label1, W, H, rows_per_sample, rows);
     HIP_OK(c, hipGetLastError());
   }
   if (tracked) track_completion(sl, ch, st, done);
@@ -1416,12 +1490,13 @@
   return OFDG_OK;
 }
 
-static int prepare_counter_slot(ofdg_ctx* c, ofdg_ctx::Slot& sl, int n) {
+static int prepare_counter_slot(ofdg_ctx* c, ofdg_ctx::Slot& sl, int n, int front = 1) {
   if (c->prm.mode == 9) OFDG_TRY(ensure_counter_croptab(c));
   OFDG_TRY(finalise_pool(c));
   OFDG_TRY(ensure_tex_table(c));
   if (!c->pool.p && !c->pool_mixed) { c->err = "Could not open texture collection (no texture pool)"; return OFDG_ETEXTURES; }
   if (n < 1 || n > 512) { c->err = "counter sampler: batch must be 1..512 samples"; return OFDG_EINVAL; }
+  n *= front;
   const int max_objects = c->prm.num_objects > 0 ? std::min(c->prm.num_objects, kCsMaxObjects) : 24;
   const size_t shapes_cap = (size_t)n * (size_t)(c->prm.mode >= 6 ? max_objects * 7 : max_objects);
   const size_t n_obj = (size_t)n * (1 + kCsMaxObjects);
@@ -1443,13 +1518,24 @@
     OFDG_TRY(prepare_counter_slot(c, cj.slot, n_samples));
     return launch_prepare(c, cj, cj.slot, s_, first, hand_over);
   };
-  OFDG_TRY(prepare_on(ch, first_index, st, chain_stream(c, ch, st) != st));
+  const long long prev_first = c->last_first;
+  const long long stride = (prev_first >= 0 && first_index > prev_first) ? first_index - prev_first
+                                                                           : (long long)n_samples * std::max(1, c->prm.world_size);
+  const bool hand_over = chain_stream(c, ch, st) != st;
+  if (c->front_batches == 2 && c->overlap && c->lookahead == 0 && 2 * n_samples <= 512) {
+    if (ch.half.valid && ch.half.slot == &ch.slot && ch.half.first_index == first_index && ch.half.n == n_samples && !ch.prep.valid) {
+      OFDG_TRY(launch_second_half(c, ch, hand_over));
+    } else {
+      OFDG_TRY(discard_prepared(c, ch));
+      OFDG_TRY(prepare_counter_slot(c, ch.slot, n_samples, 2));
+      OFDG_TRY(launch_prepare(c, ch, ch.slot, st, first_index, hand_over, 0, 0, first_index + (long long)c->n_chains * stride, n_samples));
+    }
+  } else {
+    OFDG_TRY(prepare_on(ch, first_index, st, hand_over));
+  }
   OFDG_TRY(launch_compose(c, ch, o, st));
-  const long long prev_first = c->last_first;
   c->last_first = first_index;
   if (c->overlap && c->lookahead > 0) {
-    const long long stride = (prev_first >= 0 && first_index > prev_first) ? first_index - prev_first
-                                                                             : (long long)n_samples * std::max(1, c->prm.world_size);
     for (int d = 1; d <= std::min(c->lookahead, c->n_chains - 1); ++d) {
       ofdg_ctx::Chain& cj = c->chains[(k + d) % c->n_chains];
       if (prepare_on(cj, first_index + (long long)d * stride, cj.stream, true) != OFDG_OK) { (void)discard_prepared(c, cj); break; }
@@ -1587,7 +1673,16 @@
       }
     }
   }
+  if (step != c->step) for (int k = 0; k < c->n_chains; ++k) OFDG_TRY(discard_half(c, c->chains[k]));
   c->step = step;
+  return OFDG_OK;
+}
+
+int ofdg_set_front_batches(ofdg_ctx* c, int n) {
+  if (!c || (n != 1 && n != 2)) { if (c) c->err = "ofdg_set_front_batches: n = " + std::to_string(n) + " (valid: 1, 2)"; return OFDG_EINVAL; }
+  for (int k = 0; k < c->n_chains; ++k) OFDG_TRY(discard_half(c, c->chains[k]));
+  c->front_batches = n;
+  c->info = c->info_head + " front=" + std::to_string(n);
   return OFDG_OK;
 }
 
@@ -1890,11 +1985,11 @@
   int cap_cw, cap_ch;
   bool fusable;
   bgprep_caps(c, &cap_cw, &cap_ch, &fusable);
-  const int n = sl.res_samples;
+  const int n = c->last_n;
   if (c->prm.background_prep != 1 || !fusable || n > kPrepMaxSamples || n < 1 || !sl.d_bgprep.p) return OFDG_OK;
   HIP_OK(c, hipDeviceSynchronize());
   std::vector<DevBgPrep> rec((size_t)n);
-  HIP_OK(c, hipMemcpy(rec.data(), sl.d_bgprep.p, rec.size() * sizeof(DevBgPrep), hipMemcpyDeviceToHost));
+  HIP_OK(c, hipMemcpy(rec.data(), sl.d_bgprep.p + c->last_base, rec.size() * sizeof(DevBgPrep), hipMemcpyDeviceToHost));
   for (const DevBgPrep& q : rec)
     if (prep_sample_fits(q, cap_cw, cap_ch)) *tiles += prep_tile_cols(q) * prep_tile_rows(q);
   return OFDG_OK;
@@ -1928,6 +2023,7 @@
   }
   c->ev_composed.assign((size_t)c->ev_sets, 0);
   c->ev_bgprep.assign((size_t)c->ev_sets, 0);
+  c->ev_front.assign((size_t)c->ev_sets, 0);
   return OFDG_OK;
 }
 
@@ -1948,6 +2044,7 @@
   for (int k = 0; k < c->ev_sets; ++k) {
     if (!c->ev_composed[(size_t)k]) continue;
     if (i == 3 && !c->ev_bgprep[(size_t)k]) continue;
+    if (i < 2 && !c->ev_front[(size_t)k]) continue;
     ++n;
     const Event* ev = &c->ev[(size_t)k * 6];
     HIP_OK(c, hipEventSynchronize(ev[5]));
diff --git a/optical-flow-2d-data-generation_amd/csrc/ofdg_device.h b/optical-flow-2d-data-generation_amd/csrc/ofdg_device.h
--- a/optical-flow-2d-data-generation_amd/csrc/ofdg_device.h
+++ b/optical-flow-2d-data-generation_amd/csrc/ofdg_device.h
@@ -12,6 +12,10 @@
 constexpr int kBandRows = 8;
 constexpr int kMaxFgObjects = 64;
 constexpr int kRasterGrid = 512;
+#ifndef OFDG_RASTER_GRID_PAIRED
+#define OFDG_RASTER_GRID_PAIRED 768
+#endif
+constexpr int kRasterGridPaired = OFDG_RASTER_GRID_PAIRED;
 
 constexpr uint32_t kErrVertCapacity = 1u;
 constexpr uint32_t kErrCurveCapacity = 2u;
diff --git a/optical-flow-2d-data-generation_amd/csrc/sampler_counter.hip b/optical-flow-2d-data-generation_amd/csrc/sampler_counter.hip
--- a/optical-flow-2d-data-generation_amd/csrc/sampler_counter.hip
+++ b/optical-flow-2d-data-generation_amd/csrc/sampler_counter.hip
@@ -463,11 +463,14 @@
 __global__ __launch_bounds__(64) void cs_sample_realize_kernel(CsMode M, CsRealizeDims D, long long first_index,
                                                                DevShape* __restrict__ shapes, DevObject* __restrict__ objects,
                                                                DevSample* __restrict__ samples, uint32_t* __restrict__ err,
-                                                               DevBgPrep* __restrict__ bgprep) {
+                                                               DevBgPrep* __restrict__ bgprep, int split, long long first_index2,
+                                                               uint32_t* __restrict__ err2) {
   __shared__ CsShared S;
   __shared__ Mat s_bgm;
   __builtin_amdgcn_s_setprio(3);
-  cs_sample_realize_block(S, s_bgm, (int)blockIdx.x, M, D, first_index, shapes, objects, samples, err, bgprep);
-}
-
-}
+  const bool second = (int)blockIdx.x / kCsGroups >= split;
+  cs_sample_realize_block(S, s_bgm, (int)blockIdx.x, M, D, second ? first_index2 - split : first_index, shapes, objects, samples,
+                          second ? err2 : err, bgprep);
+}
+
+}
```

Result: faster. 384,600, median of 6 (+8.0%).
